# Joao-M-Silva/padel_analytics

Measured on AMD Instinct MI355X. Metric: frames/sec (all trackers) on 1280x720, higher is better.
Workload: dtype f32-equivalent (h2: fp16 pairs h + m/2048, 2 or 3 f16 MFMA products per multiply, fp32 accumulate)

## Files before the change

include/padel_hip.h:

```cpp
#ifndef PADEL_HIP_H
#define PADEL_HIP_H

#include <stddef.h>
#include <stdint.h>

#ifdef __cplusplus
extern "C" {
#endif

typedef struct pa_engine pa_engine;
typedef struct pa_model pa_model;

#define PA_ABI_VERSION 5


enum pa_op_kind {
    PA_OP_STEM = 1,
    PA_OP_CONV = 2,
    PA_OP_SPPF_POOL = 3,
    PA_OP_UPSAMPLE2X = 4,
    PA_OP_MAXPOOL2 = 5,
    PA_OP_STEM7 = 6,
    PA_OP_MAXPOOL3S2 = 7,
    PA_OP_GAP_FC = 8,
    PA_OP_DWCONV3 = 9,
    PA_OP_PSA_ATTN = 10
};

enum pa_act { PA_ACT_NONE = 0, PA_ACT_SILU = 1, PA_ACT_RELU = 2, PA_ACT_SIGMOID = 3, PA_ACT_LEAKY = 4  };

typedef struct pa_buf_desc {
    int32_t level;
    int32_t channels;
} pa_buf_desc;

typedef struct pa_op_desc {
    int32_t kind;
    int32_t in_buf, in_choff, cin;
    int32_t out_buf, out_choff, cout;
    int32_t ksize, stride, act;
    int32_t res_buf, res_choff;
    int32_t npad;
    int32_t reserved;
    int64_t w_off, b_off;
    int32_t flags;
    int32_t pad_;
} pa_op_desc;
#define PA_CONV_W_SINGLE 1
#define PA_CONV_RES_PREACT 4

enum pa_task { PA_TASK_DETECT = 0, PA_TASK_POSE = 1, PA_TASK_TRACKNET = 2, PA_TASK_RESNET = 3  };

enum pa_dtype { PA_DTYPE_F32 = 0, PA_DTYPE_F16 = 1, PA_DTYPE_H2 = 2 };

typedef struct pa_model_desc {
    int32_t task;
    int32_t nc;
    int32_t nk, kpt_dim;
    int32_t n_bufs;
    const pa_buf_desc* bufs;
    int32_t n_ops;
    const pa_op_desc* ops;
    int32_t head_buf[3];
    int32_t in_channels;
    int32_t dtype;
} pa_model_desc;

int pa_abi_version(void);
int pa_device_count(void);
int pa_engine_create(int device_id, pa_engine** out);
void pa_engine_destroy(pa_engine* eng);
const char* pa_last_error(pa_engine* eng);
int pa_engine_synchronize(pa_engine* eng);

int pa_device_malloc(pa_engine* eng, size_t nbytes, void** out_dev);
int pa_device_free(pa_engine* eng, void* dev);
size_t pa_device_bytes_live(void);
int pa_memcpy_h2d(pa_engine* eng, void* dst_dev, const void* src_host, size_t nbytes);
int pa_memcpy_d2h(pa_engine* eng, void* dst_host, const void* src_dev, size_t nbytes);
int pa_upload(pa_engine* eng, void* dst_dev, const void* src_host, size_t nbytes);

int pa_host_register(pa_engine* eng, void* ptr, size_t nbytes);
int pa_host_unregister(pa_engine* eng, void* ptr);

enum pa_yuv_layout {
    PA_YUV_NV12 = 0,
    PA_YUV_I420 = 1
};
typedef struct pa_yuv_desc {
    int32_t layout;
    int32_t pitch_y, pitch_c;
    int32_t off_u, off_v;
    int32_t reserved;
    int64_t frame_stride;
    int32_t y_off, cy, cvr, cug, cvg, cub;
} pa_yuv_desc;
int pa_yuv420_to_bgr(pa_engine* eng, const uint8_t* src, int src_on_device, int n, int h, int w,
                     const pa_yuv_desc* d, uint8_t* dst_bgr_dev);
int pa_yuv_last_path(pa_engine* eng);

enum pa_mark_kind { PA_MARK_DISC = 1, PA_MARK_SEGMENT = 2, PA_MARK_FILL = 3, PA_MARK_BOX = 4, PA_MARK_GLYPH = 5, PA_MARK_BLEND = 6 };
typedef struct pa_mark {
    int32_t kind;
    int32_t x0, y0, x1, y1;
    int32_t size;
    uint32_t bgr;
    int32_t arg;
} pa_mark;
typedef struct pa_yuv_enc {
    int32_t y_off;
    int32_t yr, yg, yb, ur, ug, ub, vr, vg, vb;
} pa_yuv_enc;
enum pa_render_out { PA_RENDER_BGR = 0, PA_RENDER_YUV420 = 1 };
int pa_render(pa_engine* eng, const uint8_t* src_bgr_dev, int n, int h, int w, const pa_mark* marks_host, const int32_t* first_host,
              int out, const pa_yuv_desc* geom, const pa_yuv_enc* enc, uint8_t* dst_dev);
int pa_render_check(int n, int h, int w, const pa_mark* marks_host, const int32_t* first_host, int out, const pa_yuv_desc* geom,
                    const pa_yuv_enc* enc, char* why, size_t cap);
int pa_render_last_path(pa_engine* eng);
int pa_glyph_rows(int code, uint8_t rows[7]);

#define PA_ACTIVITY_MAX_SIDE 16384
#define PA_ACTIVITY_MAX_FRAMES 65535
const char* pa_frame_activity_check(int n, int h, int w, const int32_t* roi, int tau);
int pa_frame_activity(pa_engine* eng, const uint8_t* frames_bgr_dev, int n, int h, int w, const uint8_t* ref_bgr_dev,
                      const uint8_t* prev_bgr_dev_or_null, const int32_t* roi_or_null, int tau, uint64_t* out_u64);
int pa_frames_median(pa_engine* eng, const uint8_t* frames_bgr_dev, int n, int h, int w, uint8_t* out_bgr_dev);

#define PA_BOX_HIST_BINS 512
#define PA_BOX_HIST_MAX_RECTS 16384
const char* pa_box_histograms_check(int n, int h, int w, const int32_t* rects, int k);
int pa_box_histograms(pa_engine* eng, const uint8_t* frames_bgr_dev, int n, int h, int w,
                      const int32_t* rects , int k, uint32_t* out_u32 );

#define PA_JPEG_MAX_WIDTH 2560
int pa_jpeg_encode(pa_engine* eng, const uint8_t* src_yuv_dev, int n, int h, int w, const pa_yuv_desc* geom, int quality,
                   uint8_t* dst_host, size_t cap, int64_t* offsets_host);
int pa_jpeg_check(int n, int h, int w, const pa_yuv_desc* geom, int quality, char* why, size_t cap);
size_t pa_jpeg_interval_bytes(int w);

#define PA_JPEG_DEC_MAX_DIM 4096
#define PA_JPEG_DEC_MAX_BYTES (1 << 27)
enum { PA_JPEG_ST_CODE = 1, PA_JPEG_ST_INDEX = 2, PA_JPEG_ST_SIZE = 4, PA_JPEG_ST_DATA = 8, PA_JPEG_ST_MARKERS = 16 };
typedef struct pa_jpeg_huff {
    uint8_t bits[16];
    uint8_t vals[256];
    int32_t nvals;
} pa_jpeg_huff;
typedef struct pa_jpeg_interval {
    int64_t begin, end;
    int32_t first_mcu, mcus;
} pa_jpeg_interval;
typedef struct pa_jpeg_frame_info {
    int32_t w, h, mcus_x, mcus_y;
    int32_t restart_interval;
    int32_t n_intervals;
    int32_t default_huffman;
    int32_t status;
    int64_t scan_begin, scan_end;
    uint8_t quant[3][64];
    uint8_t comp_dc[3], comp_ac[3], pad_[2];
    pa_jpeg_huff dc[2], ac[2];
} pa_jpeg_frame_info;
int pa_jpeg_parse(const uint8_t* jpeg, size_t len, pa_jpeg_frame_info* info, pa_jpeg_interval* ivls, size_t ivl_cap, char* why,
                  size_t cap);
int pa_jpeg_decode(pa_engine* eng, const uint8_t* jpegs_host, const int64_t* offsets, int n, int h, int w, uint8_t* dst_bgr_dev,
                   int32_t* status_host);
#define PA_JPEG_DEC_SPLIT_MIN_BYTES 7168
#define PA_JPEG_DEC_SPLIT_SUB_BYTES 128
int pa_jpeg_decode_set_split(pa_engine* eng, int64_t min_bytes, int32_t sub_bytes);
int pa_jpeg_decode_last_split(pa_engine* eng, int64_t out[4]);
int pa_jpeg_decode_last_path(pa_engine* eng);
int pa_jpeg_decode_last_times(pa_engine* eng, double ms[5]);

int pa_engine_timer_start(pa_engine* eng);
int pa_engine_timer_stop(pa_engine* eng, float* ms);

int pa_engine_set_tuning(pa_engine* eng, const char* key, int value);
int pa_engine_set_timeline_path(pa_engine* eng, const char* path);

int pa_model_create(pa_engine* eng, const pa_model_desc* desc, const float* weights, size_t n_floats,
                    pa_model** out);
void pa_model_destroy(pa_model* m);
int pa_model_take_overflow(pa_model* m, int* out);
int pa_model_set_max_batch(pa_model* m, int max_batch);
int pa_model_plan_bytes(pa_model* m, size_t* arena_bytes, size_t* logical_bytes);

int pa_model_fill_arena(pa_model* m, int byte_value);

enum pa_pre_mode {
    PA_PRE_LETTERBOX = 0,
    PA_PRE_PIL_STRETCH = 1
};

typedef struct pa_yolo_params {
    int32_t imgsz;
    int32_t pre_mode;
    int32_t channel_reverse;
    int32_t letterbox_auto;
    float conf, iou;
    int32_t max_det;
    int32_t n_classes;
    const int32_t* classes;
    int32_t frames_on_device;
} pa_yolo_params;

int pa_yolo_infer(pa_model* m, const uint8_t* frames, int n, int h, int w, const pa_yolo_params* p,
                  float* out_boxes, float* out_kpts, int32_t* out_counts);

#define PA_MAX_INFLIGHT 4
int pa_yolo_submit(pa_model* m, const uint8_t* frames, int n, int h, int w, const pa_yolo_params* p,
                   float* out_boxes, float* out_kpts, int32_t* out_counts, int* ticket);
int pa_yolo_wait(pa_model* m, int ticket, int* overflow);

int pa_yolo_postprocess(pa_model* m, const float* const* heads, int n, int h, int w, const pa_yolo_params* p,
                        float* out_boxes, float* out_kpts, int32_t* out_counts);

int pa_yolo_head_shape(pa_model* m, int level, int* h, int* w, int* c);
int pa_yolo_read_head(pa_model* m, int level, int n, float* out);
int pa_yolo_last_post_path(pa_model* m);
int pa_model_lanes_allocated(pa_model* m);
int pa_yolo_resample_passes(pa_model* m);
int pa_model_last_lane(pa_model* m);
int pa_model_last_stem_path(pa_model* m);

int pa_yolo_netin_shape(pa_model* m, int* h, int* w);
int pa_yolo_read_netin(pa_model* m, int n, uint8_t* out);

int pa_tracknet_infer(pa_model* m, const float* x, int n, int h, int w, int x_on_device, float* out,
                      int out_on_device);

int pa_resnet_infer(pa_model* m, const uint8_t* frames, int n, int h, int w, int frames_on_device, float* out_xy, float* out_logits);
int pa_resnet_read_netin(pa_model* m, int n, uint8_t* out);
int pa_resnet_read_fc(pa_model* m, int n, float* out_xy, float* out_logits);
int pa_resnet_read_head(pa_model* m, int n, float* out);

int pa_pil_coeffs(int in_size, int out_size, int filter, int32_t* bounds, int32_t* coefs, int coefs_cap, int* ksize);

typedef struct pa_ball pa_ball;
int pa_ball_create(pa_model* tracknet, int src_h, int src_w, pa_ball** out);
void pa_ball_destroy(pa_ball* b);
int pa_ball_set_background(pa_ball* b, const uint8_t* median_rgb);
int pa_ball_background_from_frames(pa_ball* b, const uint8_t* frames_bgr, int n, int frames_on_device,
                                   uint8_t* out_median_rgb);
int pa_ball_feed(pa_ball* b, const uint8_t* frames_bgr, int n, int frames_on_device, int flush,
                 uint8_t* out_masks, float* out_heat, int32_t* out_rects, int* out_count);

int pa_ball_locate(pa_ball* b, const uint8_t* masks, int n, int32_t* out_rects);

int pa_ball_read_resized(pa_ball* b, long long frame, uint8_t* out);

int pa_comm_unique_id(void* out, size_t cap);
int pa_engine_comm_init(pa_engine* eng, const void* unique_id, size_t id_bytes, int nranks, int rank);
void pa_engine_comm_destroy(pa_engine* eng);
int pa_engine_bcast_weights(pa_engine* eng, pa_model* m, int root);
int pa_engine_bcast_weights_from(pa_engine* eng, pa_model* src, pa_model* dst, int root);
int pa_engine_bcast(pa_engine* eng, void* dev_ptr, size_t nbytes, int root);
int pa_engine_allreduce_max(pa_engine* eng, double* value);
int pa_engine_gather_sizes(pa_engine* eng, size_t nbytes, uint64_t* sizes);
int pa_engine_gather(pa_engine* eng, const void* send, size_t nbytes, void* recv, size_t recv_cap, const uint64_t* sizes, int root);

typedef struct pa_bytetrack pa_bytetrack;
int pa_bytetrack_create(double track_activation_threshold, int lost_track_buffer, double minimum_matching_threshold,
                        int frame_rate, pa_bytetrack** out);
void pa_bytetrack_destroy(pa_bytetrack* b);
void pa_bytetrack_reset(pa_bytetrack* b);
int pa_bytetrack_update_batch(pa_bytetrack* b, const float* boxes, const int32_t* counts, const uint8_t* keep,
                              int n_frames, int stride, int32_t* out_ids);

int pa_engine_set_profiling(pa_engine* eng, int enable);
int pa_model_last_profile(pa_model* m, int cap, int32_t* kinds, float* ms, double* flops, int32_t* ksizes);
int pa_model_profile_text(pa_model* m, char* buf, size_t cap);

#ifdef __cplusplus
}
#endif
#endif
```

padel_analytics_amd/csrc/conv_patch_h2v.hip:

```cpp
#include "h2_common.h"

namespace padel {

namespace {

constexpr int kVSpans = (kPatchSqPix + 15) / 16;
constexpr int kVPlaneB = kVSpans * 1024;
constexpr int kVTSpans = (kPatchSqPix + 31) / 32;
constexpr int kVTPlaneB = kVTSpans * 1024;

}

template <int NF, bool CHUNK, bool TAIL, bool WS>
__global__ void __launch_bounds__(256, 2) conv_h2v_kernel(const ConvArgs a) {
    static_assert(CHUNK || TAIL, "cin = 32 CHUNK + 16 TAIL");
    static_assert(WS || NF <= 2, "three products: 2 fragments per wave (6 register sets of 4 VGPRs per step)");
    constexpr int MF = 4;
    constexpr int PATCH_B = (CHUNK ? 2 * kVPlaneB : 0);
    constexpr int TPATCH_B = (TAIL ? 2 * kVTPlaneB : 0);
    constexpr int NSTEPS = (CHUNK ? 9 : 0) + (TAIL ? 5 : 0);
    constexpr int NPL = WS ? 1 : 2;
    constexpr int NW = NF * NPL;
    __shared__ __attribute__((aligned(16))) float lds[(PATCH_B + TPATCH_B) / 4];
    char* const ldsb = reinterpret_cast<char*>(lds);
    const int tid = threadIdx.x;
    const int lane = tid & 63;
    const int wave = __builtin_amdgcn_readfirstlane(tid >> 6);
    const int lr = lane & 15, lq = lane >> 4;

    const int nmt = a.n_mtiles, nnt = a.n_ntiles;
    const int bid = blockIdx.x;
    const XcdSlot slot = xcd_slot(nmt, nnt, bid);
    if (xcd_slot_padding(slot)) return;
    const int mt = xcd_slot_mtile(slot), nt = slot.nt;
    const TileOrigin org = tile_origin<4, 4>(a.Ho, a.Wo, mt);
    const int n = org.n, y0 = org.y0, x0 = org.x0;
    const int f0 = nt * NF;

    const float* const in0 = a.in + (((long long)n * a.H + (y0 - 1)) * a.W + (x0 - 1)) * a.in_cs + a.in_choff;
    const i32x4 rsrcP = make_rsrc(in0);
    const unsigned lp0 = __builtin_amdgcn_readfirstlane((unsigned)(uintptr_t)lds);

    if constexpr (CHUNK) {
        const int p_lane = lane >> 2;
        const int p_q = (lane & 3) ^ (((lane >> 4) & 1) << 1);
        const unsigned p_piece = (unsigned)((p_q >> 1) * 64 + (p_q & 1) * 16);
#define PADEL_HV_PSPAN(S_)                                                                                        \
        if (((S_) & 3) == wave) {                                                                                 \
            const int pp_ = (S_) * 16 + p_lane;                                                                   \
            const int py_ = pp_ / kPatchW, px_ = pp_ - py_ * kPatchW;                                             \
            const bool ok_ = pp_ < kPatchSqPix && (unsigned)(y0 - 1 + py_) < (unsigned)a.H && (unsigned)(x0 - 1 + px_) < (unsigned)a.W; \
            const unsigned vo_ = ok_ ? (unsigned)((py_ * a.W + px_) * a.in_cs * 4) + p_piece : kOOR;              \
            lds_dma<(S_) * 1024>(vo_, rsrcP, 0u, lp0);                                                            \
            lds_dma<kVPlaneB + (S_) * 1024>(vo_, rsrcP, 32u, lp0);                                                \
        }
        PADEL_HV_PSPAN(0) PADEL_HV_PSPAN(1) PADEL_HV_PSPAN(2) PADEL_HV_PSPAN(3) PADEL_HV_PSPAN(4) PADEL_HV_PSPAN(5) PADEL_HV_PSPAN(6)
        PADEL_HV_PSPAN(7) PADEL_HV_PSPAN(8) PADEL_HV_PSPAN(9) PADEL_HV_PSPAN(10) PADEL_HV_PSPAN(11) PADEL_HV_PSPAN(12) PADEL_HV_PSPAN(13)
        PADEL_HV_PSPAN(14) PADEL_HV_PSPAN(15) PADEL_HV_PSPAN(16) PADEL_HV_PSPAN(17) PADEL_HV_PSPAN(18) PADEL_HV_PSPAN(19) PADEL_HV_PSPAN(20)
#undef PADEL_HV_PSPAN
    }
    if constexpr (TAIL) {
        const int t_lane = lane >> 1;
        const unsigned t_piece = (unsigned)(((lane & 1) ^ ((lane >> 4) & 1)) * 16);
        const unsigned t_so = CHUNK ? 128u : 0u;
#define PADEL_HV_TSPAN(S_)                                                                                        \
        if (((S_) & 3) == ((wave + 1) & 3)) {                                                                     \
            const int pp_ = (S_) * 32 + t_lane;                                                                   \
            const int py_ = pp_ / kPatchW, px_ = pp_ - py_ * kPatchW;                                             \
            const bool ok_ = pp_ < kPatchSqPix && (unsigned)(y0 - 1 + py_) < (unsigned)a.H && (unsigned)(x0 - 1 + px_) < (unsigned)a.W; \
            const unsigned vo_ = ok_ ? (unsigned)((py_ * a.W + px_) * a.in_cs * 4) + t_piece : kOOR;              \
            lds_dma<PATCH_B + (S_) * 1024>(vo_, rsrcP, t_so, lp0);                                                \
            lds_dma<PATCH_B + kVTPlaneB + (S_) * 1024>(vo_, rsrcP, t_so + 32u, lp0);                              \
        }
        PADEL_HV_TSPAN(0) PADEL_HV_TSPAN(1) PADEL_HV_TSPAN(2) PADEL_HV_TSPAN(3) PADEL_HV_TSPAN(4) PADEL_HV_TSPAN(5)
        PADEL_HV_TSPAN(6) PADEL_HV_TSPAN(7) PADEL_HV_TSPAN(8) PADEL_HV_TSPAN(9) PADEL_HV_TSPAN(10)
#undef PADEL_HV_TSPAN
    }

    constexpr unsigned fragb = (unsigned)NSTEPS * 2048u;
    const unsigned voffW = (unsigned)lane * 16u;
    i32x4 rsrcW[NF];
#pragma unroll
    for (int j = 0; j < NF; ++j) {
        const int frag = min(f0 + j, a.n16 - 1);
        rsrcW[j] = make_rsrc(reinterpret_cast<const char*>(a.wr) + (long long)frag * fragb);
    }
    i32x4 w[3][NF], wm[3][WS ? 1 : NF];
#define PADEL_HV_LOADW(ST_)                                                                                       \
    do {                                                                                                          \
        const unsigned so_ = (unsigned)((ST_) * 2048);                                                            \
        _Pragma("unroll") for (int j = 0; j < NF; ++j) {                                                          \
            asm volatile("buffer_load_dwordx4 %0, %1, %2, %3 offen"                                               \
                         : "=v"(w[(ST_) % 3][j]) : "v"(voffW), "s"(rsrcW[j]), "s"(so_) : "memory");               \
            if constexpr (!WS)                                                                                    \
                asm volatile("buffer_load_dwordx4 %0, %1, %2, %3 offen offset:1024"                               \
                             : "=v"(wm[(ST_) % 3][j]) : "v"(voffW), "s"(rsrcW[j]), "s"(so_) : "memory");          \
        }                                                                                                         \
    } while (0)
#define PADEL_HV_WAITW(ST_, N_)                                                                                   \
    do {                                                                                                          \
        if constexpr (NF == 3)                                                                                    \
            asm volatile("s_waitcnt vmcnt(%3)" : "+v"(w[(ST_) % 3][0]), "+v"(w[(ST_) % 3][1]), "+v"(w[(ST_) % 3][2]) : "n"(N_) : "memory"); \
        else if constexpr (NF == 2 && WS)                                                                         \
            asm volatile("s_waitcnt vmcnt(%2)" : "+v"(w[(ST_) % 3][0]), "+v"(w[(ST_) % 3][1]) : "n"(N_) : "memory"); \
        else if constexpr (NF == 2)                                                                               \
            asm volatile("s_waitcnt vmcnt(%4)" : "+v"(w[(ST_) % 3][0]), "+v"(w[(ST_) % 3][1]), "+v"(wm[(ST_) % 3][0]), "+v"(wm[(ST_) % 3][WS ? 0 : NF - 1]) \
                         : "n"(N_) : "memory");                                                                   \
        else if constexpr (WS)                                                                                    \
            asm volatile("s_waitcnt vmcnt(%1)" : "+v"(w[(ST_) % 3][0]) : "n"(N_) : "memory");                     \
        else                                                                                                      \
            asm volatile("s_waitcnt vmcnt(%2)" : "+v"(w[(ST_) % 3][0]), "+v"(wm[(ST_) % 3][0]) : "n"(N_) : "memory"); \
    } while (0)

    unsigned rbase[8];
    if constexpr (CHUNK) {
#pragma unroll
        for (int r = 0; r < 8; ++r) {
            const int p0 = 4 * wave * kPatchW + lr;
            rbase[r] = (unsigned)(p0 * 64 + ((lq ^ ((((p0 + r) >> 2) & 1) << 1)) << 4));
        }
    }
    const int rd_pix = 4 * wave * kPatchW + lr;

    f32x4 acc[MF][NF], part[MF][NF], cross[MF][NF];
#pragma unroll
    for (int f = 0; f < MF; ++f)
#pragma unroll
        for (int j = 0; j < NF; ++j) { acc[f][j] = (f32x4){0.f, 0.f, 0.f, 0.f}; part[f][j] = acc[f][j]; cross[f][j] = acc[f][j]; }
    h16x8 ah[4], am[4];
#define PADEL_HV_READROW(R_, KX_)                                                                                 \
    do {                                                                                                          \
        constexpr int d_ = (R_) * kPatchW + (KX_);                                                                \
        const char* p_ = ldsb + rbase[d_ & 7];                                                                    \
        ah[(R_) & 3] = *reinterpret_cast<const h16x8*>(p_ + d_ * 64);                                             \
        am[(R_) & 3] = *reinterpret_cast<const h16x8*>(p_ + d_ * 64 + kVPlaneB);                                  \
    } while (0)
#define PADEL_HV_MFMA_ROW(F_, S_, ST_)                                                                            \
    do {                                                                                                          \
        _Pragma("unroll") for (int j = 0; j < NF; ++j)                                                            \
            cross[F_][j] = __builtin_amdgcn_mfma_f32_16x16x32_f16(__builtin_bit_cast(h16x8, w[(ST_) % 3][j]), am[S_], cross[F_][j], 0, 0, 0); \
        if constexpr (!WS) {                                                                                      \
            _Pragma("unroll") for (int j = 0; j < NF; ++j)                                                        \
                cross[F_][j] = __builtin_amdgcn_mfma_f32_16x16x32_f16(__builtin_bit_cast(h16x8, wm[(ST_) % 3][WS ? 0 : j]), ah[S_], cross[F_][j], 0, 0, 0); \
        }                                                                                                         \
        _Pragma("unroll") for (int j = 0; j < NF; ++j)                                                            \
            part[F_][j] = __builtin_amdgcn_mfma_f32_16x16x32_f16(__builtin_bit_cast(h16x8, w[(ST_) % 3][j]), ah[S_], part[F_][j], 0, 0, 0); \
        __builtin_amdgcn_sched_barrier(0);                                                                        \
    } while (0)
#define PADEL_HV_TOP(ST_)                                                                                         \
    do {                                                                                                          \
        if constexpr ((ST_) + 2 < NSTEPS) PADEL_HV_LOADW((ST_) + 2);                                              \
        PADEL_HV_WAITW(ST_, NW * (((ST_) + 1 < NSTEPS ? 1 : 0) + ((ST_) + 2 < NSTEPS ? 1 : 0)));                  \
        __builtin_amdgcn_sched_barrier(0);                                                                        \
    } while (0)
#define PADEL_HV_STEP(T_)                                                                                         \
    do {                                                                                                          \
        constexpr int kx_ = h2_tap_kx(T_), ky_ = h2_tap_ky(T_);                                                   \
        PADEL_HV_TOP(T_);                                                                                         \
        if constexpr (ky_ == 0) {                                                                                 \
            PADEL_HV_MFMA_ROW(0, 0, T_);                                                                          \
            PADEL_HV_READROW(4, kx_);                                                                             \
            __builtin_amdgcn_sched_barrier(0);                                                                    \
            PADEL_HV_MFMA_ROW(1, 1, T_); PADEL_HV_MFMA_ROW(2, 2, T_); PADEL_HV_MFMA_ROW(3, 3, T_);                \
        } else if constexpr (ky_ == 1) {                                                                          \
            PADEL_HV_MFMA_ROW(0, 1, T_);                                                                          \
            PADEL_HV_READROW(5, kx_);                                                                             \
            __builtin_amdgcn_sched_barrier(0);                                                                    \
            PADEL_HV_MFMA_ROW(1, 2, T_); PADEL_HV_MFMA_ROW(2, 3, T_); PADEL_HV_MFMA_ROW(3, 0, T_);                \
        } else {                                            \
            PADEL_HV_MFMA_ROW(2, 0, T_);                                                                          \
            if constexpr (kx_ < 2) PADEL_HV_READROW(0, kx_ + 1);                                                  \
            __builtin_amdgcn_sched_barrier(0);                                                                    \
            PADEL_HV_MFMA_ROW(3, 1, T_);                                                                          \
            if constexpr (kx_ < 2) PADEL_HV_READROW(1, kx_ + 1);                                                  \
            __builtin_amdgcn_sched_barrier(0);                                                                    \
            PADEL_HV_MFMA_ROW(0, 2, T_);                                                                          \
            if constexpr (kx_ < 2) PADEL_HV_READROW(2, kx_ + 1);                                                  \
            __builtin_amdgcn_sched_barrier(0);                                                                    \
            PADEL_HV_MFMA_ROW(1, 3, T_);                                                                          \
            if constexpr (kx_ < 2) PADEL_HV_READROW(3, kx_ + 1);                                                  \
            __builtin_amdgcn_sched_barrier(0);                                                                    \
        }                                                                                                         \
    } while (0)
#define PADEL_HV_TSTEP(JT_, ST_)                                                                                  \
    do {                                                                                                          \
        constexpr int ta_ = 2 * (JT_), tb_ = 2 * (JT_) + 1 < 9 ? 2 * (JT_) + 1 : 8;                               \
        int rp_ = rd_pix;                                                                                         \
        asm volatile("" : "+v"(rp_));                                                                             \
        _Pragma("unroll") for (int f = 0; f < MF; ++f) {                                                          \
            const int pa_ = rp_ + (f + h2_tap_ky(ta_)) * kPatchW + h2_tap_kx(ta_), pb_ = rp_ + (f + h2_tap_ky(tb_)) * kPatchW + h2_tap_kx(tb_); \
            const char* p_ = ldsb + PATCH_B + swz_tail_off((lq >> 1) ? pb_ : pa_, lq & 1);                        \
            ah[f] = *reinterpret_cast<const h16x8*>(p_);                                                          \
            am[f] = *reinterpret_cast<const h16x8*>(p_ + kVTPlaneB);                                              \
        }                                                                                                         \
        __builtin_amdgcn_sched_barrier(0);                                                                        \
        PADEL_HV_TOP(ST_);                                                                                        \
        PADEL_HV_MFMA_ROW(0, 0, ST_); PADEL_HV_MFMA_ROW(1, 1, ST_); PADEL_HV_MFMA_ROW(2, 2, ST_); PADEL_HV_MFMA_ROW(3, 3, ST_); \
    } while (0)
#define PADEL_HV_FLUSH()                                                                                          \
    do {                                                                                                          \
        _Pragma("unroll") for (int f = 0; f < MF; ++f)                                                            \
            _Pragma("unroll") for (int j = 0; j < NF; ++j) { acc[f][j] += part[f][j]; part[f][j] = (f32x4){0.f, 0.f, 0.f, 0.f}; } \
    } while (0)

    PADEL_HV_LOADW(0);
    if constexpr (NSTEPS > 1) PADEL_HV_LOADW(1);
    wait_vm<NW * (NSTEPS > 1 ? 2 : 1)>();
    __builtin_amdgcn_s_barrier();
    asm volatile("" ::: "memory");
    if constexpr (CHUNK) {
        PADEL_HV_READROW(0, 0); PADEL_HV_READROW(1, 0); PADEL_HV_READROW(2, 0); PADEL_HV_READROW(3, 0);
        __builtin_amdgcn_sched_barrier(0);
        PADEL_HV_STEP(0); PADEL_HV_STEP(1); PADEL_HV_STEP(2); PADEL_HV_STEP(3); PADEL_HV_STEP(4);
        PADEL_HV_STEP(5); PADEL_HV_STEP(6); PADEL_HV_STEP(7); PADEL_HV_STEP(8);
        PADEL_HV_FLUSH();
    }
    if constexpr (TAIL) {
        constexpr int S0 = CHUNK ? 9 : 0;
        PADEL_HV_TSTEP(0, S0); PADEL_HV_TSTEP(1, S0 + 1); PADEL_HV_TSTEP(2, S0 + 2); PADEL_HV_TSTEP(3, S0 + 3); PADEL_HV_TSTEP(4, S0 + 4);
        PADEL_HV_FLUSH();
    }
#undef PADEL_HV_FLUSH
#undef PADEL_HV_TSTEP
#undef PADEL_HV_STEP
#undef PADEL_HV_TOP
#undef PADEL_HV_MFMA_ROW
#undef PADEL_HV_READROW
#undef PADEL_HV_WAITW
#undef PADEL_HV_LOADW

    int mpix[MF];
#pragma unroll
    for (int f = 0; f < MF; ++f) {
        const int oy = y0 + 4 * wave + f, ox = x0 + lr;
        mpix[f] = (oy < a.Ho && ox < a.Wo) ? (n * a.Ho + oy) * a.Wo + ox : -1;
    }
    const bool fast = y0 + 16 <= a.Ho && x0 + 16 <= a.Wo && (f0 + NF) * 16 <= a.cout && (((a.out_choff | a.out_cs) & 3) == 0) &&
                      (!a.res || (((a.res_choff | a.res_cs) & 3) == 0));
    h2_epilogue<MF, NF>(a, acc, cross, mpix, f0, lq, fast);
}

template <int NF, bool WS>
static hipError_t launch_hv(const ConvArgs& a_in, hipStream_t s) {
    ConvArgs a = a_in;
    const int batch = a.M / (a.Ho * a.Wo);
    a.n_mtiles = batch * ((a.Ho + 15) / 16) * ((a.Wo + 15) / 16);
    a.n_ntiles = (a.n16 + NF - 1) / NF;
    dim3 grid(8u * (unsigned)((a.n_mtiles + 7) / 8) * (unsigned)a.n_ntiles, 1, 1);
    if (a.cin == 48) hipLaunchKernelGGL((conv_h2v_kernel<NF, true, true, WS>), grid, dim3(256), 0, s, a);
    else if (a.cin == 32) hipLaunchKernelGGL((conv_h2v_kernel<NF, true, false, WS>), grid, dim3(256), 0, s, a);
    else hipLaunchKernelGGL((conv_h2v_kernel<NF, false, true, WS>), grid, dim3(256), 0, s, a);
    return hipGetLastError();
}

hipError_t launch_conv_h2v(const ConvArgs& a, int tile, hipStream_t s) {
    const int nf = tile - 340;
    if (a.w_single) {
        switch (nf) {
            case 1: return launch_hv<1, true>(a, s);
            case 2: return launch_hv<2, true>(a, s);
            case 3: return launch_hv<3, true>(a, s);
        }
    } else {
        switch (nf) {
            case 1: return launch_hv<1, false>(a, s);
            case 2: return launch_hv<2, false>(a, s);
        }
    }
    return hipErrorNotSupported;
}

}
```

padel_analytics_amd/csrc/conv_select.cpp:

```cpp
#include "kernels.h"

#include <string.h>

namespace padel {

struct ConvTile {
    int id;
    ConvFamily family;
    int rows, cols, bn;
    float s3, s1;
};

static const ConvTile kTapTiles[] = {
    {7, CONV_TAP, 0, 64, 96, 1.00f, 1.00f},   {13, CONV_TAP, 0, 128, 96, 0.99f, 0.99f}, {9, CONV_TAP, 0, 128, 64, 0.99f, 0.99f},
    {14, CONV_TAP, 0, 128, 128, 1.00f, 1.00f}, {6, CONV_TAP, 0, 64, 128, 0.98f, 0.98f},  {20, CONV_TAP, 0, 128, 48, 0.98f, 0.98f},
    {11, CONV_TAP, 0, 128, 32, 0.99f, 0.99f},  {12, CONV_TAP, 0, 128, 16, 0.80f, 0.80f},
    {10, CONV_TAP, 0, 128, 64, 0.f, 0.f},
    {15, CONV_TAP, 0, 128, 64, 0.f, 0.f},
};

static const ConvTile kBx3Tiles[] = {
    {213, CONV_BX3T, 0, 128, 96, 1.07f, 1.08f},
    {220, CONV_BX3T, 0, 128, 48, 1.00f, 1.00f}, {207, CONV_BX3T, 0, 64, 96, 0.98f, 0.95f}, {209, CONV_BX3T, 0, 128, 64, 1.00f, 1.00f},
    {206, CONV_BX3T, 0, 64, 128, 0.90f, 0.70f}, {211, CONV_BX3T, 0, 128, 32, 0.85f, 0.87f}, {225, CONV_BX3T, 0, 64, 80, 0.95f, 0.90f},
    {7, CONV_BX3T, 0, 64, 96, 0.93f, 0.84f},    {20, CONV_BX3T, 0, 128, 48, 0.93f, 0.87f}, {13, CONV_BX3T, 0, 128, 96, 0.85f, 0.82f},
    {14, CONV_BX3T, 0, 128, 128, 0.83f, 0.85f}, {25, CONV_BX3T, 0, 64, 80, 0.90f, 0.78f},
    {11, CONV_BX3T, 0, 128, 32, 0.80f, 0.61f},  {9, CONV_BX3T, 0, 128, 64, 0.65f, 0.70f},  {6, CONV_BX3T, 0, 64, 128, 0.50f, 0.49f},
    {12, CONV_BX3T, 0, 128, 16, 0.45f, 0.26f},
    {303, CONV_BX3P, 8, 16, 48, 1.17f, 0.f},    {304, CONV_BX3P, 8, 16, 64, 1.14f, 0.f},   {306, CONV_BX3P, 8, 16, 96, 0.f, 0.f},
#ifdef PADEL_BX3_PROBES
    {420, CONV_BX3T, 0, 128, 48, 0.f, 0.f},     {520, CONV_BX3T, 0, 128, 48, 0.f, 0.f},    {620, CONV_BX3T, 0, 128, 48, 0.f, 0.f},
    {720, CONV_BX3T, 0, 128, 48, 0.f, 0.f},     {820, CONV_BX3T, 0, 128, 48, 0.f, 0.f},    {920, CONV_BX3T, 0, 128, 48, 0.f, 0.f},
    {1020, CONV_BX3T, 0, 128, 48, 0.f, 0.f},    {1120, CONV_BX3T, 0, 128, 48, 0.f, 0.f},
#endif
};

static const ConvTile kH2Tiles[] = {
    {213, CONV_H2T, 0, 128, 96, 1.07f, 1.08f},
    {220, CONV_H2T, 0, 128, 48, 1.00f, 1.00f}, {207, CONV_H2T, 0, 64, 96, 0.98f, 0.95f}, {209, CONV_H2T, 0, 128, 64, 1.00f, 1.00f},
    {211, CONV_H2T, 0, 128, 32, 0.85f, 0.87f}, {225, CONV_H2T, 0, 64, 80, 0.95f, 0.90f},
    {239, CONV_H2D, 0, 128, 64, 0.f, 0.f},     {243, CONV_H2D, 0, 128, 96, 0.f, 0.f},
    {244, CONV_H2S, 0, 128, 96, 0.f, 0.f},     {245, CONV_H2S, 0, 128, 192, 0.f, 0.f},   {247, CONV_H2S, 0, 64, 192, 0.f, 0.f},
    {246, CONV_H2S3, 0, 128, 192, 0.f, 0.f},   {248, CONV_H2S3, 0, 64, 192, 0.f, 0.f},
    {303, CONV_H2P, 8, 16, 48, 1.17f, 0.f},    {304, CONV_H2P, 8, 16, 64, 1.10f, 0.f},
    {313, CONV_H2P, 8, 16, 48, 0.f, 0.f},
    {323, CONV_H2Q, 8, 16, 96, 1.21f, 0.f},
    {324, CONV_H2R, 8, 16, 96, 1.40f, 0.f},
    {325, CONV_H2R, 8, 16, 64, 1.33f, 0.f},
    {341, CONV_H2V, 16, 16, 16, 0.f, 0.f},     {341, CONV_H2W, 16, 16, 16, 1.28f, 0.f},
    {342, CONV_H2V, 16, 16, 32, 0.f, 0.f},     {342, CONV_H2W, 16, 16, 32, 1.42f, 0.f},
    {343, CONV_H2V, 16, 16, 48, 0.f, 0.f},     {343, CONV_H2W, 16, 16, 48, 1.46f, 0.f},
#ifdef PADEL_H2P_PROBES
    {333, CONV_H2P, 8, 16, 48, 0.f, 0.f},      {334, CONV_H2P, 8, 16, 48, 0.f, 0.f},     {335, CONV_H2P, 8, 16, 48, 0.f, 0.f},
    {336, CONV_H2P, 8, 16, 48, 0.f, 0.f},      {337, CONV_H2P, 8, 16, 48, 0.f, 0.f},     {339, CONV_H2P, 8, 16, 48, 0.f, 0.f},
    {340, CONV_H2P, 8, 16, 48, 0.f, 0.f},      {347, CONV_H2P, 8, 16, 48, 0.f, 0.f},     {348, CONV_H2P, 8, 16, 48, 0.f, 0.f},
    {349, CONV_H2P, 8, 16, 48, 0.f, 0.f},      {363, CONV_H2P, 8, 16, 48, 0.f, 0.f},
#endif
};
static const float kH2rThreeProducts = 1.22f;

static const ConvTile kF16Tiles[] = {
    {30, CONV_TAP16, 0, 128, 128, 1.30f, 1.30f},
    {31, CONV_TAP16, 0, 128, 96, 1.25f, 1.25f},  {32, CONV_TAP16, 0, 128, 64, 1.10f, 1.10f},  {6, CONV_TAP16, 0, 64, 128, 1.05f, 1.05f},
    {7, CONV_TAP16, 0, 64, 96, 1.00f, 1.00f},    {9, CONV_TAP16, 0, 128, 64, 1.00f, 1.00f},   {20, CONV_TAP16, 0, 128, 48, 0.95f, 0.95f},
    {11, CONV_TAP16, 0, 128, 32, 0.85f, 0.85f},  {12, CONV_TAP16, 0, 128, 16, 0.60f, 0.60f},
    {49, CONV_TAP16D, 0, 128, 64, 1.40f, 0.f},   {72, CONV_TAP16D, 0, 128, 64, 1.40f, 0.f},
    {46, CONV_TAP16D, 0, 64, 128, 0.f, 0.f},     {47, CONV_TAP16D, 0, 64, 96, 0.f, 0.f},      {51, CONV_TAP16D, 0, 128, 32, 0.f, 0.f},
    {60, CONV_TAP16D, 0, 128, 48, 0.f, 0.f},     {70, CONV_TAP16D, 0, 128, 128, 0.f, 0.f},    {71, CONV_TAP16D, 0, 128, 96, 0.f, 0.f},
    {304, CONV_P16, 8, 16, 64, 1.70f, 0.f},      {303, CONV_P16, 8, 16, 48, 1.55f, 0.f},      {306, CONV_P16, 8, 16, 96, 1.45f, 0.f},
    {323, CONV_P16Q, 16, 16, 48, 0.f, 0.f},      {324, CONV_P16Q, 16, 16, 64, 0.f, 0.f},      {326, CONV_P16Q, 16, 16, 96, 1.78f, 0.f},
};

struct TileSpan { const ConvTile* t; int n; };
static TileSpan tiles_of(int path) {
    switch (path) {
        case CONV_PATH_TAP: return {kTapTiles, (int)(sizeof(kTapTiles) / sizeof(ConvTile))};
        case CONV_PATH_BX3: return {kBx3Tiles, (int)(sizeof(kBx3Tiles) / sizeof(ConvTile))};
        case CONV_PATH_H2: return {kH2Tiles, (int)(sizeof(kH2Tiles) / sizeof(ConvTile))};
        case CONV_PATH_F16: return {kF16Tiles, (int)(sizeof(kF16Tiles) / sizeof(ConvTile))};
    }
    return {nullptr, 0};
}
static const ConvTile* find_tile(int path, int id, int family = -1) {
    const TileSpan ts = tiles_of(path);
    for (int i = 0; i < ts.n; ++i)
        if (ts.t[i].id == id && (family < 0 || ts.t[i].family == family)) return &ts.t[i];
    return nullptr;
}

bool conv_tile_shape(int path, int id, int* bm, int* bn) {
    const ConvTile* t = find_tile(path, id);
    if (!t) return false;
    *bm = t->rows ? t->rows * t->cols : t->cols;
    *bn = t->bn;
    return true;
}

int conv_timeline_words(const ConvLaunched& k, int ksize) {
    if (!strcmp(k.family, "h2q") || (!strcmp(k.family, "h2r") && k.tile == 324)) return kPatchDbgWords;
    if (!strcmp(k.family, "tap") && k.tile == 7 && ksize == 3) return kConvDbgWords;
    return 0;
}

int h2_ksteps(int cin, int ksize) { return ksize == 3 ? (cin >> 5) * 9 + ((cin & 16) ? 5 : 0) : (cin + 31) >> 5; }
size_t conv_h2r_copy_bytes(int n16, int cin, int ksize) { return (size_t)n16 * (size_t)h2_ksteps(cin, ksize) * 2048; }

static bool few_channels(int cin) { return cin == 16 || cin == 32 || cin == 48; }
static bool whole_chunks(int cin, int at_least) { return (cin & 31) == 0 && cin >= at_least; }
static bool h2r_layer(int k, int s, int cin) { return k == 3 && s == 1 && whole_chunks(cin, 64); }
static bool h2v_layer(int k, int s, int cin) { return k == 3 && s == 1 && few_channels(cin); }
static bool h2s_layer(int k, int s, int cin) { return k == 1 && s == 1 && whole_chunks(cin, 64); }
static bool h2s3_layer(int k, int s, int cin) { return k == 3 && s == 2 && whole_chunks(cin, 32); }
static bool stem_l1_layer(int k, int s, int cin) { return k == 3 && s == 2 && few_channels(cin); }

bool conv_wants_operand_copy(int ksize, int stride, int cin, bool w_single) {
    return h2r_layer(ksize, stride, cin) || h2v_layer(ksize, stride, cin) || stem_l1_layer(ksize, stride, cin) ||
           (w_single && (h2s_layer(ksize, stride, cin) || h2s3_layer(ksize, stride, cin)));
}

static bool same_size(const ConvArgs& a) { return a.Ho == a.H && a.Wo == a.W; }
static bool up_ok(const ConvArgs& a) { return (a.up_c & 31) == 0 && a.up_c > 0 && a.up_c <= a.cin && ((a.H | a.W) & 1) == 0; }
static bool up_ok_1x1(const ConvArgs& a) { return !a.in2 || (a.ksize == 1 && a.stride == 1 && up_ok(a)); }
static bool up_ok_patch(const ConvArgs& a) { return !a.in2 || ((a.cin & 31) == 0 && up_ok(a)); }

static bool conv_bx3p_supported(const ConvArgs& a) {
    return a.ksize == 3 && a.stride == 1 && (a.cin & 15) == 0 && a.cin >= 16 && same_size(a) && a.w3 != nullptr && up_ok_patch(a);
}
static bool conv_h2p_supported(const ConvArgs& a) {
    return a.ksize == 3 && a.stride == 1 && (a.cin & 15) == 0 && a.cin >= 16 && same_size(a) && a.w != nullptr && up_ok_patch(a);
}
static bool conv_h2q_supported(const ConvArgs& a) {
    return a.ksize == 3 && a.stride == 1 && whole_chunks(a.cin, 32) && same_size(a) && a.w != nullptr && !a.in2;
}
static bool conv_h2r_supported(const ConvArgs& a) {
    return a.wr && h2r_layer(a.ksize, a.stride, a.cin) && same_size(a) && a.w != nullptr && !a.in2;
}
static bool conv_h2w_supported(const ConvArgs& a) {
    return a.ksize == 3 && a.stride == 1 && few_channels(a.cin) && same_size(a) && a.w != nullptr && !a.in2;
}
static bool conv_h2v_supported(const ConvArgs& a) {
    return a.wr && h2v_layer(a.ksize, a.stride, a.cin) && same_size(a) && a.w != nullptr && !a.in2;
}
static bool conv_h2s_supported(const ConvArgs& a) {
    return a.w_single && a.wr && h2s_layer(a.ksize, a.stride, a.cin) && same_size(a) && a.w != nullptr && !a.in2 &&
           (long long)128 * a.in_cs * 4 < 0x7FFFFFFFll;
}
static bool conv_h2s3_supported(const ConvArgs& a) {
    return a.w_single && a.wr && h2s3_layer(a.ksize, a.stride, a.cin) && a.w != nullptr && !a.in2 && a.Ho <= (a.H + 1) / 2 &&
           a.Wo <= (a.W + 1) / 2 && (long long)4 * a.W * a.in_cs * 4 < 0x3FFFFFFFll;
}
static bool conv_p16_supported(const ConvArgs& a) { return a.ksize == 3 && a.stride == 1 && whole_chunks(a.cin, 32) && same_size(a); }

static bool family_takes(ConvFamily family, const ConvArgs& a, int id) {
    switch (family) {
        case CONV_TAP: case CONV_TAP16: case CONV_TAP16D: return true;
        case CONV_BX3T: return id < 400 ? up_ok_1x1(a) : a.ksize == 3;
        case CONV_BX3P: return conv_bx3p_supported(a);
        case CONV_H2T: return up_ok_1x1(a);
        case CONV_H2D: return a.ksize == 1 && up_ok_1x1(a);
        case CONV_H2S: return conv_h2s_supported(a);
        case CONV_H2S3: return conv_h2s3_supported(a);
        case CONV_H2P: return conv_h2p_supported(a) && (id < 330 || (!a.in2 && !(a.cin & 16)));
        case CONV_H2Q: return conv_h2q_supported(a);
        case CONV_H2R: return conv_h2r_supported(a) && (id == 325 || a.w_single);
        case CONV_H2V: return !(a.tune & 8) && conv_h2v_supported(a) && (id < 343 || a.w_single);
        case CONV_H2W: return conv_h2w_supported(a);
        case CONV_P16: case CONV_P16Q: return conv_p16_supported(a);
    }
    return false;
}

struct Resolved { int tile; ConvFamily family; };
static bool take(int path, const ConvArgs& a, int id, ConvFamily family, Resolved* out) {
    if (!find_tile(path, id, family) || !family_takes(family, a, id)) return false;
    out->tile = id; out->family = family;
    return true;
}
static bool take(int path, const ConvArgs& a, int id, Resolved* out) {
    const ConvTile* t = find_tile(path, id);
    return t && take(path, a, id, t->family, out);
}

static bool resolve_bx3(const ConvArgs& a, int id, Resolved* out) {
    if ((a.cin & 15) || a.cin < 16 || !a.w3) return false;
    const bool patch_id = id >= 300 && id < 400;
    if (a.in2 && a.ksize == 3) return patch_id && take(CONV_PATH_BX3, a, id, CONV_BX3P, out);
    if (a.in2) {
        id = (id == 209 || id == 9 || id == 304) ? 209 : (id == 213 || id == 13 || id == 14 || id == 306 || id == 206 || id == 6) ? 213 : 220;
        return take(CONV_PATH_BX3, a, id, CONV_BX3T, out);
    }
    if (patch_id) {
        if (conv_bx3p_supported(a)) return take(CONV_PATH_BX3, a, id, CONV_BX3P, out);
        id = id == 303 ? 220 : id == 304 ? 209 : 206;
    }
    return take(CONV_PATH_BX3, a, id, CONV_BX3T, out);
}

static bool resolve_f16(const ConvArgs& a, int id, Resolved* out) {
    if ((a.cin & 31) || a.cin < 32 || a.res_pre) return false;
    if (id >= 300 && id < 400) {
        if (conv_p16_supported(a)) return take(CONV_PATH_F16, a, id, out);
        id = id == 303 ? 20 : id == 304 ? 9 : 31;
    }
    return take(CONV_PATH_F16, a, id, out);
}

static bool resolve_h2(const ConvArgs& a, int id, Resolved* out) {
    const int P = CONV_PATH_H2;
    if ((a.cin & 15) || a.cin < 16 || !a.w || !a.oscale || !a.ovf_flag) return false;
    if (id >= 341 && id <= 343) {
        if (take(P, a, id, CONV_H2V, out) || take(P, a, id, CONV_H2W, out)) return true;
        id = 303;
    }
    if (id == 324 || id == 325) {
        if (take(P, a, id, CONV_H2R, out)) return true;
        id = id == 324 ? 323 : 304;
    }
    if (id == 323) {
        if (take(P, a, id, CONV_H2Q, out)) return true;
        id = 303;
    }
    if (a.in2 && a.ksize == 3) return id >= 300 && id < 400 && take(P, a, id, CONV_H2P, out);
    if (id >= 300 && id < 400) {
        if (conv_h2p_supported(a)) return take(P, a, id, CONV_H2P, out);
        const int nf = id - 300;
        id = (nf == 3 || nf == 13) ? 220 : (nf == 4 || nf == 14) ? 209 : 213;
    }
    if (id == 246 || id == 248) {
        if (take(P, a, id, CONV_H2S3, out)) return true;
        id = 213;
    }
    if (id == 244 || id == 245 || id == 247) {
        if (take(P, a, id, CONV_H2S, out)) return true;
        id = 243;
    }
    if (id == 243 || id == 239) {
        if (take(P, a, id, CONV_H2D, out)) return true;
        id -= 30;
    }
    return take(P, a, id, CONV_H2T, out);
}

const char* conv_family_name(ConvFamily f) {
    static const char* const names[] = {"tap", "bx3t", "bx3p", "h2t", "h2d", "h2s", "h2s3", "h2p", "h2q", "h2r", "h2w", "h2v", "tap16", "tap16d", "p16", "p16q"};
    return names[f];
}

bool resolve_conv(int path, const ConvArgs& a, int requested, ConvLaunched* out, ConvFamily* family) {
    Resolved r{-1, CONV_TAP};
    if (a.ksize != 3 && a.ksize != 1) return false;
    bool ok = false;
    switch (path) {
        case CONV_PATH_TAP: ok = !(a.cin & 15) && a.cin >= 16 && !a.res_pre && take(path, a, requested, &r); break;
        case CONV_PATH_BX3: ok = resolve_bx3(a, requested, &r); break;
        case CONV_PATH_H2: ok = resolve_h2(a, requested, &r); break;
        case CONV_PATH_F16: ok = resolve_f16(a, requested, &r); break;
    }
    if (ok && out) *out = ConvLaunched{r.tile, conv_family_name(r.family)};
    if (ok && family) *family = r.family;
    return ok;
}

static float tile_score(const ConvTile& t, const ConvArgs& a, float speed, bool rounds = true) {
    const int nf = t.bn / 16, bm = t.rows ? t.rows * t.cols : t.cols;
    const long long mtiles = t.rows ? (long long)(a.M / (a.Ho * a.Wo)) * ((a.Ho + t.rows - 1) / t.rows) * ((a.Wo + t.cols - 1) / t.cols)
                                    : (long long)((a.M + bm - 1) / bm);
    const int ntiles = (a.n16 + nf - 1) / nf;
    const float fill = (float)a.n16 / (float)(ntiles * nf) * (float)a.M / (float)(mtiles * bm);
    if (!rounds) return speed * fill;
    const long long blocks = mtiles * ntiles;
    const long long per_cu = (blocks + 255) / 256;
    if (t.rows) return speed * fill * (float)blocks / (256.f * (float)per_cu);
    const float occ = (float)blocks / (256.f * (float)per_cu);
    return speed * fill * occ;
}
struct Best {
    float score = -1.f;
    int id;
    void offer(float sc, int tile) { if (sc > score) { score = sc; id = tile; } }
};
static void offer_linear(Best& b, int path, const ConvArgs& a) {
    const TileSpan ts = tiles_of(path);
    for (int i = 0; i < ts.n; ++i) {
        const float sp = a.ksize == 3 ? ts.t[i].s3 : ts.t[i].s1;
        if (!ts.t[i].rows && sp > 0.0f) b.offer(tile_score(ts.t[i], a, sp), ts.t[i].id);
    }
}

int choose_conv_tap_variant(int M, int n16) {
    ConvArgs a{};
    a.M = M; a.n16 = n16; a.ksize = 3;
    Best b{-1.f, 7};
    offer_linear(b, CONV_PATH_TAP, a);
    return b.id;
}

int choose_conv_bx3_variant(const ConvArgs& a) {
    Best b{-1.f, 7};
    offer_linear(b, CONV_PATH_BX3, a);
    if (conv_bx3p_supported(a))
        for (const ConvTile& t : kBx3Tiles)
            if (t.rows && t.s3 > 0.f) b.offer(tile_score(t, a, t.s3), t.id);
    return b.id;
}

int choose_conv_tap16_variant(const ConvArgs& a) {
    const bool dbl_ok = a.ksize == 3 && (a.cin & 63) == 0 && a.cin >= 128;
    const int nch = a.cin >> 5;
    const bool patch_ok = conv_p16_supported(a);
    Best b{-1.f, 7};
    for (const ConvTile& t : kF16Tiles) {
        if (t.s3 <= 0.f) continue;
        if (t.rows) {
            if (patch_ok) b.offer(tile_score(t, a, t.s3 * (float)nch / (float)(nch + 1)), t.id);
            continue;
        }
        const bool dbl = t.family == CONV_TAP16D;
        if (dbl && !dbl_ok) continue;
        const int ntiles = (a.n16 + t.bn / 16 - 1) / (t.bn / 16);
        const float reread = 1.0f / (1.0f + 0.25f * (float)(ntiles - 1));
        b.offer(tile_score(t, a, t.s3) * (dbl ? 1.0f : reread), t.id);
    }
    return b.id;
}

int choose_conv_h2_variant(const ConvArgs& a) {
    const int n16 = a.n16, ksize = a.ksize;
    Best b{-1.f, 220};
    offer_linear(b, CONV_PATH_H2, a);
    int& bv = b.id;
    if (ksize == 1 && a.cin >= 192 && (bv == 213 || bv == 209)) bv += 30;
    if (ksize == 1 && a.w_single && n16 >= 24 && a.cin >= 384 && conv_h2s_supported(a)) bv = 245;
    if (ksize == 1 && a.w_single && n16 >= 12 && (float)(((n16 + 11) / 12) * 12) <= 1.1f * (float)n16 && a.cin >= 192 && a.cin < 960 &&
        conv_h2s_supported(a)) bv = 247;
    if (ksize == 3 && a.stride == 2 && n16 >= 10 && (float)(((n16 + 11) / 12) * 12) <= 1.2f * (float)n16 && conv_h2s3_supported(a)) bv = 246;
    if (bv == 246 && a.cin != 192) bv = 248;
    if (!conv_h2p_supported(a)) return bv;
    for (const ConvTile& t : kH2Tiles) {
        if (!t.rows || t.s3 <= 0.f || !family_takes(t.family, a, t.id)) continue;
        if (t.id == 323 && n16 % 6 != 0) continue;
        const bool persistent = t.family == CONV_H2R;
        b.offer(tile_score(t, a, t.id == 325 && !a.w_single ? kH2rThreeProducts : t.s3, !persistent), t.id);
    }
    if (bv == 303 && (a.cin & 16)) bv = 313;
    return bv;
}

}
```

padel_analytics_amd/csrc/engine.cpp:

```cpp
#include "engine_internal.h"

#include <atomic>

thread_local std::string g_err;

static std::atomic<size_t> g_live_bytes{0};
int dev_alloc(void** p, size_t bytes) { const hipError_t r = hipMalloc(p, bytes); if (r == hipSuccess) g_live_bytes += bytes; return (int)r; }
void dev_free(void* p, size_t bytes) { (void)hipFree(p); g_live_bytes -= bytes; }
int pin_alloc(void** p, size_t bytes) { return (int)hipHostMalloc(p, bytes, hipHostMallocDefault); }
void pin_free(void* p, size_t) { (void)hipHostFree(p); }
size_t pa_device_bytes_live(void) { return g_live_bytes.load(); }

static int knob_raw(int v) { return v; }
static int knob_flag(int v) { return v ? 1 : 0; }
static int knob_tap_pd(int v) { return v == 3 ? 3 : 2; }
static int knob_lanes(int v) { return v >= 2 ? 2 : 1; }
static const struct Knob { const char* key; const char* env; int Tuning::*field; int (*norm)(int); } kKnobs[] = {
    {"variant", "PADEL_CONV_VARIANT", &Tuning::variant, knob_raw},
    {"tune", "PADEL_CONV_TUNE", &Tuning::tune, knob_raw},
    {"tap_pd", "PADEL_CONV_TAP_PD", &Tuning::tap_pd, knob_tap_pd},
    {"graph", "PADEL_GRAPH", &Tuning::graph, knob_flag},
    {"timeline", nullptr, &Tuning::timeline, knob_flag},
    {"alias", "PADEL_ALIAS", &Tuning::alias, knob_flag},
    {"fold_up", "PADEL_FOLD_UP", &Tuning::fold_up, knob_flag},
    {"lanes", "PADEL_LANES", &Tuning::lanes, knob_lanes},
    {"fuse_stem", "PADEL_FUSE_STEM", &Tuning::fuse_stem, knob_raw},
    {"fuse_sppf", "PADEL_FUSE_SPPF", &Tuning::fuse_sppf, knob_raw},
    {"fuse_head", "PADEL_FUSE_HEAD", &Tuning::fuse_head, knob_flag},
    {"fuse_stem_cv1", "PADEL_FUSE_STEM_CV1", &Tuning::fuse_stem_cv1, knob_flag},
    {"w_single", nullptr, &Tuning::w_single, knob_flag},
};

int pa_abi_version(void) { return PA_ABI_VERSION; }

int pa_device_count(void) {
    int n = 0;
    if (hipGetDeviceCount(&n) != hipSuccess) return 0;
    return n;
}

const char* pa_last_error(pa_engine* eng) { return eng ? eng->err.c_str() : g_err.c_str(); }

int pa_engine_create(int device_id, pa_engine** out) {
    if (!out) PA_FAIL((pa_engine*)nullptr, "pa_engine_create: out is NULL");
    int n = 0;
    PA_HIP((pa_engine*)nullptr, hipGetDeviceCount(&n));
    if (device_id < 0 || device_id >= n) PA_FAIL((pa_engine*)nullptr, "pa_engine_create: device %d of %d", device_id, n);
    PA_HIP((pa_engine*)nullptr, hipSetDevice(device_id));
    pa_engine* e = new pa_engine();
    e->dev = device_id;
    hipError_t r = e->create_streams();
    if (r == hipSuccess) r = hipStreamCreateWithFlags(&e->copy_stream, hipStreamNonBlocking);
    if (r != hipSuccess) { pa_engine_destroy(e); PA_FAIL((pa_engine*)nullptr, "hipStreamCreate: %s", hipGetErrorString(r)); }
    r = (hipError_t)e->zeros.alloc(256);
    if (r == hipSuccess) r = hipMemset(e->zeros.get(), 0, 256);
    if (r != hipSuccess) { delete e; PA_FAIL((pa_engine*)nullptr, "zero page: %s", hipGetErrorString(r)); }
    r = padel::init_misc_kernels();
    if (r == hipSuccess) r = padel::init_head_tail_kernels();
    if (r != hipSuccess) { delete e; PA_FAIL((pa_engine*)nullptr, "kernel attributes: %s", hipGetErrorString(r)); }
    if (const char* v = getenv("PADEL_CONV_IMPL")) {
        if (v[0] == 'l') { delete e; PA_FAIL((pa_engine*)nullptr, "PADEL_CONV_IMPL=%s: the LDS kernel was retired in round 5; tap or bx3", v); }
        e->t.impl = (v[0] == 'b') ? 2 : 0;
    }
    for (const Knob& k : kKnobs)
        if (const char* v = k.env ? getenv(k.env) : nullptr) e->t.*k.field = k.norm(atoi(v));
    *out = e;
    return 0;
}

hipError_t pa_engine::create_streams() {
    hipError_t r = hipStreamCreateWithFlags(&main_, hipStreamNonBlocking);
    for (int i = 0; i < kMaxLanes && r == hipSuccess; ++i) {
        r = hipStreamCreateWithFlags(&lane_stream[i], hipStreamNonBlocking);
        if (r == hipSuccess) r = hipEventCreateWithFlags(&fork_ev_[i], hipEventDisableTiming);
    }
    return r;
}

void pa_engine::destroy_streams() {
    for (int i = 0; i < kMaxLanes; ++i) {
        if (lane_stream[i]) { hipStreamSynchronize(lane_stream[i]); hipStreamDestroy(lane_stream[i]); }
        if (fork_ev_[i]) hipEventDestroy(fork_ev_[i]);
        lane_stream[i] = nullptr; fork_ev_[i] = nullptr;
    }
    if (main_) hipStreamDestroy(main_);
    main_ = nullptr;
}

hipError_t pa_engine::fork_lane(int i) {
    if (forked_seq_[i] == main_seq_) return hipSuccess;
    hipError_t r = hipEventRecord(fork_ev_[i], main_);
    if (r == hipSuccess) r = hipStreamWaitEvent(lane_stream[i], fork_ev_[i], 0);
    if (r == hipSuccess) forked_seq_[i] = main_seq_;
    return r;
}

hipError_t pa_engine::sync_lanes() {
    for (hipStream_t s : lane_stream)
        if (s) { const hipError_t r = hipStreamSynchronize(s); if (r != hipSuccess) return r; }
    return hipSuccess;
}

int pa_engine_set_tuning(pa_engine* e, const char* key, int value) {
    if (!e || !key) return 1;
    if (!strcmp(key, "impl")) {
        if (value != 0 && value != 2) PA_FAIL(e, "tuning impl = %d: 0 (fp32-input MFMA tap kernels) or 2 (bf16x3); 1 was the LDS kernel, retired in round 5 (tools/legacy_conv)", value);
        e->t.impl = value;
    } else {
        const Knob* k = std::find_if(std::begin(kKnobs), std::end(kKnobs), [&](const Knob& c) { return !strcmp(c.key, key); });
        if (k == std::end(kKnobs)) PA_FAIL(e, "pa_engine_set_tuning: unknown key '%s'", key);
        e->t.*k->field = k->norm(value);
    }
    e->tuning_epoch++;
    return 0;
}

int pa_engine_set_timeline_path(pa_engine* e, const char* path) {
    if (!e) return 1;
    e->timeline_path = path ? path : "";
    return 0;
}

void pa_engine_destroy(pa_engine* e) {
    if (!e) return;
    hipSetDevice(e->dev);
    pa_engine_comm_destroy(e);
    if (e->main_stream_wait_only()) hipStreamSynchronize(e->main_stream_wait_only());
    jpeg_scratch_free(e);
    jpeg_dec_scratch_free(e);
    for (hipEvent_t ev : e->timer_ev) if (ev) hipEventDestroy(ev);
    e->destroy_streams();
    if (e->copy_stream) hipStreamDestroy(e->copy_stream);
    delete e;
}

int pa_engine_synchronize(pa_engine* e) {
    PA_HIP(e, hipSetDevice(e->dev));
    PA_HIP(e, hipStreamSynchronize(e->main_stream_wait_only()));
    return 0;
}

int pa_engine_set_profiling(pa_engine* e, int enable) { e->profiling = enable != 0; return 0; }

int pa_device_malloc(pa_engine* e, size_t nbytes, void** out) {
    PA_HIP(e, hipSetDevice(e->dev));
    PA_HIP(e, hipMalloc(out, nbytes));
    return 0;
}
int pa_device_free(pa_engine* e, void* p) {
    PA_HIP(e, hipSetDevice(e->dev));
    PA_HIP(e, hipFree(p));
    return 0;
}
int pa_memcpy_h2d(pa_engine* e, void* dst, const void* src, size_t n) {
    PA_HIP(e, hipSetDevice(e->dev));
    PA_HIP(e, hipMemcpyAsync(dst, src, n, hipMemcpyHostToDevice, e->main_stream()));
    PA_HIP(e, hipStreamSynchronize(e->main_stream_wait_only()));
    return 0;
}
int pa_upload(pa_engine* e, void* dst, const void* src, size_t n) {
    PA_HIP(e, hipSetDevice(e->dev));
    PA_HIP(e, hipMemcpyAsync(dst, src, n, hipMemcpyHostToDevice, e->copy_stream));
    PA_HIP(e, hipStreamSynchronize(e->copy_stream));
    return 0;
}
int pa_host_register(pa_engine* e, void* ptr, size_t nbytes) {
    PA_HIP(e, hipSetDevice(e->dev));
    PA_HIP(e, hipHostRegister(ptr, nbytes, hipHostRegisterDefault));
    return 0;
}
int pa_host_unregister(pa_engine* e, void* ptr) {
    PA_HIP(e, hipSetDevice(e->dev));
    PA_HIP(e, hipHostUnregister(ptr));
    return 0;
}
int pa_memcpy_d2h(pa_engine* e, void* dst, const void* src, size_t n) {
    PA_HIP(e, hipSetDevice(e->dev));
    PA_HIP(e, hipMemcpyAsync(dst, src, n, hipMemcpyDeviceToHost, e->main_stream()));
    PA_HIP(e, hipStreamSynchronize(e->main_stream_wait_only()));
    return 0;
}

int pa_engine_timer_start(pa_engine* e) {
    if (!e) return 1;
    PA_HIP(e, hipSetDevice(e->dev));
    for (hipEvent_t& ev : e->timer_ev) if (!ev) PA_HIP(e, hipEventCreate(&ev));
    PA_HIP(e, hipEventRecord(e->timer_ev[0], e->main_stream()));
    return 0;
}
int pa_engine_timer_stop(pa_engine* e, float* ms) {
    if (!e || !ms) return 1;
    if (!e->timer_ev[0] || !e->timer_ev[1]) PA_FAIL(e, "pa_engine_timer_stop without pa_engine_timer_start");
    PA_HIP(e, hipSetDevice(e->dev));
    PA_HIP(e, hipEventRecord(e->timer_ev[1], e->main_stream()));
    PA_HIP(e, hipEventSynchronize(e->timer_ev[1]));
    PA_HIP(e, hipEventElapsedTime(ms, e->timer_ev[0], e->timer_ev[1]));
    return 0;
}

int pa_model_create(pa_engine* e, const pa_model_desc* desc, const float* weights, size_t n_floats, pa_model** out) {
    if (!e || !desc || !out) PA_FAIL(e, "pa_model_create: NULL argument");
    std::string why;
    if (validate_desc(desc, n_floats, why)) PA_FAIL(e, "%s", why.c_str());
    PA_HIP(e, hipSetDevice(e->dev));
    pa_model* m = new pa_model();
    m->e = e;
    m->d = *desc;
    m->bufs.assign(desc->bufs, desc->bufs + desc->n_bufs);
    m->ops.assign(desc->ops, desc->ops + desc->n_ops);
    m->d.bufs = m->bufs.data();
    m->d.ops = m->ops.data();
    std::vector<int> fold_dst;
    find_upsample_folds(m->d, m->fold_src, fold_dst);
    m->stem_fuse.resize(m->ops.size());
    for (size_t i = 0; i < m->ops.size(); ++i) m->stem_fuse[i] = stem_cv1_fusable(m->d, i) ? 2 : stem_fusable(m->d, i) ? 1 : 0;
    m->tail = find_head_tail(m->d, m->fold_src);
    m->n_w = n_floats;
    if (desc->task == PA_TASK_DETECT || desc->task == PA_TASK_POSE)
        for (int i = 0; i < kMaxLanes; ++i) m->ln[i].stream = e->lane_stream[i];
    hipError_t r = (hipError_t)m->d_w.alloc(n_floats * sizeof(float) + kConvReadSlack);
    if (r == hipSuccess)
        r = weights ? hipMemcpyAsync(m->d_w.get(), weights, n_floats * sizeof(float), hipMemcpyHostToDevice, e->main_stream())
                    : hipMemsetAsync(m->d_w.get(), 0, n_floats * sizeof(float), e->main_stream());
    if (r == hipSuccess) r = hipMemsetAsync(m->d_w.get() + n_floats, 0, kConvReadSlack, e->main_stream());
    if (r == hipSuccess) r = (hipError_t)m->d_ovf.alloc(256);
    if (r == hipSuccess) r = hipMemsetAsync(m->d_ovf.get(), 0, 256, e->main_stream());
    if (r == hipSuccess) r = (hipError_t)m->h_pin.alloc(64 * sizeof(unsigned));
    if (r == hipSuccess) memset(m->h_pin.get(), 0, 64 * sizeof(unsigned));
    for (int k = 0; k < PA_MAX_INFLIGHT && r == hipSuccess; ++k) r = hipEventCreateWithFlags(&m->tk_ev[k], hipEventDisableTiming);
    if (r == hipSuccess) r = hipStreamSynchronize(e->main_stream_wait_only());
    if (r != hipSuccess) { delete m; PA_FAIL(e, "weights upload: %s", hipGetErrorString(r)); }
    *out = m;
    return 0;
}

static void destroy_graphs(pa_model* m) {
    for (Lane& L : m->ln) {
        for (auto& g : L.graphs) hipGraphExecDestroy(g.second);
        L.graphs.clear();
    }
}

void free_lane(Lane& L) {
    for (auto& g : L.graphs) hipGraphExecDestroy(g.second);
    L.graphs.clear();
    const hipStream_t s = L.stream;
    L = Lane{};
    L.stream = s;
}

void free_plan(pa_model* m) {
    (void)m->e->sync_lanes();
    for (Lane& L : m->ln) free_lane(L);
    m->d_xtab.reset();
    m->d_ytab.reset();
    m->rs = ResamplePlan{};
    m->lane1_refused = false;
    m->last_lane = 0;
    m->planned = false;
    m->heads_stale = false;
}

void pa_model_destroy(pa_model* m) {
    if (!m) return;
    hipSetDevice(m->e->dev);
    hipStreamSynchronize(m->e->main_stream_wait_only());
    free_plan(m);
    for (auto& r : m->prof) { hipEventDestroy(r.e0); hipEventDestroy(r.e1); }
    for (int k = 0; k < PA_MAX_INFLIGHT; ++k) if (m->tk_ev[k]) hipEventDestroy(m->tk_ev[k]);
    delete m;
}

int pa_model_take_overflow(pa_model* m, int* out) {
    if (!m || !out) return 1;
    pa_engine* e = m->e;
    *out = 0;
    if (!guards_range(m)) return 0;
    PA_HIP(e, hipSetDevice(e->dev));
    unsigned v = 0;
    if (m->ovf_cached) {
        v = m->h_ovf;
    } else {
        PA_HIP(e, hipMemcpyAsync(&v, m->d_ovf.get(), sizeof(v), hipMemcpyDeviceToHost, e->main_stream()));
        PA_HIP(e, hipStreamSynchronize(e->main_stream_wait_only()));
    }
    m->ovf_cached = false;
    m->h_ovf = 0;
    if (v) {
        PA_HIP(e, hipMemsetAsync(m->d_ovf.get(), 0, sizeof(v), e->main_stream()));
        PA_HIP(e, hipStreamSynchronize(e->main_stream_wait_only()));
    }
    *out = v ? 1 : 0;
    return 0;
}

int pa_model_set_max_batch(pa_model* m, int max_batch) {
    if (max_batch < 1) PA_FAIL(m->e, "max_batch %d", max_batch);
    if (max_batch != m->max_batch) { hipSetDevice(m->e->dev); hipStreamSynchronize(m->e->main_stream_wait_only()); free_plan(m); m->max_batch = max_batch; }
    return 0;
}

int plan_buffers(pa_model* m, Lane& L, int batch, hipStream_t s) {
    pa_engine* e = m->e;
    BufferPlan bp;
    std::string why;
    if (plan_activations(m->d, m->fold_src, m->net_h, m->net_w, batch, e->t.alias != 0, bp, why, &m->tail)) PA_FAIL(e, "%s", why.c_str());
    m->fc_nout = 0;
    m->conv_flops = 0;
    for (const auto& o : m->ops) {
        if (o.kind == PA_OP_GAP_FC) m->fc_nout = o.cout;
        if (o.kind == PA_OP_CONV) {
            const int lvl = m->bufs[o.out_buf].level;
            m->conv_flops += 2.0 * batch * (double)(m->net_h >> lvl) * (m->net_w >> lvl) * o.cout * o.cin * o.ksize * o.ksize;
        }
    }
    if (m->fc_nout) {
        PA_HIP(e, L.d_fc.alloc((size_t)batch * 2 * kGapFcMaxOut * sizeof(float)));
        PA_HIP(e, hipMemsetAsync(L.d_fc.get(), 0, (size_t)batch * 2 * kGapFcMaxOut * sizeof(float), s));
    }
    PA_HIP(e, L.arena.alloc(bp.arena_bytes + kConvReadSlack));
    PA_HIP(e, hipMemsetAsync(L.arena.get(), 0, bp.arena_bytes + kConvReadSlack, s));
    L.bptr.assign(m->bufs.size(), nullptr);
    for (size_t i = 0; i < m->bufs.size(); ++i) L.bptr[i] = reinterpret_cast<float*>(L.arena.get() + bp.off[i]);
    L.allocated = true;
    m->arena_bytes = bp.arena_bytes;
    m->logical_bytes = bp.logical_bytes;
    m->p_batch = batch;
    return 0;
}

ProfRec* prof_begin(pa_model* m, hipStream_t s, size_t idx, int kind, int ksize, double flops) {
    if (!m->e->profiling) return nullptr;
    if (m->prof.size() <= idx) {
        m->prof.resize(idx + 1);
        hipEventCreate(&m->prof[idx].e0);
        hipEventCreate(&m->prof[idx].e1);
    }
    ProfRec* r = &m->prof[idx];
    r->kind = kind; r->ksize = ksize; r->flops = flops; r->ms = 0.f;
    r->M = r->cout = r->cin = r->stride = r->mf = r->nf = r->res = 0;
    r->tile = -1; r->family = "";
    hipEventRecord(r->e0, s);
    return r;
}

static PlanPointers plan_pointers(const pa_model* m, const Lane& L) {
    return PlanPointers{L.bptr.data(), m->d_w.get(), m->d_wr.get(), m->wr_valid ? m->wr_off.data() : nullptr, m->e->zeros.get(), m->d_ovf.get(),
                        L.d_netin.get(), L.d_fc.get(), m->p_batch};
}

static int plan_steps(pa_model* m, Lane& L, int n) {
    std::string why;
    if (build_steps(m->d, m->fold_src, m->stem_fuse, m->tail, m->e->t, plan_pointers(m, L), m->net_h, m->net_w, n, L.steps, why,
                    hipGetErrorString(hipErrorNotSupported)))
        PA_FAIL(m->e, "%s", why.c_str());
    return 0;
}

void head_tail_convs(const pa_model* m, const Lane& L, HeadTailArgs& a) {
    bool single = m->e->t.w_single != 0;
    for (int l = 0; l < 3; ++l)
        for (int c = 0; c < 3; ++c) {
            HeadTailConv& v = a.cv[l][c];
            v = HeadTailConv{};
            const int i = m->tail.op[l][c];
            if (i < 0) continue;
            const pa_op_desc& o = m->ops[i];
            v.in = L.bptr[o.in_buf]; v.in_cs = m->bufs[o.in_buf].channels; v.in_choff = o.in_choff;
            v.w = m->d_w.get() + o.w_off; v.bias = m->d_w.get() + o.b_off; v.oscale = m->d_w.get() + o.reserved;
            v.cin = o.cin; v.n16 = o.npad / 16;
            single = single && (o.flags & PA_CONV_W_SINGLE);
        }
    a.w_single = single ? 1 : 0;
}

bool head_fused(const pa_model* m) {
    const pa_engine* e = m->e;
    if (!e->t.fuse_head || m->d.dtype != PA_DTYPE_H2 || !m->tail.found || e->profiling || e->t.timeline || !m->planned) return false;
    HeadTailArgs a{};
    a.d.cs = m->bufs[m->d.head_buf[0]].channels; a.d.nc = m->d.nc; a.d.nk = m->d.nk;
    head_tail_convs(m, m->ln[0], a);
    return head_tail_h2_supported(a);
}

static hipError_t launch_step(const Step& st, const ConvArgs& a, hipStream_t s) {
    const SliceArgs& v = st.sl;
    switch (st.kind) {
        case PA_OP_CONV: return launch_conv_family(st.family, a, st.ran.tile, s);
        case PA_OP_STEM: return st.n_ops == 2 ? launch_stem_l1_h2(st.stem, a, nullptr, s) : launch_stem(st.stem, s);
        case PA_OP_SPPF_POOL: return launch_sppf_pool(v.in, v.in_cs, v.in_choff, v.c, v.B, v.H, v.W, s, v.fmt, v.fused);
        case PA_OP_UPSAMPLE2X: return launch_upsample2x(v.in, v.in_cs, v.in_choff, v.out, v.out_cs, v.out_choff, v.c, v.B, v.H, v.W, s, v.fmt);
        case PA_OP_MAXPOOL2: return launch_maxpool2(v.in, v.in_cs, v.in_choff, v.out, v.out_cs, v.out_choff, v.c, v.B, v.H, v.W, s, v.fmt);
        case PA_OP_MAXPOOL3S2: return launch_maxpool3s2(v.in, v.in_cs, v.in_choff, v.out, v.out_cs, v.out_choff, v.c, v.B, v.H, v.W, v.Ho, v.Wo, s, v.fmt);
        case PA_OP_STEM7: return launch_stem7(st.stem7, s);
        case PA_OP_GAP_FC: return launch_gap_fc(v.in, v.in_cs, v.in_choff, v.c, v.B, v.H, v.w, v.bias, v.nout, v.logits, v.probs, s, v.fmt);
        case PA_OP_DWCONV3: return launch_dwconv3(st.dw, s);
        case PA_OP_PSA_ATTN: return launch_psa_attn(st.attn, s);
    }
    return hipSuccess;
}

static hipError_t launch_conv_timeline(pa_model* m, const Step& st, hipStream_t s) {
    pa_engine* e = m->e;
    ConvArgs a = st.conv;
    const size_t patches = (size_t)(a.M / (a.Ho * a.Wo)) * ((a.Ho + 7) / 8) * ((a.Wo + 15) / 16);
    const size_t records = st.path == CONV_PATH_H2 ? 8 * ((patches + 7) / 8) * (size_t)((a.n16 + 5) / 6)
                                                   : (size_t)((a.M + 63) / 64) * ((m->ops[st.op].npad + 95) / 96);
    const size_t dbg_bytes = records * conv_timeline_words(st.ran, a.ksize) * 8;
    DevMem<unsigned long long> dbg_dev;
    if (dbg_bytes && dbg_dev.alloc(dbg_bytes) == 0) (void)hipMemsetAsync(dbg_dev.get(), 0, dbg_bytes, s);
    a.dbg = dbg_dev.get();
    const hipError_t r = launch_step(st, a, s);
    if (dbg_dev) {
        (void)hipStreamSynchronize(s);
        std::vector<unsigned long long> host(dbg_bytes / 8);
        (void)hipMemcpy(host.data(), dbg_dev.get(), dbg_bytes, hipMemcpyDeviceToHost);
        if (FILE* f = fopen(e->timeline_path.c_str(), "wb")) { fwrite(host.data(), 1, dbg_bytes, f); fclose(f); }
    }
    return r;
}

int run_tail_ops(pa_model* m, Lane& L, hipStream_t s, int n) {
    if (plan_steps(m, L, n)) return 1;
    for (const Step& st : L.steps) {
        if (!st.tail) continue;
        const hipError_t r = launch_step(st, st.conv, s);
        if (r != hipSuccess) PA_FAIL(m->e, "op %d (head tail) launch failed: %s", st.op, hipGetErrorString(r));
    }
    return 0;
}

static int run_ops(pa_model* m, Lane& L, hipStream_t s, int n, size_t* pi, bool skip_tail) {
    pa_engine* e = m->e;
    if (plan_steps(m, L, n)) return 1;
    const bool cv1_fused = !e->profiling && !e->t.timeline;
    m->last_stem_path = 0;
    for (const Step& st : L.steps) {
        if (skip_tail && st.tail) continue;
        if (cv1_fused && st.stem_cv1) continue;
        if (cv1_fused && st.kind == PA_OP_STEM && st.n_ops == 2 && st.has_cv1) {
            const hipError_t r = launch_stem_l1_h2(st.stem, st.conv, &st.cv1, s);
            if (r != hipSuccess) PA_FAIL(e, "fused stem + layer 1 + 1x1 launch failed: %s", hipGetErrorString(r));
            m->last_stem_path = 1;
            ++*pi;
            continue;
        }
        ProfRec* pr = prof_begin(m, s, (*pi)++, st.kind, st.ksize, st.flops);
        if (pr) {
            pr->M = st.M; pr->cout = st.cout; pr->cin = st.cin; pr->stride = st.stride; pr->mf = st.mf; pr->nf = st.nf; pr->res = st.res;
            pr->tile = st.ran.tile; pr->family = st.ran.family;
        }
        const bool timeline = st.kind == PA_OP_CONV && e->t.timeline && !e->timeline_path.empty() && st.ran.tile == st.requested;
        const hipError_t r = timeline ? launch_conv_timeline(m, st, s) : launch_step(st, st.conv, s);
        prof_end(s, pr);
        if (r != hipSuccess && st.n_ops == 2) PA_FAIL(e, "fused stem + layer 1 launch failed: %s", hipGetErrorString(r));
        if (r != hipSuccess) PA_FAIL(e, "op %d (kind %d) launch failed: %s", st.op, st.kind, hipGetErrorString(r));
    }
    return 0;
}

static int ensure_operand_copies(pa_model* m) {
    if (m->wr_valid || m->d.dtype != PA_DTYPE_H2) return 0;
    pa_engine* e = m->e;
    {
        bool any = false;
        PA_HIP(e, hipMemsetAsync(m->d_ovf.get() + 32, 0, sizeof(unsigned) * 8, e->main_stream()));
        for (size_t i = 0; i < m->ops.size(); ++i) {
            const pa_op_desc& o = m->ops[i];
            if (o.kind != PA_OP_CONV || !(o.flags & PA_CONV_W_SINGLE)) continue;
            PA_HIP(e, launch_h2_mplane_check(m->d_w.get() + o.w_off, (long long)o.npad * h2_ksteps(o.cin, o.ksize), m->d_ovf.get() + 32, e->main_stream()));
            any = true;
        }
        if (any) {
            unsigned bad = 0;
            PA_HIP(e, hipMemcpyAsync(&bad, m->d_ovf.get() + 32, sizeof(bad), hipMemcpyDeviceToHost, e->main_stream()));
            PA_HIP(e, hipStreamSynchronize(e->main_stream_wait_only()));
            if (bad) PA_FAIL(e, "a conv flagged PA_CONV_W_SINGLE has a non-zero m plane in the weight blob (pack it without the flag, or with fp16-number weights)");
        }
    }
    if (m->wr_off.empty()) {
        std::vector<long long> off;
        const size_t total = operand_copy_offsets(m->d, m->stem_fuse, off);
        if (total) {
            PA_HIP(e, m->d_wr.fit(total + 8192, total + 8192));
            PA_HIP(e, hipMemsetAsync(m->d_wr.get() + total, 0, 8192, e->main_stream()));
        }
        m->wr_off = std::move(off);
    }
    for (size_t i = 0; i < m->ops.size(); ++i) {
        if (m->wr_off[i] < 0) continue;
        const pa_op_desc& o = m->ops[i];
        if (o.kind == PA_OP_STEM) {
            PA_HIP(e, launch_stem_l1_operands(m->d_w.get() + o.w_off, o.cout, m->d_wr.get() + m->wr_off[i], e->main_stream()));
            continue;
        }
        PA_HIP(e, launch_h2r_repack(m->d_w.get() + o.w_off, m->d_wr.get() + m->wr_off[i], o.npad / 16, o.cin, o.ksize, e->main_stream()));
    }
    PA_HIP(e, hipStreamSynchronize(e->main_stream_wait_only()));
    m->wr_valid = true;
    return 0;
}

int run_graph(pa_model* m, Lane& L, hipStream_t s, int n, size_t* pi, bool skip_tail) {
    pa_engine* e = m->e;
    if (ensure_operand_copies(m)) return 1;
    if (!e->t.graph || e->profiling || e->t.timeline) return run_ops(m, L, s, n, pi, skip_tail);
    if (m->graph_epoch != e->tuning_epoch) {
        PA_HIP(e, hipStreamSynchronize(e->main_stream_wait_only()));
        PA_HIP(e, e->sync_lanes());
        destroy_graphs(m);
        m->graph_epoch = e->tuning_epoch;
    }
    auto it = L.graphs.find(n);
    if (it == L.graphs.end()) {
        hipGraph_t g = nullptr;
        hipGraphExec_t ge = nullptr;
        PA_HIP(e, hipStreamBeginCapture(s, hipStreamCaptureModeThreadLocal));
        size_t dummy = 0;
        const int rc = run_ops(m, L, s, n, &dummy, skip_tail);
        const hipError_t r = hipStreamEndCapture(s, &g);
        if (rc) { if (g) hipGraphDestroy(g); return 1; }
        if (r != hipSuccess) PA_FAIL(e, "hipStreamEndCapture: %s", hipGetErrorString(r));
        const hipError_t ri = hipGraphInstantiate(&ge, g, nullptr, nullptr, 0);
        hipGraphDestroy(g);
        if (ri != hipSuccess) PA_FAIL(e, "hipGraphInstantiate: %s", hipGetErrorString(ri));
        it = L.graphs.emplace(n, ge).first;
        L.graph_stem_path[n] = m->last_stem_path;
    }
    PA_HIP(e, hipGraphLaunch(it->second, s));
    m->last_stem_path = L.graph_stem_path[n];
    return 0;
}

int finish_profile(pa_model* m, size_t n_rec) {
    if (!m->e->profiling) { m->n_prof = 0; return 0; }
    for (size_t i = 0; i < n_rec && i < m->prof.size(); ++i)
        hipEventElapsedTime(&m->prof[i].ms, m->prof[i].e0, m->prof[i].e1);
    m->n_prof = n_rec;
    return 0;
}

int pa_model_plan_bytes(pa_model* m, size_t* arena_bytes, size_t* logical_bytes) {
    if (!m->planned) PA_FAIL(m->e, "pa_model_plan_bytes: no plan yet");
    if (arena_bytes) *arena_bytes = m->arena_bytes;
    if (logical_bytes) *logical_bytes = m->logical_bytes;
    return 0;
}

int pa_model_fill_arena(pa_model* m, int byte_value) {
    if (!m) return 1;
    pa_engine* e = m->e;
    if (!m->planned || !m->ln[0].arena) PA_FAIL(e, "pa_model_fill_arena: no plan yet");
    PA_HIP(e, hipSetDevice(e->dev));
    for (Lane& L : m->ln) {
        if (!L.allocated) continue;
        const hipStream_t s = L.stream ? L.stream : e->main_stream();
        PA_HIP(e, hipMemsetAsync(L.arena.get(), byte_value & 0xFF, m->arena_bytes, s));
        if (L.d_netin) PA_HIP(e, hipMemsetAsync(L.d_netin.get(), byte_value & 0xFF, (size_t)m->p_batch * m->net_h * m->net_w * 4, s));
        PA_HIP(e, hipStreamSynchronize(s));
    }
    return 0;
}

int pa_model_lanes_allocated(pa_model* m) {
    int n = 0;
    if (m) for (const Lane& L : m->ln) n += L.allocated ? 1 : 0;
    return n;
}

int pa_model_last_lane(pa_model* m) { return m ? m->last_lane : 0; }

int pa_model_last_stem_path(pa_model* m) { return m ? m->last_stem_path : 0; }

int pa_model_profile_text(pa_model* m, char* buf, size_t cap) {
    size_t off = 0;
    for (size_t i = 0; i < m->n_prof && i < m->prof.size(); ++i) {
        const ProfRec& r = m->prof[i];
        int n = snprintf(buf + off, off < cap ? cap - off : 0, "%d,%d,%d,%d,%d,%d,%d,%d,%.5f,%.0f,%d,%d,%s\n", r.kind, r.ksize, r.M, r.cout,
                         r.cin, r.stride, r.mf, r.nf, r.ms, r.flops, r.res, r.tile, r.family ? r.family : "");
        if (n < 0 || off + n >= cap) break;
        off += n;
    }
    if (off < cap) buf[off] = 0;
    return (int)off;
}

int pa_model_last_profile(pa_model* m, int cap, int32_t* kinds, float* ms, double* flops, int32_t* ksizes) {
    int n = 0;
    for (size_t i = 0; i < m->n_prof && i < m->prof.size() && n < cap; ++i, ++n) {
        kinds[n] = m->prof[i].kind; ms[n] = m->prof[i].ms; flops[n] = m->prof[i].flops; ksizes[n] = m->prof[i].ksize;
    }
    return n;
}
```

padel_analytics_amd/csrc/engine_internal.h:

```cpp
#pragma once
#include "../../include/padel_hip.h"
#include "graph_plan.h"
#include "launch_plan.h"
#include "lane_plan.h"
#include "device_mem.h"
#include "kernels.h"

#include <algorithm>
#include <cmath>
#include <cstdio>
#include <cstdlib>
#include <cstring>
#include <map>
#include <memory>
#include <string>
#include <vector>

using namespace padel;

struct pa_comm;
struct JpegScratch;
struct JpegDecScratch;

struct pa_engine {
    int dev = 0;
    hipStream_t main_stream() { ++main_seq_; return main_; }
    hipStream_t main_stream_wait_only() const { return main_; }
    hipError_t create_streams();
    void destroy_streams();
    hipError_t fork_lane(int i);
    hipError_t join_lane(hipEvent_t ev) { return hipStreamWaitEvent(main_, ev, 0); }
    hipError_t sync_lanes();
    hipStream_t lane_stream[kMaxLanes] = {nullptr, nullptr};
    hipStream_t copy_stream = nullptr;
    std::string err;
    bool profiling = false;
    DevMem<float> zeros;
    Tuning t;
    int tuning_epoch = 0;
    std::string timeline_path;
    pa_comm* comm = nullptr;
    DevMem<uint8_t> yuv_stage;
    int yuv_last_path = 0;
    hipEvent_t timer_ev[2]{};
    DevMem<uint8_t> render_stage;
    DevMem<uint8_t> activity_stage;
    DevMem<uint8_t> box_stage;
    int render_last_path = 0;
    JpegScratch* jpeg = nullptr;
    JpegDecScratch* jpeg_dec = nullptr;
    int jpeg_dec_last_path = 0;
    long long jpeg_dec_split_min = 0;
    int jpeg_dec_split_sub = 0;
    long long jpeg_dec_last_split[4] = {0, 0, 0, 0};
private:
    hipStream_t main_ = nullptr;
    unsigned long long main_seq_ = 1;
    unsigned long long forked_seq_[kMaxLanes] = {0, 0};
    hipEvent_t fork_ev_[kMaxLanes] = {nullptr, nullptr};
};

extern thread_local std::string g_err;

#define PA_FAIL(eng, ...)                                        \
    do {                                                         \
        char _b[512];                                            \
        snprintf(_b, sizeof(_b), __VA_ARGS__);                   \
        if (eng) (eng)->err = _b; else g_err = _b;               \
        return 1;                                                \
    } while (0)

#define PA_HIP(eng, call)                                                                  \
    do {                                                                                   \
        const hipError_t _e = static_cast<hipError_t>(call);    \
        if (_e != hipSuccess) {                                                            \
            (void)hipGetLastError();    \
            PA_FAIL(eng, "%s failed: %s (%s:%d)", #call, hipGetErrorString(_e), __FILE__, __LINE__); \
        }                                                                                  \
    } while (0)

struct ProfRec { int kind; int ksize; double flops; hipEvent_t e0, e1; float ms; int M, cout, cin, stride, mf, nf, res; int tile; const char* family; };
enum { PROF_PRE = 100, PROF_DECODE = 101, PROF_NMS = 102 };

struct ResamplePlan {
    int sh = 0, sw = 0, dh = 0, dw = 0;
    DevMem<int32_t> d_hb, d_hk, d_vb, d_vk;
    int hks = 0, vks = 0;
    DevMem<uint8_t> d_tmp;
};

struct Lane {
    bool allocated = false;
    hipStream_t stream = nullptr;
    DevMem<char> arena;
    std::vector<float*> bptr;
    DevMem<float> d_fc;
    DevMem<float> d_stage;
    DevMem<uint8_t> d_netin;
    HeadLevel lv[3]{};
    DevMem<float> d_cand; DevMem<int32_t> d_cidx, d_ccnt;
    DevMem<uint64_t> d_keys; DevMem<int32_t> d_order; DevMem<uint8_t> d_supp;
    DevMem<float> d_oboxes, d_okpts; DevMem<int32_t> d_ocnt;
    std::vector<Step> steps;
    std::map<int, hipGraphExec_t> graphs;
    std::map<int, int> graph_stem_path;
    DevMem<uint8_t> d_rs_tmp;
    LaneState st;
    size_t device_bytes() const {
        return arena.bytes() + d_fc.bytes() + d_stage.bytes() + d_netin.bytes() + d_cand.bytes() + d_cidx.bytes() + d_ccnt.bytes() + d_keys.bytes() +
               d_order.bytes() + d_supp.bytes() + d_oboxes.bytes() + d_okpts.bytes() + d_ocnt.bytes() + d_rs_tmp.bytes();
    }
};

struct pa_model {
    pa_engine* e = nullptr;
    pa_model_desc d{};
    std::vector<pa_buf_desc> bufs;
    std::vector<pa_op_desc> ops;
    std::vector<int> fold_src;
    std::vector<char> stem_fuse;
    HeadTail tail;
    DevMem<float> d_w;
    size_t n_w = 0;
    DevMem<char> d_wr;
    std::vector<long long> wr_off;
    bool wr_valid = false;
    DevMem<unsigned> d_ovf;
    int fc_nout = 0;
    int max_batch = 64;
    Lane ln[kMaxLanes];
    int last_lane = 0;
    bool lane1_refused = false;
    double conv_flops = 0;
    size_t lane_bytes = 0;

    bool planned = false;
    int p_h0 = 0, p_w0 = 0, p_imgsz = 0, p_pre = 0, p_auto = 0, p_batch = 0;
    int net_h = 0, net_w = 0;
    int rw = 0, rh = 0, top = 0, left = 0, lb_mode = 0;
    size_t arena_bytes = 0, logical_bytes = 0;
    unsigned h_ovf = 0;
    bool ovf_cached = false;
    PinMem<unsigned> h_pin;
    hipEvent_t tk_ev[PA_MAX_INFLIGHT]{};
    bool tk_busy[PA_MAX_INFLIGHT]{};
    int tk_lane[PA_MAX_INFLIGHT]{};
    int next_ticket = 0, n_inflight = 0;
    std::vector<int32_t> classes_host;
    int graph_epoch = -1;
    DevMem<uint8_t> d_frames;
    DevMem<int32_t> d_xtab, d_ytab;
    ResamplePlan rs;
    int A = 0, P2 = 0;
    YoloGeometry geom;
    DevMem<int32_t> d_classes;
    int last_n = 0;
    int last_post_path = 0;
    int last_stem_path = 0;
    bool heads_stale = false;
    std::vector<ProfRec> prof;
    size_t n_prof = 0;
};

inline bool guards_range(const pa_model* m) { return m->d.dtype == PA_DTYPE_H2 || m->d.dtype == PA_DTYPE_F16; }
ProfRec* prof_begin(pa_model* m, hipStream_t s, size_t idx, int kind, int ksize, double flops);
inline void prof_end(hipStream_t s, ProfRec* r) { if (r) hipEventRecord(r->e1, s); }
int finish_profile(pa_model* m, size_t n_rec);
void free_plan(pa_model* m);
int plan_buffers(pa_model* m, Lane& L, int batch, hipStream_t s);
void free_lane(Lane& L);
int run_graph(pa_model* m, Lane& L, hipStream_t s, int n, size_t* pi, bool skip_tail);
bool head_fused(const pa_model* m);
void head_tail_convs(const pa_model* m, const Lane& L, HeadTailArgs& a);
int run_tail_ops(pa_model* m, Lane& L, hipStream_t s, int n);

void jpeg_scratch_free(pa_engine* e);

void jpeg_dec_scratch_free(pa_engine* e);

hipError_t upload_table(pa_engine* e, DevMem<int32_t>& d, const std::vector<int32_t>& v);
int stage_frames(pa_model* m, const uint8_t** src, int nb, size_t frame_bytes, hipStream_t s);
int resample_plan(pa_engine* e, ResamplePlan* rs, int sh, int sw, int dh, int dw, int filter, int max_batch, bool identity_pass = false);
hipError_t resample_enqueue(const ResamplePlan& rs, const uint8_t* src, uint8_t* dst, int n, int out_c, int reverse, hipStream_t s, uint8_t* tmp = nullptr);
```

padel_analytics_amd/csrc/kernels.h:

```cpp
#pragma once
#include <hip/hip_runtime.h>
#include <stdint.h>

namespace padel {

enum Act : int { ACT_NONE = 0, ACT_SILU = 1, ACT_RELU = 2, ACT_SIGMOID = 3, ACT_LEAKY = 4 };

struct ConvArgs {
    const float* in;
    const float* w;
    const void* w3;
    const float* bias;
    const float* res;
    int res_pre;
    const float* zeros;
    const float* in2;
    int in2_cs, in2_choff, up_c;
    float* out;
    int in_cs, in_choff;
    int out_cs, out_choff;
    int res_cs, res_choff;
    int H, W;
    int Ho, Wo;
    int cin;
    int cout;
    int n16;
    int ksize, stride;
    int act;
    int M;
    int n_mtiles;
    int n_ntiles;
    int tune;
    int tap_pd;
    int out_f32;
    const float* oscale;
    unsigned* ovf_flag;
    unsigned* f16_flag;
    int w_single;
    const void* wr;
    unsigned long long* dbg;
    unsigned howo_magic, howo_shift, wo_magic, wo_shift;
};
inline void fill_fastdiv(unsigned d, unsigned* magic, unsigned* shift) {
    unsigned s = 0;
    while ((1ull << s) < d) ++s;
    *magic = (unsigned)((((1ull << 32) * ((1ull << s) - d)) / d) + 1ull);
    *shift = s;
}
constexpr int conv_dbg_words(int steps) { return 8 + 4 * steps * 5; }
constexpr int kConvDbgSteps = 64;
constexpr int kConvDbgWords = conv_dbg_words(kConvDbgSteps);
constexpr int kPatchDbgSteps = 32;
constexpr int kPatchDbgWords = conv_dbg_words(kPatchDbgSteps);

enum ConvPath : int { CONV_PATH_TAP = 0, CONV_PATH_BX3 = 1, CONV_PATH_H2 = 2, CONV_PATH_F16 = 3 };
bool conv_tile_shape(int path, int id, int* bm, int* bn);
struct ConvLaunched { int tile; const char* family; };
enum ConvFamily : int { CONV_TAP, CONV_BX3T, CONV_BX3P, CONV_H2T, CONV_H2D, CONV_H2S, CONV_H2S3, CONV_H2P, CONV_H2Q, CONV_H2R, CONV_H2W, CONV_H2V,
                        CONV_TAP16, CONV_TAP16D, CONV_P16, CONV_P16Q };
const char* conv_family_name(ConvFamily f);
bool resolve_conv(int path, const ConvArgs& a, int requested, ConvLaunched* out, ConvFamily* family = nullptr);
int conv_timeline_words(const ConvLaunched& k, int ksize);
hipError_t launch_conv_family(ConvFamily f, const ConvArgs& a, int tile, hipStream_t s);
constexpr size_t kConvReadSlack = 512;
int choose_conv_tap_variant(int M, int n16);
int choose_conv_bx3_variant(const ConvArgs& a);
int choose_conv_h2_variant(const ConvArgs& a);
int choose_conv_tap16_variant(const ConvArgs& a);
bool conv_wants_operand_copy(int ksize, int stride, int cin, bool w_single);
int h2_ksteps(int cin, int ksize);
size_t conv_h2r_copy_bytes(int n16, int cin, int ksize);

hipError_t launch_conv_tapt(const ConvArgs& a, int tile, hipStream_t s);
hipError_t launch_conv_bx3t(const ConvArgs& a, int tile, hipStream_t s);
hipError_t launch_conv_bx3p(const ConvArgs& a, int tile, hipStream_t s);
hipError_t launch_conv_h2t(const ConvArgs& a, int tile, hipStream_t s);
hipError_t launch_conv_h2d(const ConvArgs& a, int tile, hipStream_t s);
hipError_t launch_conv_h2s(const ConvArgs& a, int tile, hipStream_t s);
hipError_t launch_conv_h2s3(const ConvArgs& a, int tile, hipStream_t s);
hipError_t launch_conv_h2p(const ConvArgs& a, int tile, hipStream_t s);
hipError_t launch_conv_h2q(const ConvArgs& a, int tile, hipStream_t s);
hipError_t launch_conv_h2r(const ConvArgs& a, int tile, hipStream_t s);
hipError_t launch_conv_h2w(const ConvArgs& a, int tile, hipStream_t s);
hipError_t launch_conv_h2v(const ConvArgs& a, int tile, hipStream_t s);
hipError_t launch_conv_t16(const ConvArgs& a, int tile, hipStream_t s);
hipError_t launch_conv_p16(const ConvArgs& a, int tile, hipStream_t s);
hipError_t launch_h2r_repack(const float* w, void* wr, int n16, int cin, int ksize, hipStream_t s);
hipError_t launch_h2_mplane_check(const float* w, long long rows_x_ksteps, unsigned* flag, hipStream_t s);

struct StemArgs {
    const uint8_t* in;
    const float* w;
    const float* bias;
    float* out;
    int out_cs, out_choff;
    int H, W, Ho, Wo, cout, B;
    int out_f16;
    unsigned* ovf_flag;
    unsigned howo_magic, howo_shift, wo_magic, wo_shift;
    const void* opw;
};
hipError_t launch_stem(const StemArgs& a, hipStream_t s);
struct ConvArgs;
bool stem_l1_h2_supported(const StemArgs& st, const ConvArgs& cv);
bool stem_l1_cv1_h2_supported(const StemArgs& st, const ConvArgs& cv, const ConvArgs& cv1);
hipError_t launch_stem_l1_h2(const StemArgs& st, const ConvArgs& cv, const ConvArgs* cv1, hipStream_t s);
size_t stem_l1_operand_bytes(int cout);
hipError_t launch_stem_l1_operands(const float* w, int cout, void* blk, hipStream_t s);

hipError_t init_misc_kernels();
hipError_t launch_sppf_pool(float* buf, int cs, int choff, int c, int B, int H, int W, hipStream_t s, int f16 = 0, int fused = 1);
hipError_t launch_upsample2x(const float* in, int in_cs, int in_choff, float* out, int out_cs, int out_choff,
                             int c, int B, int H, int W, hipStream_t s, int f16 = 0);
hipError_t launch_h2_encode(const float* in, float* out, long long n_floats, unsigned* ovf_flag, hipStream_t s);
hipError_t launch_maxpool2(const float* in, int in_cs, int in_choff, float* out, int out_cs, int out_choff,
                           int c, int B, int H, int W, hipStream_t s, int f16 = 0);

struct Stem7Args {
    const uint8_t* in;
    const float* w;
    const float* bias;
    const float* lut;
    float* out;
    int out_cs, out_choff;
    int H, W, Ho, Wo, B;
    int act;
    int out_h2;
    unsigned* ovf_flag;
    unsigned howo_magic, howo_shift, wo_magic, wo_shift;
};
hipError_t launch_stem7(const Stem7Args& a, hipStream_t s);
hipError_t launch_maxpool3s2(const float* in, int in_cs, int in_choff, float* out, int out_cs, int out_choff,
                             int c, int B, int H, int W, int Ho, int Wo, hipStream_t s, int h2);
hipError_t launch_gap_fc(const float* in, int in_cs, int in_choff, int c, int B, int HW, const float* w, const float* bias, int nout,
                         float* logits, float* probs, hipStream_t s, int h2);
constexpr int kGapFcMaxC = 4096, kGapFcMaxOut = 64;

struct DwConvArgs {
    const float* in;
    const float* w;
    const float* bias;
    const float* res;
    float* out;
    int in_cs, in_choff, out_cs, out_choff, res_cs, res_choff;
    int C, B, H, W;
    int act;
    int h2, out_f32;
    unsigned* ovf_flag;
};
hipError_t launch_dwconv3(const DwConvArgs& a, hipStream_t s);
struct AttnArgs {
    const float* qkv;
    float* out;
    int cs, q_choff, k_choff, v_choff, out_cs, out_choff;
    int heads, kd, hd, N, B;
    float scale;
    int h2, out_f32;
    unsigned* ovf_flag;
};
hipError_t launch_psa_attn(const AttnArgs& a, hipStream_t s);

struct LetterboxArgs {
    const uint8_t* src;
    uint8_t* dst;
    int B, h0, w0;
    int rw, rh;
    int top, left;
    int nh, nw;
    int mode;
    int reverse;
    const int32_t* xtab;
    const int32_t* ytab;
};
hipError_t launch_letterbox(const LetterboxArgs& a, hipStream_t s);

struct YuvArgs {
    const uint8_t* src;
    uint8_t* dst;
    int n, h, w;
    int nv12;
    int pitch_y, pitch_c;
    int off_u, off_v;
    long long frame_stride;
    int y_off, cy, cvr, cug, cvg, cub;
};
bool yuv_vector_path_ok(const YuvArgs& a);
hipError_t launch_yuv420_to_bgr(const YuvArgs& a, hipStream_t s, int* vec_out = nullptr);

struct RenderArgs {
    const uint8_t* src;
    uint8_t* dst;
    const void* marks;
    const void* boxes;
    const int32_t* first;
    int n, h, w;
    int out;
    int in_place;
    int pitch_y, pitch_c, off_u, off_v;
    long long frame_stride;
    int y_off, yr, yg, yb, ur, ug, ub, vr, vg, vb;
#ifdef PADEL_RENDER_PROBE
    unsigned long long* probe;
#endif
};
bool render_vector_path_ok(const RenderArgs& a);
hipError_t launch_render(const RenderArgs& a, hipStream_t s, int* vec_out = nullptr);

struct ResamplePassArgs {
    const uint8_t* in; uint8_t* out;
    int B, in_h, in_w, in_c;
    int out_h, out_w, out_c;
    int vertical;
    const int32_t* bounds;
    const int32_t* coefs;
    int ksize;
    int reverse;
};
hipError_t launch_resample_pass(const ResamplePassArgs& a, hipStream_t s);

struct HeadLevel { const float* buf; int H, W, stride, anchor0; };
struct DecodeArgs {
    HeadLevel lv[3];
    int cs;
    int nc, nk, kdim;
    int A, B;
    float conf;
    const int32_t* classes; int n_classes;
    float* cand;
    int32_t* cand_idx;
    int32_t* cand_cnt;
};
hipError_t launch_decode(const DecodeArgs& a, hipStream_t s);

struct HeadTailConv {
    const float* in;
    const float* w;
    const float* bias;
    const float* oscale;
    int in_cs, in_choff, cin, n16;
};
struct HeadTailArgs {
    DecodeArgs d;
    HeadTailConv cv[3][3];
    int w_single;
    int wg_end[3];
};
bool head_tail_h2_supported(const HeadTailArgs& a);
hipError_t init_head_tail_kernels();
hipError_t launch_head_tail_h2(const HeadTailArgs& a, hipStream_t s);

struct NmsArgs {
    const float* cand; const int32_t* cand_idx; const int32_t* cand_cnt;
    uint64_t* keys;
    int32_t* order;
    uint8_t* supp;
    HeadLevel lv[3];
    int cs, nc, nk, kdim, A, B, P2;
    float iou; int max_det; int max_nms;
    float gain; float pad_x, pad_y;
    float kpad_x, kpad_y;
    float w0, h0;
    float* out_boxes;
    float* out_kpts;
    int32_t* out_cnt;
};
hipError_t launch_nms(const NmsArgs& a, hipStream_t s);

struct BallAssembleArgs {
    const uint8_t* median;
    const uint8_t* frames;
    const float* lut;
    float* out;
    int B, H, W, ring, first_slot;
    int out_f16;
};
hipError_t launch_ball_assemble(const BallAssembleArgs& a, hipStream_t s);

struct BallEnsembleArgs {
    const float* Y;
    int cs, H, W;
    const int32_t* row0;
    const int32_t* mode;
    const float* div;
    float w[8];
    float threshold;
    float* heat;
    uint8_t* mask;
};
hipError_t launch_ball_ensemble(const BallEnsembleArgs& a, int nout, hipStream_t s);

struct BallLocateArgs {
    const uint8_t* mask;
    int32_t* label;
    int32_t* bbox;
    int32_t* rect;
    int H, W;
};
hipError_t launch_ball_locate(const BallLocateArgs& a, int nout, hipStream_t s);
hipError_t launch_median(const uint8_t* frames, int N, long long frame_bytes, uint8_t* out_rgb, hipStream_t s, bool keep_bgr = false);

struct ActivityArgs {
    const uint8_t* frames;
    const uint8_t* ref;
    const uint8_t* prev;
    int n, h, w;
    int x0, y0, x1, y1;
    int tau;
    int band_rows, bands;
    uint32_t* slab;
    unsigned long long* out;
};
hipError_t launch_frame_activity(const ActivityArgs& a, hipStream_t s);

struct BoxHistArgs {
    const uint8_t* frames;
    const int32_t* rects;
    uint32_t* out;
    int h, w, k;
};
hipError_t launch_box_histograms(const BoxHistArgs& a, hipStream_t s);

}
```

padel_analytics_amd/csrc/launch_plan.cpp:

```cpp
#include "launch_plan.h"

#include <cmath>
#include <cstdarg>
#include <cstdio>

namespace padel {

int choose_conv_tile(int path, const ConvArgs& a) {
    return path == CONV_PATH_H2 ? choose_conv_h2_variant(a) : path == CONV_PATH_F16 ? choose_conv_tap16_variant(a)
           : path == CONV_PATH_BX3 ? choose_conv_bx3_variant(a) : choose_conv_tap_variant(a.M, a.n16);
}

ConvRequest request_conv(int path, ConvArgs& a, int forced, const ConvUp* up) {
    ConvRequest r{forced >= 0 ? forced : choose_conv_tile(path, a), false, ConvLaunched{-1, ""}, CONV_TAP};
    if (up) {
        a.in2 = up->in2; a.in2_cs = up->cs; a.in2_choff = up->choff; a.up_c = up->c;
        if ((r.resolved = resolve_conv(path, a, r.tile, &r.ran, &r.family))) return r;
        a.in2 = nullptr; a.in2_cs = a.in2_choff = a.up_c = 0;
    }
    r.resolved = resolve_conv(path, a, r.tile, &r.ran, &r.family);
    if (!r.resolved) r.ran = ConvLaunched{-1, ""};
    return r;
}

bool stem_l1_h2_supported(const StemArgs& st, const ConvArgs& a) {
    const int c = st.cout;
    return st.out_f16 == 2 && (c == 16 || c == 32 || c == 48) && a.ksize == 3 && a.stride == 2 && a.cin == c && a.n16 * 16 == 2 * c &&
           a.cout == 2 * c && a.H == st.Ho && a.W == st.Wo && a.Ho == (st.Ho + 1) / 2 && a.Wo == (st.Wo + 1) / 2 && a.w && a.oscale &&
           a.ovf_flag && !a.in2 && !a.res && (st.Ho & 1) == 0 && (st.Wo & 1) == 0;
}

bool stem_l1_cv1_h2_supported(const StemArgs& st, const ConvArgs& a, const ConvArgs& b) {
    return stem_l1_h2_supported(st, a) && a.w_single && a.wr && st.opw && (st.W & 3) == 0 && !(a.tune & 8) &&
           a.act == ACT_SILU && !a.out_f32 && a.out &&
           b.ksize == 1 && b.stride == 1 && b.cin == a.cout && b.cout == a.cout && b.n16 * 16 == b.cout && b.H == a.Ho && b.W == a.Wo &&
           b.Ho == a.Ho && b.Wo == a.Wo && b.M == a.M && b.in == a.out && b.in_cs == a.out_cs && b.in_choff == a.out_choff &&
           b.w_single && b.wr && b.w && b.bias && b.oscale && b.out && b.ovf_flag && !b.in2 && !b.res;
}

size_t stem_l1_operand_bytes(int cout) { return (size_t)(cout / 16) * 2048 + (size_t)cout * sizeof(float); }

size_t operand_copy_offsets(const pa_model_desc& d, const std::vector<char>& stem_fuse, std::vector<long long>& off) {
    off.assign(d.n_ops, -1);
    size_t total = 0;
    for (int i = 0; i < d.n_ops; ++i) {
        const pa_op_desc& o = d.ops[i];
        if (o.kind == PA_OP_STEM && stem_fuse[i] && (o.cout == 16 || o.cout == 32 || o.cout == 48)) {
            off[i] = (long long)total;
            total += (stem_l1_operand_bytes(o.cout) + 2047) / 2048 * 2048;
            continue;
        }
        const bool stem_cv1 = i >= 2 && stem_fuse[i - 2] == 2;
        if (o.kind != PA_OP_CONV || !(stem_cv1 || conv_wants_operand_copy(o.ksize, o.stride, o.cin, (o.flags & PA_CONV_W_SINGLE) != 0))) continue;
        off[i] = (long long)total;
        total += conv_h2r_copy_bytes(o.npad / 16, o.cin, o.ksize);
    }
    return total;
}

namespace {

struct Builder {
    const pa_model_desc& d;
    const std::vector<int>& fold_src;
    const Tuning& t;
    const PlanPointers& p;
    int net_h, net_w, n;

    const void* operand_copy(int i) const { return (p.wr_off && p.wr_off[i] >= 0) ? (const void*)(p.wr + p.wr_off[i]) : nullptr; }

    bool conv(int i, Step& st) const {
        const pa_op_desc& o = d.ops[i];
        const pa_buf_desc& ob = d.bufs[o.out_buf];
        const pa_buf_desc& ib = d.bufs[o.in_buf];
        const int Ho = net_h >> ob.level, Wo = net_w >> ob.level;
        ConvArgs& a = st.conv;
        a = ConvArgs{};
        a.in = p.bptr[o.in_buf]; a.in_cs = ib.channels; a.in_choff = o.in_choff;
        a.out = p.bptr[o.out_buf]; a.out_cs = ob.channels; a.out_choff = o.out_choff;
        a.res = o.res_buf >= 0 ? p.bptr[o.res_buf] : nullptr;
        a.res_cs = o.res_buf >= 0 ? d.bufs[o.res_buf].channels : 0; a.res_choff = o.res_choff;
        a.res_pre = (o.res_buf >= 0 && (o.flags & PA_CONV_RES_PREACT)) ? 1 : 0;
        a.zeros = p.zeros;
        a.w = p.blob + o.w_off; a.bias = p.blob + o.b_off;
        a.H = net_h >> ib.level; a.W = net_w >> ib.level; a.Ho = Ho; a.Wo = Wo;
        a.cin = o.cin; a.cout = o.cout; a.n16 = o.npad / 16; a.ksize = o.ksize; a.stride = o.stride; a.act = o.act;
        a.M = n * Ho * Wo;
        fill_fastdiv((unsigned)(Ho * Wo), &a.howo_magic, &a.howo_shift);
        fill_fastdiv((unsigned)Wo, &a.wo_magic, &a.wo_shift);
        a.tune = t.tune; a.tap_pd = t.tap_pd;
        const bool f16 = d.dtype == PA_DTYPE_F16, h2 = d.dtype == PA_DTYPE_H2;
        const bool use_bx3 = !f16 && !h2 && t.impl == 2 && o.reserved > 0;
        a.w3 = use_bx3 ? (const void*)(p.blob + o.reserved) : nullptr;
        a.out_f32 = (f16 || h2) && is_head_buf(d, o.out_buf);
        st.path = h2 ? CONV_PATH_H2 : f16 ? CONV_PATH_F16 : use_bx3 ? CONV_PATH_BX3 : CONV_PATH_TAP;
        if (h2) {
            a.oscale = p.blob + o.reserved;
            a.ovf_flag = p.ovf;
            a.w_single = (o.flags & PA_CONV_W_SINGLE) && t.w_single ? 1 : 0;
            a.wr = operand_copy(i);
        }
        if (f16) a.f16_flag = p.ovf;
        ConvUp up{};
        const bool fold = (h2 || use_bx3) && t.fold_up && fold_src[i] >= 0;
        if (fold) {
            const pa_op_desc& u = d.ops[fold_src[i]];
            up = ConvUp{p.bptr[u.in_buf], d.bufs[u.in_buf].channels, u.in_choff, u.cin};
        }
        const ConvRequest r = request_conv(st.path, a, t.variant, fold ? &up : nullptr);
        st.requested = r.tile; st.ran = r.ran; st.family = r.family;
        return r.resolved;
    }

    void stem(int i, StemArgs& a) const {
        const pa_op_desc& o = d.ops[i];
        const pa_buf_desc& ob = d.bufs[o.out_buf];
        a = StemArgs{};
        a.in = p.netin; a.w = p.blob + o.w_off; a.bias = p.blob + o.b_off;
        a.out = p.bptr[o.out_buf]; a.out_cs = ob.channels; a.out_choff = o.out_choff;
        a.H = net_h; a.W = net_w; a.Ho = net_h >> ob.level; a.Wo = net_w >> ob.level; a.cout = o.cout; a.B = n;
        a.out_f16 = d.dtype == PA_DTYPE_F16 ? 1 : d.dtype == PA_DTYPE_H2 ? 2 : 0;
        a.ovf_flag = p.ovf;
        a.opw = operand_copy(i);
    }
};

int refuse(std::vector<Step>& out, std::string& err, const char* fmt, ...) {
    char b[512];
    va_list ap;
    va_start(ap, fmt);
    vsnprintf(b, sizeof(b), fmt, ap);
    va_end(ap);
    err = b;
    out.clear();
    return 1;
}

}

int build_steps(const pa_model_desc& d, const std::vector<int>& fold_src, const std::vector<char>& stem_fuse,
                const HeadTail& tail, const Tuning& t, const PlanPointers& p, int net_h, int net_w, int n, std::vector<Step>& out,
                std::string& err, const char* not_supported) {
    const Builder b{d, fold_src, t, p, net_h, net_w, n};
    const bool h2 = d.dtype == PA_DTYPE_H2;
    out.clear();
    int cv1_op = -1;
    for (int i = 0; i < d.n_ops; ++i) {
        const pa_op_desc& o = d.ops[i];
        const pa_buf_desc& ob = d.bufs[o.out_buf];
        const int Ho = net_h >> ob.level, Wo = net_w >> ob.level;
        Step st{};
        st.op = i; st.n_ops = 1; st.kind = o.kind; st.ran = ConvLaunched{-1, ""};
        st.stem_cv1 = i == cv1_op;
        for (int l = 0; l < 3 && tail.found; ++l)
            for (int c = 0; c < 3; ++c) st.tail = st.tail || tail.op[l][c] == i;
        if (o.kind == PA_OP_CONV) {
            const bool resolved = b.conv(i, st);
            const ConvArgs& a = st.conv;
            if (a.res_pre && st.path != CONV_PATH_H2 && st.path != CONV_PATH_BX3)
                return refuse(out, err, "op %d: PA_CONV_RES_PREACT needs the h2 or the bf16x3 kernels (tuning impl = 2, bf16x3 weights in the blob), not the %s family",
                              i, st.path == CONV_PATH_F16 ? "fp16" : "fp32-MFMA tap");
            if (!resolved) return refuse(out, err, "op %d (kind %d) launch failed: %s", i, o.kind, not_supported);
            if (a.in2)
                for (size_t k = out.size(); k-- > 0;)
                    if (out[k].op == fold_src[i]) { out.erase(out.begin() + (long)k); break; }
            conv_tile_shape(st.path, st.requested, &st.mf, &st.nf);
            st.ksize = o.ksize; st.flops = 2.0 * a.M * (double)o.cout * o.cin * o.ksize * o.ksize;
            st.M = a.M; st.cout = o.cout; st.cin = o.cin; st.stride = o.stride; st.res = a.res != nullptr;
        } else if (o.kind == PA_OP_STEM) {
            b.stem(i, st.stem);
            st.ksize = 3; st.flops = 2.0 * n * Ho * Wo * (double)o.cout * 27;
            if (t.fuse_stem && h2 && stem_fuse[i]) {
                b.conv(i + 1, st);
                if (stem_l1_h2_supported(st.stem, st.conv)) {
                    st.n_ops = 2;
                    if (t.fuse_stem_cv1 && stem_fuse[i] == 2) {
                        Step c1{};
                        if (b.conv(i + 2, c1) && stem_l1_cv1_h2_supported(st.stem, st.conv, c1.conv)) { st.cv1 = c1.conv; st.has_cv1 = true; cv1_op = i + 2; }
                    }
                    ++i;
                } else {
                    st.conv = ConvArgs{};
                }
                st.path = st.requested = 0; st.family = CONV_TAP; st.ran = ConvLaunched{-1, ""};
            }
        } else if (o.kind == PA_OP_SPPF_POOL) {
            st.sl = SliceArgs{p.bptr[o.in_buf], d.bufs[o.in_buf].channels, o.in_choff, nullptr, 0, 0, o.cin, n, Ho, Wo, 0, 0, (int)d.dtype, t.fuse_sppf,
                              nullptr, nullptr, 0, nullptr, nullptr};
            st.ksize = 5;
        } else if (o.kind == PA_OP_UPSAMPLE2X) {
            st.sl = SliceArgs{p.bptr[o.in_buf], d.bufs[o.in_buf].channels, o.in_choff, p.bptr[o.out_buf], ob.channels, o.out_choff, o.cin, n, Ho / 2, Wo / 2,
                              0, 0, (int)d.dtype, 0, nullptr, nullptr, 0, nullptr, nullptr};
        } else if (o.kind == PA_OP_MAXPOOL2) {
            st.sl = SliceArgs{p.bptr[o.in_buf], d.bufs[o.in_buf].channels, o.in_choff, p.bptr[o.out_buf], ob.channels, o.out_choff, o.cin, n, Ho * 2, Wo * 2,
                              0, 0, (int)d.dtype, 0, nullptr, nullptr, 0, nullptr, nullptr};
            st.ksize = 2;
        } else if (o.kind == PA_OP_MAXPOOL3S2) {
            const int lin = d.bufs[o.in_buf].level;
            st.sl = SliceArgs{p.bptr[o.in_buf], d.bufs[o.in_buf].channels, o.in_choff, p.bptr[o.out_buf], ob.channels, o.out_choff, o.cin, n,
                              net_h >> lin, net_w >> lin, Ho, Wo, h2 ? 1 : 0, 0, nullptr, nullptr, 0, nullptr, nullptr};
            st.ksize = 3;
        } else if (o.kind == PA_OP_STEM7) {
            if (!p.netin) return refuse(out, err, "op %d: the 7x7 stem reads the u8 network input of pa_resnet_infer", i);
            Stem7Args& a = st.stem7;
            a = Stem7Args{};
            a.in = p.netin; a.w = p.blob + o.w_off; a.bias = p.blob + o.b_off; a.lut = p.blob + o.reserved;
            a.out = p.bptr[o.out_buf]; a.out_cs = ob.channels; a.out_choff = o.out_choff;
            a.H = net_h; a.W = net_w; a.Ho = Ho; a.Wo = Wo; a.B = n; a.act = o.act;
            a.out_h2 = (h2 && !is_head_buf(d, o.out_buf)) ? 1 : 0;
            a.ovf_flag = p.ovf;
            st.ksize = 7; st.flops = 2.0 * n * Ho * Wo * 64.0 * 147.0;
            st.M = n * Ho * Wo; st.cout = 64; st.cin = 3; st.stride = 2;
        } else if (o.kind == PA_OP_GAP_FC) {
            const int lin = d.bufs[o.in_buf].level;
            st.sl = SliceArgs{p.bptr[o.in_buf], d.bufs[o.in_buf].channels, o.in_choff, nullptr, 0, 0, o.cin, n, (net_h >> lin) * (net_w >> lin), 0, 0, 0,
                              h2 ? 1 : 0, 0, p.blob + o.w_off, p.blob + o.b_off, o.cout, p.fc, p.fc + (size_t)p.p_batch * kGapFcMaxOut};
            st.flops = 2.0 * n * (double)o.cout * o.cin;
            st.M = n; st.cout = o.cout; st.cin = o.cin;
        } else if (o.kind == PA_OP_DWCONV3) {
            DwConvArgs& a = st.dw;
            a = DwConvArgs{};
            a.in = p.bptr[o.in_buf]; a.in_cs = d.bufs[o.in_buf].channels; a.in_choff = o.in_choff;
            a.w = p.blob + o.w_off; a.bias = p.blob + o.b_off;
            a.out = p.bptr[o.out_buf]; a.out_cs = ob.channels; a.out_choff = o.out_choff;
            if (o.res_buf >= 0) { a.res = p.bptr[o.res_buf]; a.res_cs = d.bufs[o.res_buf].channels; a.res_choff = o.res_choff; }
            a.C = o.cin; a.B = n; a.H = Ho; a.W = Wo; a.act = o.act;
            a.h2 = h2 ? 1 : 0; a.out_f32 = (h2 && is_head_buf(d, o.out_buf)) ? 1 : 0; a.ovf_flag = p.ovf;
            st.ksize = 3; st.flops = 2.0 * n * Ho * Wo * (double)o.cin * 9.0;
            st.M = n * Ho * Wo; st.cout = o.cout; st.cin = o.cin; st.stride = 1; st.res = o.res_buf >= 0;
        } else if (o.kind == PA_OP_PSA_ATTN) {
            AttnArgs& a = st.attn;
            a = AttnArgs{};
            a.heads = o.stride; a.kd = o.ksize; a.hd = o.npad;
            a.qkv = p.bptr[o.in_buf]; a.cs = d.bufs[o.in_buf].channels;
            a.q_choff = o.in_choff; a.k_choff = o.in_choff + a.heads * a.kd; a.v_choff = o.in_choff + 2 * a.heads * a.kd;
            a.out = p.bptr[o.out_buf]; a.out_cs = ob.channels; a.out_choff = o.out_choff;
            a.N = Ho * Wo; a.B = n; a.scale = (float)(1.0 / std::sqrt((double)a.kd));
            a.h2 = h2 ? 1 : 0; a.out_f32 = (h2 && is_head_buf(d, o.out_buf)) ? 1 : 0; a.ovf_flag = p.ovf;
            st.flops = 2.0 * n * (double)a.heads * a.N * (double)a.N * (a.kd + a.hd);
            st.M = n * a.N; st.cout = o.cout; st.cin = o.cin; st.stride = a.heads;
        }
        out.push_back(st);
    }
    return 0;
}

}
```

padel_analytics_amd/csrc/launch_plan.h:

```cpp
#pragma once
#include "graph_plan.h"
#include "kernels.h"

#include <string>
#include <vector>

namespace padel {

struct Tuning {
    int impl = 2;
    int variant = -1;
    int tune = 1;
    int tap_pd = 2;
    int graph = 0;
    int timeline = 0;
    int alias = 1;
    int fuse_stem = 1;
    int fuse_stem_cv1 = 1;
    int w_single = 1;
    int fuse_sppf = 1;
    int fuse_head = 1;
    int lanes = 2;
    int fold_up = 1;
};

int choose_conv_tile(int path, const ConvArgs& a);
struct ConvUp { const float* in2; int cs, choff, c; };
struct ConvRequest {
    int tile;
    bool resolved;
    ConvLaunched ran;
    ConvFamily family;
};
ConvRequest request_conv(int path, ConvArgs& a, int forced, const ConvUp* up);

size_t stem_l1_operand_bytes(int cout);
size_t operand_copy_offsets(const pa_model_desc& d, const std::vector<char>& stem_fuse, std::vector<long long>& off);

struct PlanPointers {
    float* const* bptr;
    const float* blob;
    const char* wr;
    const long long* wr_off;
    const float* zeros;
    unsigned* ovf;
    const uint8_t* netin;
    float* fc;
    int p_batch;
};

struct SliceArgs {
    float* in; int in_cs, in_choff;
    float* out; int out_cs, out_choff;
    int c, B, H, W, Ho, Wo;
    int fmt;
    int fused;
    const float* w; const float* bias; int nout; float* logits; float* probs;
};

struct Step {
    int op, n_ops;
    int kind;
    bool tail;
    ConvArgs conv;
    bool has_cv1, stem_cv1;
    ConvArgs cv1;
    int path;
    int requested;
    ConvFamily family;
    ConvLaunched ran;
    union {
        StemArgs stem;
        Stem7Args stem7;
        DwConvArgs dw;
        AttnArgs attn;
        SliceArgs sl;
    };
    int ksize; double flops; int M, cout, cin, stride, mf, nf, res;
};

int build_steps(const pa_model_desc& d, const std::vector<int>& fold_src, const std::vector<char>& stem_fuse,
                const HeadTail& tail, const Tuning& t, const PlanPointers& p, int net_h, int net_w, int n, std::vector<Step>& out,
                std::string& err, const char* not_supported = "operation not supported");

}
```

padel_analytics_amd/engine.py:

```python
from __future__ import annotations

import ctypes as C
import sys as _sys
import os
from pathlib import Path
from typing import Optional, Sequence

import numpy as np

from . import graph as G

_LIB_PATH = Path(os.environ["PADEL_LIB"]).resolve() if os.environ.get("PADEL_LIB") else Path(__file__).resolve().parent / "libpadel_hip.so"
_lib = None


class EngineUnavailable(RuntimeError):
    pass


class EngineError(RuntimeError):
    pass


class RangeOverflow(EngineError):
    """An activation of an h2 model (fp16 pairs, |x| <= 65504) did not fit: the results of that call are invalid and
    the caller repeats it on the full-range fp32 (bf16x3) model (yolo.py / trackers/ball_tracker.py do)."""


def fp32_mode() -> str:
    m = os.environ.get("PADEL_FP32_MODE", "h2").lower()
    if m not in ("h2", "bx3"):
        raise ValueError(f"PADEL_FP32_MODE={m!r}: expected 'h2' or 'bx3'")
    return m


class pa_buf_desc(C.Structure):
    _fields_ = [("level", C.c_int32), ("channels", C.c_int32)]


class pa_op_desc(C.Structure):
    _fields_ = [("kind", C.c_int32), ("in_buf", C.c_int32), ("in_choff", C.c_int32), ("cin", C.c_int32),
                ("out_buf", C.c_int32), ("out_choff", C.c_int32), ("cout", C.c_int32),
                ("ksize", C.c_int32), ("stride", C.c_int32), ("act", C.c_int32),
                ("res_buf", C.c_int32), ("res_choff", C.c_int32), ("npad", C.c_int32), ("reserved", C.c_int32),
                ("w_off", C.c_int64), ("b_off", C.c_int64), ("flags", C.c_int32), ("pad_", C.c_int32)]


class pa_model_desc(C.Structure):
    _fields_ = [("task", C.c_int32), ("nc", C.c_int32), ("nk", C.c_int32), ("kpt_dim", C.c_int32),
                ("n_bufs", C.c_int32), ("bufs", C.POINTER(pa_buf_desc)),
                ("n_ops", C.c_int32), ("ops", C.POINTER(pa_op_desc)),
                ("head_buf", C.c_int32 * 3), ("in_channels", C.c_int32), ("dtype", C.c_int32)]


class pa_yolo_params(C.Structure):
    _fields_ = [("imgsz", C.c_int32), ("pre_mode", C.c_int32), ("channel_reverse", C.c_int32),
                ("letterbox_auto", C.c_int32), ("conf", C.c_float), ("iou", C.c_float),
                ("max_det", C.c_int32), ("n_classes", C.c_int32), ("classes", C.POINTER(C.c_int32)),
                ("frames_on_device", C.c_int32)]


class pa_yuv_desc(C.Structure):
    _fields_ = [("layout", C.c_int32), ("pitch_y", C.c_int32), ("pitch_c", C.c_int32), ("off_u", C.c_int32),
                ("off_v", C.c_int32), ("reserved", C.c_int32), ("frame_stride", C.c_int64),
                ("y_off", C.c_int32), ("cy", C.c_int32), ("cvr", C.c_int32), ("cug", C.c_int32), ("cvg", C.c_int32),
                ("cub", C.c_int32)]


class pa_mark(C.Structure):
    _fields_ = [("kind", C.c_int32), ("x0", C.c_int32), ("y0", C.c_int32), ("x1", C.c_int32), ("y1", C.c_int32),
                ("size", C.c_int32), ("bgr", C.c_uint32), ("arg", C.c_int32)]


class pa_yuv_enc(C.Structure):
    _fields_ = [("y_off", C.c_int32), ("yr", C.c_int32), ("yg", C.c_int32), ("yb", C.c_int32), ("ur", C.c_int32), ("ug", C.c_int32),
                ("ub", C.c_int32), ("vr", C.c_int32), ("vg", C.c_int32), ("vb", C.c_int32)]


MARK_DTYPE = np.dtype([("kind", "<i4"), ("x0", "<i4"), ("y0", "<i4"), ("x1", "<i4"), ("y1", "<i4"), ("size", "<i4"), ("bgr", "<u4"),
                       ("arg", "<i4")])
MARK_DISC, MARK_SEGMENT, MARK_FILL, MARK_BOX, MARK_GLYPH, MARK_BLEND = 1, 2, 3, 4, 5, 6
RENDER_BGR, RENDER_YUV420 = 0, 1
RENDER_PATH_VECTOR, RENDER_PATH_BYTE = 1, 2

PRE_LETTERBOX, PRE_PIL_STRETCH = 0, 1
YUV_NV12, YUV_I420 = 0, 1
POST_PATH_DECODE, POST_PATH_FUSED = 0, 1
YUV_PATH_VECTOR, YUV_PATH_BYTE = 1, 2

ABI_SYMBOLS = [
    "pa_abi_version", "pa_device_count", "pa_engine_create", "pa_engine_destroy", "pa_last_error",
    "pa_engine_synchronize", "pa_device_malloc", "pa_device_free", "pa_memcpy_h2d", "pa_memcpy_d2h",
    "pa_model_create", "pa_model_destroy", "pa_model_set_max_batch", "pa_yolo_infer", "pa_yolo_head_shape",
    "pa_yolo_read_head", "pa_tracknet_infer", "pa_engine_set_profiling", "pa_model_last_profile",
    "pa_model_profile_text", "pa_ball_create", "pa_ball_destroy", "pa_ball_set_background", "pa_ball_feed",
    "pa_ball_locate", "pa_ball_background_from_frames",
    "pa_upload", "pa_engine_set_tuning", "pa_engine_set_timeline_path", "pa_model_plan_bytes",
    "pa_yolo_netin_shape", "pa_yolo_read_netin",
    "pa_comm_unique_id", "pa_engine_comm_init", "pa_engine_comm_destroy", "pa_engine_bcast_weights",
    "pa_engine_bcast", "pa_engine_allreduce_max", "pa_engine_gather_sizes", "pa_engine_gather",
    "pa_bytetrack_create", "pa_bytetrack_destroy", "pa_bytetrack_reset", "pa_bytetrack_update_batch",
    "pa_model_take_overflow", "pa_yolo_postprocess", "pa_host_register", "pa_host_unregister",
    "pa_engine_bcast_weights_from", "pa_model_fill_arena", "pa_yolo_submit", "pa_yolo_wait",
    "pa_resnet_infer", "pa_resnet_read_netin", "pa_resnet_read_fc", "pa_resnet_read_head", "pa_pil_coeffs",
    "pa_yuv420_to_bgr", "pa_yuv_last_path", "pa_engine_timer_start", "pa_engine_timer_stop",
    "pa_render", "pa_render_check", "pa_render_last_path", "pa_glyph_rows", "pa_ball_read_resized",
    "pa_jpeg_encode", "pa_jpeg_check", "pa_jpeg_interval_bytes",
    "pa_jpeg_parse", "pa_jpeg_decode", "pa_jpeg_decode_last_path", "pa_jpeg_decode_last_times",
    "pa_yolo_last_post_path", "pa_jpeg_decode_set_split", "pa_jpeg_decode_last_split",
    "pa_model_lanes_allocated", "pa_model_last_lane", "pa_model_last_stem_path", "pa_yolo_resample_passes", "pa_device_bytes_live",
    "pa_frame_activity", "pa_frame_activity_check", "pa_frames_median",
    "pa_box_histograms", "pa_box_histograms_check",
]


def lib_path() -> Path:
    return _LIB_PATH


def load_library():
    global _lib
    if _lib is not None:
        return _lib
    if not _LIB_PATH.exists():
        raise EngineUnavailable(f"{_LIB_PATH} not built — run `python -c 'import __graft_entry__ as g; g.build()'`")
    if os.environ.get("PADEL_HIP_STANDALONE") != "1":
        import torch
    lib = C.CDLL(str(_LIB_PATH))
    vp, i32, sz = C.c_void_p, C.c_int, C.c_size_t
    lib.pa_abi_version.restype = i32
    lib.pa_device_count.restype = i32
    lib.pa_engine_create.argtypes = [i32, C.POINTER(vp)]
    lib.pa_engine_destroy.argtypes = [vp]
    lib.pa_engine_destroy.restype = None
    lib.pa_last_error.argtypes = [vp]
    lib.pa_last_error.restype = C.c_char_p
    lib.pa_engine_synchronize.argtypes = [vp]
    lib.pa_device_malloc.argtypes = [vp, sz, C.POINTER(vp)]
    lib.pa_device_free.argtypes = [vp, vp]
    lib.pa_device_bytes_live.argtypes = []
    lib.pa_device_bytes_live.restype = sz
    lib.pa_memcpy_h2d.argtypes = [vp, vp, vp, sz]
    lib.pa_memcpy_d2h.argtypes = [vp, vp, vp, sz]
    lib.pa_model_create.argtypes = [vp, C.POINTER(pa_model_desc), vp, sz, C.POINTER(vp)]
    lib.pa_model_destroy.argtypes = [vp]
    lib.pa_model_destroy.restype = None
    lib.pa_model_set_max_batch.argtypes = [vp, i32]
    lib.pa_yolo_infer.argtypes = [vp, vp, i32, i32, i32, C.POINTER(pa_yolo_params), vp, vp, vp]
    lib.pa_yolo_submit.argtypes = [vp, vp, i32, i32, i32, C.POINTER(pa_yolo_params), vp, vp, vp, C.POINTER(C.c_int)]
    lib.pa_yolo_wait.argtypes = [vp, i32, C.POINTER(C.c_int)]
    lib.pa_yolo_head_shape.argtypes = [vp, i32, C.POINTER(i32), C.POINTER(i32), C.POINTER(i32)]
    lib.pa_yolo_read_head.argtypes = [vp, i32, i32, vp]
    lib.pa_yolo_last_post_path.argtypes = [vp]
    lib.pa_model_lanes_allocated.argtypes = [vp]
    lib.pa_model_last_lane.argtypes = [vp]
    lib.pa_model_last_stem_path.argtypes = [vp]
    lib.pa_yolo_resample_passes.argtypes = [vp]
    lib.pa_tracknet_infer.argtypes = [vp, vp, i32, i32, i32, i32, vp, i32]
    lib.pa_resnet_infer.argtypes = [vp, vp, i32, i32, i32, i32, vp, vp]
    lib.pa_resnet_read_netin.argtypes = [vp, i32, vp]
    lib.pa_resnet_read_fc.argtypes = [vp, i32, vp, vp]
    lib.pa_resnet_read_head.argtypes = [vp, i32, vp]
    lib.pa_pil_coeffs.argtypes = [i32, i32, i32, vp, vp, i32, C.POINTER(i32)]
    lib.pa_engine_set_profiling.argtypes = [vp, i32]
    lib.pa_model_last_profile.argtypes = [vp, i32, vp, vp, vp, vp]
    lib.pa_model_profile_text.argtypes = [vp, C.c_char_p, sz]
    lib.pa_ball_create.argtypes = [vp, i32, i32, C.POINTER(vp)]
    lib.pa_ball_destroy.argtypes = [vp]
    lib.pa_ball_destroy.restype = None
    lib.pa_ball_set_background.argtypes = [vp, vp]
    lib.pa_ball_feed.argtypes = [vp, vp, i32, i32, i32, vp, vp, vp, C.POINTER(i32)]
    lib.pa_ball_locate.argtypes = [vp, vp, i32, vp]
    lib.pa_ball_background_from_frames.argtypes = [vp, vp, i32, i32, vp]
    lib.pa_ball_read_resized.argtypes = [vp, C.c_longlong, vp]
    lib.pa_upload.argtypes = [vp, vp, vp, sz]
    lib.pa_engine_set_tuning.argtypes = [vp, C.c_char_p, i32]
    lib.pa_engine_set_timeline_path.argtypes = [vp, C.c_char_p]
    lib.pa_model_plan_bytes.argtypes = [vp, C.POINTER(sz), C.POINTER(sz)]
    lib.pa_yolo_netin_shape.argtypes = [vp, C.POINTER(i32), C.POINTER(i32)]
    lib.pa_yolo_read_netin.argtypes = [vp, i32, vp]
    lib.pa_comm_unique_id.argtypes = [vp, sz]
    lib.pa_engine_comm_init.argtypes = [vp, vp, sz, i32, i32]
    lib.pa_engine_comm_destroy.argtypes = [vp]
    lib.pa_engine_comm_destroy.restype = None
    lib.pa_engine_bcast_weights.argtypes = [vp, vp, i32]
    lib.pa_engine_bcast.argtypes = [vp, vp, sz, i32]
    lib.pa_engine_bcast_weights_from.argtypes = [vp, vp, vp, i32]
    lib.pa_engine_allreduce_max.argtypes = [vp, C.POINTER(C.c_double)]
    lib.pa_engine_gather_sizes.argtypes = [vp, sz, C.POINTER(C.c_uint64)]
    lib.pa_engine_gather.argtypes = [vp, vp, sz, vp, sz, C.POINTER(C.c_uint64), i32]
    lib.pa_bytetrack_create.argtypes = [C.c_double, i32, C.c_double, i32, C.POINTER(vp)]
    lib.pa_bytetrack_destroy.argtypes = [vp]
    lib.pa_bytetrack_destroy.restype = None
    lib.pa_bytetrack_reset.argtypes = [vp]
    lib.pa_bytetrack_reset.restype = None
    lib.pa_bytetrack_update_batch.argtypes = [vp, vp, vp, vp, i32, i32, vp]
    lib.pa_model_fill_arena.argtypes = [vp, i32]
    lib.pa_host_register.argtypes = [vp, vp, sz]
    lib.pa_host_unregister.argtypes = [vp, vp]
    lib.pa_model_take_overflow.argtypes = [vp, C.POINTER(i32)]
    lib.pa_yolo_postprocess.argtypes = [vp, C.POINTER(vp), i32, i32, i32, C.POINTER(pa_yolo_params), vp, vp, vp]
    lib.pa_yuv420_to_bgr.argtypes = [vp, vp, i32, i32, i32, i32, C.POINTER(pa_yuv_desc), vp]
    lib.pa_yuv_last_path.argtypes = [vp]
    lib.pa_render.argtypes = [vp, vp, i32, i32, i32, vp, vp, i32, C.POINTER(pa_yuv_desc), C.POINTER(pa_yuv_enc), vp]
    lib.pa_render_check.argtypes = [i32, i32, i32, vp, vp, i32, C.POINTER(pa_yuv_desc), C.POINTER(pa_yuv_enc), C.c_char_p, sz]
    lib.pa_render_last_path.argtypes = [vp]
    lib.pa_glyph_rows.argtypes = [i32, vp]
    lib.pa_jpeg_encode.argtypes = [vp, vp, i32, i32, i32, C.POINTER(pa_yuv_desc), i32, vp, sz, vp]
    lib.pa_jpeg_check.argtypes = [i32, i32, i32, C.POINTER(pa_yuv_desc), i32, C.c_char_p, sz]
    lib.pa_jpeg_interval_bytes.argtypes = [i32]
    lib.pa_jpeg_interval_bytes.restype = sz
    lib.pa_jpeg_parse.argtypes = [vp, sz, C.POINTER(pa_jpeg_frame_info), vp, sz, C.c_char_p, sz]
    lib.pa_jpeg_decode.argtypes = [vp, vp, vp, i32, i32, i32, vp, vp]
    lib.pa_jpeg_decode_last_path.argtypes = [vp]
    lib.pa_jpeg_decode_last_times.argtypes = [vp, vp]
    lib.pa_jpeg_decode_set_split.argtypes = [vp, C.c_int64, i32]
    lib.pa_jpeg_decode_last_split.argtypes = [vp, vp]
    lib.pa_frame_activity_check.argtypes = [i32, i32, i32, vp, i32]
    lib.pa_frame_activity_check.restype = C.c_char_p
    lib.pa_frame_activity.argtypes = [vp, vp, i32, i32, i32, vp, vp, vp, i32, vp]
    lib.pa_frames_median.argtypes = [vp, vp, i32, i32, i32, vp]
    lib.pa_box_histograms_check.argtypes = [i32, i32, i32, vp, i32]
    lib.pa_box_histograms_check.restype = C.c_char_p
    lib.pa_box_histograms.argtypes = [vp, vp, i32, i32, i32, vp, i32, vp]
    lib.pa_engine_timer_start.argtypes = [vp]
    lib.pa_engine_timer_stop.argtypes = [vp, C.POINTER(C.c_float)]
    if lib.pa_abi_version() != 5:
        raise EngineUnavailable("libpadel_hip.so ABI version mismatch")
    _lib = lib
    return lib


def device_bytes_live() -> int:
    return int(load_library().pa_device_bytes_live())


PIL_BICUBIC, PIL_BILINEAR = 0, 1


def pil_coeffs(in_size: int, out_size: int, filter: int = PIL_BICUBIC):
    lib = load_library()
    ks = C.c_int(0)
    if lib.pa_pil_coeffs(in_size, out_size, filter, None, None, 0, C.byref(ks)) != 0:
        raise EngineError("pa_pil_coeffs: bad arguments")
    bounds = np.zeros((out_size, 2), np.int32)
    coefs = np.zeros((out_size, ks.value), np.int32)
    if lib.pa_pil_coeffs(in_size, out_size, filter, bounds.ctypes.data, coefs.ctypes.data, coefs.size, C.byref(ks)) != 0:
        raise EngineError("pa_pil_coeffs failed")
    return bounds, coefs


def graph_dtype(mode: Optional[str] = None) -> str:
    return {"h2": "h2", "bx3": "f32"}[mode or fp32_mode()]


def yuv_span_bytes(n: int, h: int, w: int, d: "pa_yuv_desc") -> Optional[int]:
    if n < 1 or h < 2 or w < 2 or h % 2 or w % 2 or d.layout not in (YUV_NV12, YUV_I420):
        return None
    crow = w if d.layout == YUV_NV12 else w // 2
    if d.pitch_y < w or d.pitch_c < crow or d.off_u < 0 or d.off_v < 0:
        return None
    c_len = (h // 2 - 1) * d.pitch_c + crow
    extent = max((h - 1) * d.pitch_y + w, d.off_u + c_len, 0 if d.layout == YUV_NV12 else d.off_v + c_len)
    if d.frame_stride < extent:
        return None
    return (n - 1) * d.frame_stride + extent


def glyph_rows(code) -> Optional[np.ndarray]:
    rows = np.zeros(7, np.uint8)
    code = ord(code) if isinstance(code, str) else int(code)
    return rows if load_library().pa_glyph_rows(code, rows.ctypes.data) == 0 else None


def _render_args(marks, first, geom, enc):
    marks = np.ascontiguousarray(marks, MARK_DTYPE).reshape(-1)
    first = np.ascontiguousarray(first, np.int32).reshape(-1)
    if geom is not None and not isinstance(geom, pa_yuv_desc):
        geom = pa_yuv_desc(**{k: int(v) for k, v in geom.items()})
    if enc is not None and not isinstance(enc, pa_yuv_enc):
        enc = pa_yuv_enc(*(int(c) for c in enc))
    return marks, first, geom, enc


def render_check(n: int, h: int, w: int, marks, first, out: int = RENDER_BGR, geom=None, enc=None) -> Optional[str]:
    marks, first, geom, enc = _render_args(marks, first, geom, enc)
    if first.size != max(int(n), 0) + 1:
        return f"pa_render: first has {first.size} entries, n + 1 = {int(n) + 1} are needed"
    if marks.size < int(first[-1]):
        return f"pa_render: first[] announces {int(first[-1])} marks, marks holds {marks.size}"
    why = C.create_string_buffer(512)
    rc = load_library().pa_render_check(int(n), int(h), int(w), marks.ctypes.data if marks.size else None, first.ctypes.data, int(out),
                                        C.byref(geom) if geom is not None else None, C.byref(enc) if enc is not None else None, why, 512)
    return why.value.decode() if rc else None


ACTIVITY_MAX_SIDE, ACTIVITY_MAX_FRAMES = 16384, 65535


def _roi_arg(roi):
    if roi is None:
        return None
    roi = np.ascontiguousarray(roi, np.int32).reshape(-1)
    if roi.size != 4:
        raise ValueError(f"roi must be (x0, y0, x1, y1), got {roi.size} numbers")
    return roi


def frame_activity_check(n: int, h: int, w: int, roi=None, tau: int = 24) -> Optional[str]:
    roi = _roi_arg(roi)
    why = load_library().pa_frame_activity_check(int(n), int(h), int(w), roi.ctypes.data if roi is not None else None, int(tau))
    return why.decode() if why else None


BOX_HIST_BINS, BOX_HIST_MAX_RECTS = 512, 16384


def _rects_arg(rects) -> np.ndarray:
    rects = np.ascontiguousarray(rects, np.int32)
    if rects.size == 0:
        return rects.reshape(0, 5)
    if rects.ndim != 2 or rects.shape[1] != 5:
        raise ValueError(f"rects must be (k, 5): frame, x0, y0, x1, y1; got shape {rects.shape}")
    return rects


def box_histograms_check(n: int, h: int, w: int, rects) -> Optional[str]:
    if rects is None:
        ptr, k = None, 1
    else:
        rects = _rects_arg(rects)
        ptr, k = (rects.ctypes.data if len(rects) else None), len(rects)
    why = load_library().pa_box_histograms_check(int(n), int(h), int(w), ptr, int(k))
    return why.decode() if why else None


JPEG_MAX_WIDTH = 2560


def _yuv_desc_arg(desc):
    return desc if desc is None or isinstance(desc, pa_yuv_desc) else pa_yuv_desc(**{k: int(v) for k, v in desc.items()})


def jpeg_check(n: int, h: int, w: int, desc, quality: int = 90) -> Optional[str]:
    desc = _yuv_desc_arg(desc)
    why = C.create_string_buffer(512)
    rc = load_library().pa_jpeg_check(int(n), int(h), int(w), C.byref(desc) if desc is not None else None, int(quality), why, 512)
    return why.value.decode() if rc else None


def jpeg_interval_bytes(w: int) -> int:
    return int(load_library().pa_jpeg_interval_bytes(int(w)))


JPEG_DEC_MAX_DIM = 4096
JPEG_DEC_PATH_VECTOR, JPEG_DEC_PATH_BYTE = 1, 2
JPEG_DEC_SPLIT_MIN_BYTES, JPEG_DEC_SPLIT_SUB_BYTES = 7168, 128


class pa_jpeg_huff(C.Structure):
    _fields_ = [("bits", C.c_uint8 * 16), ("vals", C.c_uint8 * 256), ("nvals", C.c_int32)]


class pa_jpeg_interval(C.Structure):
    _fields_ = [("begin", C.c_int64), ("end", C.c_int64), ("first_mcu", C.c_int32), ("mcus", C.c_int32)]


class pa_jpeg_frame_info(C.Structure):
    _fields_ = [("w", C.c_int32), ("h", C.c_int32), ("mcus_x", C.c_int32), ("mcus_y", C.c_int32), ("restart_interval", C.c_int32),
                ("n_intervals", C.c_int32), ("default_huffman", C.c_int32), ("status", C.c_int32), ("scan_begin", C.c_int64),
                ("scan_end", C.c_int64), ("quant", (C.c_uint8 * 64) * 3), ("comp_dc", C.c_uint8 * 3), ("comp_ac", C.c_uint8 * 3),
                ("pad_", C.c_uint8 * 2), ("dc", pa_jpeg_huff * 2), ("ac", pa_jpeg_huff * 2)]


def jpeg_parse(jpeg) -> dict:
    raw = np.frombuffer(bytes(jpeg), np.uint8)
    info, why = pa_jpeg_frame_info(), C.create_string_buffer(512)
    lib = load_library()
    if lib.pa_jpeg_parse(raw.ctypes.data, raw.size, C.byref(info), None, 0, why, 512):
        raise ValueError(why.value.decode())
    ivls = (pa_jpeg_interval * max(info.n_intervals, 1))()
    if lib.pa_jpeg_parse(raw.ctypes.data, raw.size, C.byref(info), ivls, info.n_intervals, why, 512):
        raise ValueError(why.value.decode())
    table = lambda t: (list(t.bits), list(t.vals)[:t.nvals])
    return dict(w=info.w, h=info.h, mcus_x=info.mcus_x, mcus_y=info.mcus_y, restart_interval=info.restart_interval,
                n_intervals=info.n_intervals, default_huffman=info.default_huffman, status=info.status, scan_begin=info.scan_begin,
                scan_end=info.scan_end, quant=np.array([list(q) for q in info.quant], np.uint8), comp_dc=list(info.comp_dc),
                comp_ac=list(info.comp_ac), dc=[table(t) for t in info.dc], ac=[table(t) for t in info.ac],
                intervals=[(v.begin, v.end, v.first_mcu, v.mcus) for v in ivls[:info.n_intervals]])


class DeviceBuffer:

    def __init__(self, engine: "Engine", nbytes: int, _ptr: Optional[int] = None):
        self.engine, self.nbytes = engine, nbytes
        self.owner = _ptr is None
        if _ptr is None:
            p = C.c_void_p()
            engine._check(engine.lib.pa_device_malloc(engine.handle, nbytes, C.byref(p)))
            _ptr = p.value
        self.ptr = _ptr

    def view(self, offset: int, nbytes: int) -> "DeviceBuffer":
        assert 0 <= offset and offset + nbytes <= self.nbytes
        return DeviceBuffer(self.engine, nbytes, _ptr=self.ptr + offset)

    def upload(self, arr: np.ndarray, copy_stream: bool = False) -> "DeviceBuffer":
        arr = np.ascontiguousarray(arr)
        assert arr.nbytes <= self.nbytes
        f = self.engine.lib.pa_upload if copy_stream else self.engine.lib.pa_memcpy_h2d
        self.engine._check(f(self.engine.handle, self.ptr, arr.ctypes.data, arr.nbytes))
        return self

    def download(self, arr: np.ndarray) -> np.ndarray:
        assert arr.flags.c_contiguous and arr.nbytes <= self.nbytes
        self.engine._check(self.engine.lib.pa_memcpy_d2h(self.engine.handle, arr.ctypes.data, self.ptr, arr.nbytes))
        return arr

    def free(self):
        if self.ptr and self.owner:
            self.engine.lib.pa_device_free(self.engine.handle, self.ptr)
        self.ptr = None


class Engine:

    def __init__(self, device_id: int = 0):
        self.lib = load_library()
        if self.lib.pa_device_count() <= 0:
            raise EngineUnavailable("no HIP device visible: the padel_analytics_amd engine needs an AMD GPU (gfx950)")
        h = C.c_void_p()
        if self.lib.pa_engine_create(device_id, C.byref(h)) != 0:
            raise EngineUnavailable(self.lib.pa_last_error(None).decode())
        self.handle = h
        self.device_id = device_id

    def _check(self, rc: int):
        if rc != 0:
            raise EngineError(self.lib.pa_last_error(self.handle).decode())

    def synchronize(self):
        self._check(self.lib.pa_engine_synchronize(self.handle))

    def set_profiling(self, on: bool):
        self._check(self.lib.pa_engine_set_profiling(self.handle, 1 if on else 0))
        self.profiling = bool(on)

    def alloc(self, nbytes: int) -> DeviceBuffer:
        return DeviceBuffer(self, nbytes)

    def pin(self, arr: np.ndarray) -> None:
        assert arr.flags.c_contiguous
        self._check(self.lib.pa_host_register(self.handle, arr.ctypes.data, arr.nbytes))

    def unpin(self, arr: np.ndarray) -> None:
        self._check(self.lib.pa_host_unregister(self.handle, arr.ctypes.data))

    def yuv420_to_bgr(self, src, n: int, h: int, w: int, desc, dst: DeviceBuffer) -> None:
        if not isinstance(desc, pa_yuv_desc):
            desc = pa_yuv_desc(**{k: int(v) for k, v in desc.items()})
        on_dev = isinstance(src, DeviceBuffer)
        if on_dev:
            ptr, have = src.ptr, src.nbytes
        else:
            if not (isinstance(src, np.ndarray) and src.dtype == np.uint8 and src.ndim == 1 and src.flags.c_contiguous):
                raise TypeError("yuv420_to_bgr: src must be a contiguous 1-D uint8 array of raw bytes or a DeviceBuffer")
            ptr, have = src.ctypes.data, src.nbytes
        need = yuv_span_bytes(n, h, w, desc)
        if need is not None and have < need:
            raise EngineError(f"yuv420_to_bgr: {n} frames as described span {need} bytes, src holds {have}")
        if n >= 1 and h >= 1 and w >= 1 and dst.nbytes < n * h * w * 3:
            raise EngineError(f"yuv420_to_bgr: dst holds {dst.nbytes} bytes, {n} BGR frames need {n * h * w * 3}")
        self._check(self.lib.pa_yuv420_to_bgr(self.handle, ptr, int(on_dev), int(n), int(h), int(w), C.byref(desc), dst.ptr))

    def yuv_last_path(self) -> int:
        return int(self.lib.pa_yuv_last_path(self.handle))

    def render(self, src: DeviceBuffer, n: int, h: int, w: int, marks, first, dst: DeviceBuffer, out: int = RENDER_BGR, geom=None,
               enc=None) -> None:
        marks, first, geom, enc = _render_args(marks, first, geom, enc)
        if first.size != max(int(n), 0) + 1:
            raise EngineError(f"render: first has {first.size} entries, n + 1 = {int(n) + 1} are needed")
        if marks.size < int(first[-1]):
            raise EngineError(f"render: first[] announces {int(first[-1])} marks, marks holds {marks.size}")
        if n >= 1 and h >= 1 and w >= 1 and src.nbytes < n * h * w * 3:
            raise EngineError(f"render: src holds {src.nbytes} bytes, {n} BGR frames need {n * h * w * 3}")
        if out == RENDER_YUV420 and geom is not None:
            need = yuv_span_bytes(n, h, w, geom)
        else:
            need = n * h * w * 3 if (n >= 1 and h >= 1 and w >= 1) else None
        if need is not None and dst.nbytes < need:
            raise EngineError(f"render: {n} frames as described span {need} bytes, dst holds {dst.nbytes}")
        self._check(self.lib.pa_render(self.handle, src.ptr, int(n), int(h), int(w), marks.ctypes.data if marks.size else None,
                                       first.ctypes.data, int(out), C.byref(geom) if geom is not None else None,
                                       C.byref(enc) if enc is not None else None, dst.ptr))

    def render_last_path(self) -> int:
        return int(self.lib.pa_render_last_path(self.handle))

    def frame_activity(self, src: DeviceBuffer, n: int, h: int, w: int, ref: DeviceBuffer, prev: Optional[DeviceBuffer] = None, roi=None,
                       tau: int = 24, out: Optional[np.ndarray] = None) -> np.ndarray:
        roi = _roi_arg(roi)
        why = frame_activity_check(n, h, w, roi, tau)
        if why is not None:
            raise EngineError(why)
        fb = h * w * 3
        if src.nbytes < n * fb:
            raise EngineError(f"frame_activity: src holds {src.nbytes} bytes, {n} BGR frames need {n * fb}")
        for name, buf in (("ref", ref), ("prev", prev)):
            if buf is not None and buf.nbytes < fb:
                raise EngineError(f"frame_activity: {name} holds {buf.nbytes} bytes, one BGR frame needs {fb}")
        if out is None:
            out = np.zeros((n, 3), np.uint64)
        elif not (isinstance(out, np.ndarray) and out.dtype == np.uint64 and out.flags.c_contiguous and out.ndim == 2
                  and out.shape[1] == 3 and out.shape[0] >= n):
            raise EngineError("frame_activity: out must be a C-contiguous uint64 array of at least n rows of 3")
        self._check(self.lib.pa_frame_activity(self.handle, src.ptr, int(n), int(h), int(w), ref.ptr, prev.ptr if prev is not None else None,
                                               roi.ctypes.data if roi is not None else None, int(tau), out.ctypes.data))
        return out

    def box_histograms(self, src: DeviceBuffer, n: int, h: int, w: int, rects, out: Optional[np.ndarray] = None) -> np.ndarray:
        if rects is None:
            raise EngineError(box_histograms_check(n, h, w, None))
        rects = _rects_arg(rects)
        k = len(rects)
        why = box_histograms_check(n, h, w, rects)
        if why is not None:
            raise EngineError(why)
        if src.nbytes < n * h * w * 3:
            raise EngineError(f"box_histograms: src holds {src.nbytes} bytes, {n} BGR frames need {n * h * w * 3}")
        if out is None:
            out = np.zeros((k, BOX_HIST_BINS), np.uint32)
        elif not (isinstance(out, np.ndarray) and out.dtype == np.uint32 and out.flags.c_contiguous and out.ndim == 2
                  and out.shape[1] == BOX_HIST_BINS and out.shape[0] >= k):
            raise EngineError("box_histograms: out must be a C-contiguous uint32 array of at least k rows of 512")
        self._check(self.lib.pa_box_histograms(self.handle, src.ptr, int(n), int(h), int(w), rects.ctypes.data if k else None, int(k),
                                               out.ctypes.data))
        return out

    def frames_median(self, src: DeviceBuffer, n: int, h: int, w: int, out: Optional[DeviceBuffer] = None) -> DeviceBuffer:
        fb = h * w * 3
        if n >= 1 and h >= 1 and w >= 1 and src.nbytes < n * fb:
            raise EngineError(f"frames_median: src holds {src.nbytes} bytes, {n} BGR frames need {n * fb}")
        own = out is None
        if own:
            out = self.alloc(max(fb, 1))
        elif out.nbytes < fb:
            raise EngineError(f"frames_median: out holds {out.nbytes} bytes, one BGR frame needs {fb}")
        try:
            self._check(self.lib.pa_frames_median(self.handle, src.ptr, int(n), int(h), int(w), out.ptr))
        except EngineError:
            if own:
                out.free()
            raise
        return out

    def jpeg_encode(self, buffer: DeviceBuffer, n: int, h: int, w: int, desc, quality: int = 90, out: Optional[np.ndarray] = None):
        desc = _yuv_desc_arg(desc)
        need = yuv_span_bytes(n, h, w, desc)
        if need is not None and buffer.nbytes < need:
            raise EngineError(f"jpeg_encode: {n} frames as described span {need} bytes, the buffer holds {buffer.nbytes}")
        offsets = np.zeros(max(int(n), 0) + 1, np.int64)
        own = out is None
        if own:
            out = np.empty(max(int(n), 1) * (max(int(h), 1) * max(int(w), 1) // 4 + 4096), np.uint8)
        elif not (isinstance(out, np.ndarray) and out.dtype == np.uint8 and out.ndim == 1 and out.flags.c_contiguous):
            raise TypeError("jpeg_encode: out must be a contiguous 1-D uint8 array")
        for attempt in (0, 1):
            rc = self.lib.pa_jpeg_encode(self.handle, buffer.ptr, int(n), int(h), int(w), C.byref(desc), int(quality), out.ctypes.data,
                                         out.size, offsets.ctypes.data)
            if rc == 0:
                return out[:int(offsets[-1])], offsets
            needed = int(offsets[-1])
            if needed <= out.size or not own or attempt:
                err = EngineError(self.lib.pa_last_error(self.handle).decode())
                err.needed = needed if needed > out.size else None
                raise err
            out = np.empty(needed, np.uint8)

    def jpeg_decode(self, data, offsets, dst: DeviceBuffer, h: Optional[int] = None, w: Optional[int] = None) -> np.ndarray:
        data = np.frombuffer(data, np.uint8) if isinstance(data, (bytes, bytearray)) else data
        if not (isinstance(data, np.ndarray) and data.dtype == np.uint8 and data.ndim == 1 and data.flags.c_contiguous):
            raise TypeError("jpeg_decode: data must be bytes or a contiguous 1-D uint8 array")
        offsets = np.ascontiguousarray(offsets, np.int64)
        n = offsets.size - 1
        if n < 1 or offsets[0] < 0 or np.any(np.diff(offsets) < 0) or offsets[-1] > data.size:
            raise EngineError(f"jpeg_decode: offsets must be n + 1 >= 2 ascending positions inside the {data.size} bytes of data")
        if h is None or w is None:
            try:
                info = jpeg_parse(data[int(offsets[0]):int(offsets[1])].tobytes())
            except ValueError as e:
                raise EngineError(f"jpeg_decode: frame 0: {e}") from None
            h, w = info["h"], info["w"]
        h, w = int(h), int(w)
        if dst.nbytes < n * h * w * 3:
            raise EngineError(f"jpeg_decode: dst holds {dst.nbytes} bytes, {n} BGR frames of {w} x {h} need {n * h * w * 3}")
        status = np.zeros(n, np.int32)
        self._check(self.lib.pa_jpeg_decode(self.handle, data.ctypes.data, offsets.ctypes.data, n, h, w, dst.ptr, status.ctypes.data))
        return status

    def jpeg_decode_last_path(self) -> int:
        return int(self.lib.pa_jpeg_decode_last_path(self.handle))

    def jpeg_decode_last_times(self) -> dict:
        ms = (C.c_double * 5)()
        self._check(self.lib.pa_jpeg_decode_last_times(self.handle, ms))
        return dict(zip(("parse", "upload", "entropy", "idct", "colour"), (float(v) for v in ms)))

    def jpeg_decode_set_split(self, min_bytes: int = 0, sub_bytes: int = 0) -> None:
        self._check(self.lib.pa_jpeg_decode_set_split(self.handle, int(min_bytes), int(sub_bytes)))

    def jpeg_decode_last_split(self) -> dict:
        out = (C.c_int64 * 4)()
        self._check(self.lib.pa_jpeg_decode_last_split(self.handle, out))
        return dict(zip(("split", "subsequences", "rounds", "serial"), (int(v) for v in out)))

    def timer_start(self) -> None:
        self._check(self.lib.pa_engine_timer_start(self.handle))

    def timer_stop(self) -> float:
        ms = C.c_float(0.0)
        self._check(self.lib.pa_engine_timer_stop(self.handle, C.byref(ms)))
        return float(ms.value)

    def set_tuning(self, **kv):
        for k, v in kv.items():
            self._check(self.lib.pa_engine_set_tuning(self.handle, k.encode(), int(v)))
            if k == "timeline":
                self.timeline = bool(v)

    def comm_init(self, unique_id: bytes, nranks: int, rank: int):
        buf = C.create_string_buffer(bytes(unique_id), len(unique_id))
        self._check(self.lib.pa_engine_comm_init(self.handle, buf, len(unique_id), nranks, rank))
        self.nranks, self.rank = nranks, rank
        if nranks > 1:
            from . import dist as _dist
            _dist.use_engine_comm(self)

    def bcast_weights(self, model: "Model", root: int = 0):
        self._check(self.lib.pa_engine_bcast_weights(self.handle, model.handle, root))

    def bcast_weights_from(self, src: Optional["Model"], dst: "Model", root: int = 0):
        self._check(self.lib.pa_engine_bcast_weights_from(self.handle, src.handle if src is not None else None, dst.handle, root))

    def bcast(self, buf: DeviceBuffer, nbytes: int, root: int = 0):
        self._check(self.lib.pa_engine_bcast(self.handle, buf.ptr, nbytes, root))

    def gather_bytes(self, buf: np.ndarray, root: int = 0):
        buf = np.ascontiguousarray(buf, np.uint8).reshape(-1)
        n = max(getattr(self, "nranks", 1), 1)
        me = getattr(self, "rank", 0)
        sizes = (C.c_uint64 * n)()
        self._check(self.lib.pa_engine_gather_sizes(self.handle, int(buf.size), sizes))
        total = int(sum(sizes))
        recv = np.empty(max(total, 1), np.uint8) if me == root else None
        self._check(self.lib.pa_engine_gather(self.handle, buf.ctypes.data if buf.size else None, int(buf.size),
                                              recv.ctypes.data if recv is not None else None, total if recv is not None else 0, sizes, root))
        if me != root:
            return None
        out, off = [], 0
        for k in range(n):
            out.append(recv[off:off + int(sizes[k])])
            off += int(sizes[k])
        return out

    def allreduce_max(self, value: float) -> float:
        v = C.c_double(value)
        self._check(self.lib.pa_engine_allreduce_max(self.handle, C.byref(v)))
        return v.value

    def close(self):
        if self.handle:
            from . import dist as _dist
            if _dist._comm_engine is self:
                _dist.use_engine_comm(None)
            self.lib.pa_engine_destroy(self.handle)
            self.handle = None


_default_engines: dict = {}


def comm_unique_id() -> bytes:
    lib = load_library()
    buf = C.create_string_buffer(128)
    if lib.pa_comm_unique_id(buf, 128) != 0:
        raise EngineError(lib.pa_last_error(None).decode())
    return buf.raw


def default_engine(device_id: Optional[int] = None) -> Engine:
    if device_id is None:
        device_id = int(os.environ.get("LOCAL_RANK", "0")) if os.environ.get("PADEL_DEVICE") is None \
            else int(os.environ["PADEL_DEVICE"])
        load_library()
        n = _lib.pa_device_count()
        if n > 0:
            device_id %= n
    if device_id not in _default_engines:
        _default_engines[device_id] = Engine(device_id)
    return _default_engines[device_id]


_PAGE = 4096


def _round_up(x: int, a: int) -> int:
    return (int(x) + a - 1) // a * a


def _frames_arg(frames, n: Optional[int], h: int, w: int):
    if isinstance(frames, DeviceBuffer):
        assert n is not None and frames.nbytes >= n * h * w * 3
        return frames, frames.ptr, n, True
    frames = np.ascontiguousarray(frames, np.uint8)
    n = len(frames) if n is None else n
    assert frames.shape == (n, h, w, 3), frames.shape
    return frames, frames.ctypes.data, n, False


def _yolo_params(classes: Optional[Sequence[int]], **fields):
    cls_arr = (C.c_int32 * len(classes))(*[int(c) for c in classes]) if classes is not None and len(classes) else None
    return pa_yolo_params(n_classes=0 if cls_arr is None else len(cls_arr), classes=cls_arr, **fields), cls_arr


class _PinnedBlock:

    def __init__(self, engine, nbytes: int):
        import mmap
        size = _round_up(max(int(nbytes), 1), _PAGE)
        self._mm = mmap.mmap(-1, size, flags=mmap.MAP_PRIVATE | mmap.MAP_ANONYMOUS, prot=mmap.PROT_READ | mmap.PROT_WRITE)
        self.block = np.frombuffer(self._mm, np.uint8)
        self.engine = engine
        engine.pin(self.block)
        self._pinned = True

    def release(self) -> None:
        if self._pinned:
            self._pinned = False
            try:
                self.engine.unpin(self.block)
            except Exception as exc:
                if _sys is not None and getattr(_sys, "meta_path", None) is not None and getattr(self.engine, "handle", None):
                    print(f"padel_analytics_amd: hipHostUnregister of a result block failed ({exc}); pages left registered", file=_sys.stderr)

    def __del__(self):
        self.release()


class Model:

    def __init__(self, engine: Engine, graph: G.Graph, blob: Optional[np.ndarray] = None, *, empty: bool = False):
        self.engine, self.graph = engine, graph
        if not empty:
            blob = graph.blob() if blob is None else np.ascontiguousarray(blob, np.float32)
        bufs = (pa_buf_desc * len(graph.bufs))(*[pa_buf_desc(l, c) for l, c in graph.bufs])
        ops = (pa_op_desc * len(graph.ops))()
        for i, o in enumerate(graph.ops):
            for k, v in o.items():
                setattr(ops[i], k, int(v))
        d = pa_model_desc(task=graph.task, nc=graph.nc, nk=graph.nk, kpt_dim=graph.kpt_dim, n_bufs=len(graph.bufs),
                          bufs=bufs, n_ops=len(graph.ops), ops=ops, in_channels=graph.in_channels,
                          dtype=graph.dtype)
        for i in range(3):
            d.head_buf[i] = graph.head_buf[i] if i < len(graph.head_buf) else -1
        h = C.c_void_p()
        engine._check(engine.lib.pa_model_create(engine.handle, C.byref(d), None if empty else blob.ctypes.data,
                                                 graph.n_floats if empty else blob.size, C.byref(h)))
        self.handle = h
        self.max_batch = 64
        self._out_ring: dict = {}

    MAX_INFLIGHT = 4
    OUT_RING = MAX_INFLIGHT + 2

    def _ring_outputs(self, n: int, max_det: int):
        key = (int(n), int(max_det))
        ring = self._out_ring.get(key)
        if ring is None:
            nk = self.graph.nk
            sizes = [n * max_det * 6 * 4, n * max_det * nk * 4, n * 4]
            offs = [0, _round_up(sizes[0], 64), 0]
            offs[2] = offs[1] + _round_up(sizes[1], 64)
            sets = []
            for _ in range(self.OUT_RING):
                pb = _PinnedBlock(self.engine, offs[2] + sizes[2])
                block = pb.block
                boxes = block[offs[0]:offs[0] + sizes[0]].view(np.float32).reshape(n, max_det, 6)
                kpts = block[offs[1]:offs[1] + sizes[1]].view(np.float32).reshape(n, max_det, nk) if nk else None
                counts = block[offs[2]:offs[2] + sizes[2]].view(np.int32).reshape(n)
                sets.append((boxes, kpts, counts, pb))
            ring = self._out_ring[key] = [sets, 0]
        sets, i = ring
        ring[1] = (i + 1) % self.OUT_RING
        return sets[i][:3]

    def _fresh_outputs(self, n: int, max_det: int):
        nk = self.graph.nk
        return (np.zeros((n, max_det, 6), np.float32), np.zeros((n, max_det, nk), np.float32) if nk else None,
                np.zeros((n,), np.int32))

    def _free_rings(self):
        for sets, _ in self._out_ring.values():
            for arrs in sets:
                arrs[3].release()
        self._out_ring = {}

    def __del__(self):
        try:
            if self._out_ring and getattr(self, "handle", None) and self.engine.handle:
                self.engine.synchronize()
        except Exception:
            pass
        try:
            self._free_rings()
        except Exception:
            pass

    def set_max_batch(self, n: int):
        self.engine._check(self.engine.lib.pa_model_set_max_batch(self.handle, int(n)))
        self.max_batch = int(n)

    def yolo_infer(self, frames, n: int, h: int, w: int, *, imgsz: int, conf: float, iou: float,
                   classes: Optional[Sequence[int]] = None, max_det: int = 300, pre_mode: int = PRE_LETTERBOX,
                   channel_reverse: bool = False, letterbox_auto: bool = True, reuse_outputs: bool = False):
        frames, ptr, n, on_dev = _frames_arg(frames, n, h, w)
        p, cls_arr = _yolo_params(classes, imgsz=imgsz, pre_mode=pre_mode, channel_reverse=int(channel_reverse),
                                  letterbox_auto=int(letterbox_auto), conf=conf, iou=iou, max_det=max_det,
                                  frames_on_device=int(on_dev))
        boxes, kpts, counts = self._ring_outputs(n, max_det) if reuse_outputs else self._fresh_outputs(n, max_det)
        self.engine._check(self.engine.lib.pa_yolo_infer(
            self.handle, ptr, n, h, w, C.byref(p), boxes.ctypes.data,
            kpts.ctypes.data if kpts is not None else None, counts.ctypes.data))
        return boxes, kpts, counts

    def yolo_submit(self, frames: "DeviceBuffer", n: int, h: int, w: int, *, imgsz: int, conf: float, iou: float,
                    classes: Optional[Sequence[int]] = None, max_det: int = 300, pre_mode: int = PRE_LETTERBOX,
                    channel_reverse: bool = False, letterbox_auto: bool = True):
        assert isinstance(frames, DeviceBuffer) and frames.nbytes >= n * h * w * 3
        p, cls_arr = _yolo_params(classes, imgsz=imgsz, pre_mode=pre_mode, channel_reverse=int(channel_reverse),
                                  letterbox_auto=int(letterbox_auto), conf=conf, iou=iou, max_det=max_det, frames_on_device=1)
        boxes, kpts, counts = self._ring_outputs(n, max_det)
        t = C.c_int(-1)
        self.engine._check(self.engine.lib.pa_yolo_submit(
            self.handle, frames.ptr, n, h, w, C.byref(p), boxes.ctypes.data,
            kpts.ctypes.data if kpts is not None else None, counts.ctypes.data, C.byref(t)))
        return (t.value, boxes, kpts, counts)

    def yolo_wait(self, ticket):
        t, boxes, kpts, counts = ticket
        ovf = C.c_int(0)
        self.engine._check(self.engine.lib.pa_yolo_wait(self.handle, t, C.byref(ovf)))
        return boxes, kpts, counts, bool(ovf.value)

    def head_shapes(self, h: int, w: int, imgsz: int, pre_mode: int = PRE_LETTERBOX, letterbox_auto: bool = True) -> list:
        if pre_mode == PRE_PIL_STRETCH or not letterbox_auto:
            nh = nw = imgsz
        else:
            r = min(imgsz / h, imgsz / w)
            rw, rh = int(round(w * r)), int(round(h * r))
            nw, nh = rw + (imgsz - rw) % 32, rh + (imgsz - rh) % 32
        c = self.graph.bufs[self.graph.head_buf[0]][1]
        return [(nh >> (3 + l), nw >> (3 + l), c) for l in range(3)]

    def yolo_postprocess(self, heads, h: int, w: int, *, imgsz: int, conf: float, iou: float,
                         classes: Optional[Sequence[int]] = None, max_det: int = 300, pre_mode: int = PRE_LETTERBOX):
        heads = [np.ascontiguousarray(x, np.float32) for x in heads]
        n = heads[0].shape[0]
        assert [x.shape[1:] for x in heads] == [tuple(s) for s in self.head_shapes(h, w, imgsz, pre_mode)], [x.shape for x in heads]
        p, cls_arr = _yolo_params(classes, imgsz=imgsz, pre_mode=pre_mode, channel_reverse=0, letterbox_auto=1, conf=conf, iou=iou,
                                  max_det=max_det, frames_on_device=0)
        ptrs = (C.c_void_p * 3)(*[x.ctypes.data for x in heads])
        boxes, kpts, counts = self._fresh_outputs(n, max_det)
        self.engine._check(self.engine.lib.pa_yolo_postprocess(self.handle, ptrs, n, h, w, C.byref(p), boxes.ctypes.data,
                                                               kpts.ctypes.data if kpts is not None else None, counts.ctypes.data))
        return boxes, kpts, counts

    def fill_arena(self, byte_value: int = 0xFF) -> None:
        self.engine._check(self.engine.lib.pa_model_fill_arena(self.handle, int(byte_value)))

    def take_overflow(self) -> bool:
        v = C.c_int(0)
        self.engine._check(self.engine.lib.pa_model_take_overflow(self.handle, C.byref(v)))
        return bool(v.value)

    def read_head(self, level: int, n: int) -> np.ndarray:
        hh, ww, cc = C.c_int(), C.c_int(), C.c_int()
        self.engine._check(self.engine.lib.pa_yolo_head_shape(self.handle, level, C.byref(hh), C.byref(ww), C.byref(cc)))
        out = np.empty((n, hh.value, ww.value, cc.value), np.float32)
        self.engine._check(self.engine.lib.pa_yolo_read_head(self.handle, level, n, out.ctypes.data))
        return out

    def last_post_path(self) -> int:
        return int(self.engine.lib.pa_yolo_last_post_path(self.handle))

    def last_stem_path(self) -> int:
        return int(self.engine.lib.pa_model_last_stem_path(self.handle))

    def lanes_allocated(self) -> int:
        return int(self.engine.lib.pa_model_lanes_allocated(self.handle))

    def resample_passes(self) -> int:
        return int(self.engine.lib.pa_yolo_resample_passes(self.handle))

    def last_lane(self) -> int:
        return int(self.engine.lib.pa_model_last_lane(self.handle))

    def read_netin(self, n: int) -> np.ndarray:
        hh, ww = C.c_int(), C.c_int()
        self.engine._check(self.engine.lib.pa_yolo_netin_shape(self.handle, C.byref(hh), C.byref(ww)))
        out = np.empty((n, hh.value, ww.value, 4), np.uint8)
        self.engine._check(self.engine.lib.pa_yolo_read_netin(self.handle, n, out.ctypes.data))
        return out

    def plan_bytes(self) -> tuple:
        a, l = C.c_size_t(), C.c_size_t()
        self.engine._check(self.engine.lib.pa_model_plan_bytes(self.handle, C.byref(a), C.byref(l)))
        return a.value, l.value

    def tracknet_infer(self, x: np.ndarray) -> np.ndarray:
        x = np.ascontiguousarray(x, np.float16 if self.graph.dtype == G.DTYPE_F16 else np.float32)
        n, h, w, c = x.shape
        assert c == self.graph.bufs[0][1], (c, self.graph.bufs[0])
        lvl, cout = self.graph.bufs[self.graph.head_buf[0]]
        out = np.empty((n, h >> lvl, w >> lvl, cout), np.float32)
        self.engine._check(self.engine.lib.pa_tracknet_infer(self.handle, x.ctypes.data, n, h, w, 0, out.ctypes.data, 0))
        return out

    def resnet_infer(self, frames, n: int, h: int, w: int, *, want_logits: bool = False):
        frames, ptr, n, on_dev = _frames_arg(frames, n, h, w)
        c = next((o["cout"] for o in self.graph.ops if o["kind"] == G.OP_GAP_FC), 0)
        xy = np.zeros((n, c), np.float32) if c else None
        logits = np.zeros((n, c), np.float32) if (c and want_logits) else None
        self.engine._check(self.engine.lib.pa_resnet_infer(self.handle, ptr, n, h, w, int(on_dev),
                                                           xy.ctypes.data if c else None,
                                                           logits.ctypes.data if logits is not None else None))
        return xy, logits

    def resnet_read_netin(self, n: int) -> np.ndarray:
        out = np.empty((n, G.RESNET_INPUT, G.RESNET_INPUT, 4), np.uint8)
        self.engine._check(self.engine.lib.pa_resnet_read_netin(self.handle, n, out.ctypes.data))
        return out

    def read_fc(self, n: int):
        c = next(o["cout"] for o in self.graph.ops if o["kind"] == G.OP_GAP_FC)
        xy, logits = np.empty((n, c), np.float32), np.empty((n, c), np.float32)
        self.engine._check(self.engine.lib.pa_resnet_read_fc(self.handle, n, xy.ctypes.data, logits.ctypes.data))
        return xy, logits

    def resnet_read_head(self, n: int) -> np.ndarray:
        lvl, ch = self.graph.bufs[self.graph.head_buf[0]]
        out = np.empty((n, G.RESNET_INPUT >> lvl, G.RESNET_INPUT >> lvl, ch), np.float32)
        self.engine._check(self.engine.lib.pa_resnet_read_head(self.handle, n, out.ctypes.data))
        return out

    def last_profile(self, cap: int = 4096):
        kinds = np.zeros(cap, np.int32)
        ms = np.zeros(cap, np.float32)
        fl = np.zeros(cap, np.float64)
        ks = np.zeros(cap, np.int32)
        n = self.engine.lib.pa_model_last_profile(self.handle, cap, kinds.ctypes.data, ms.ctypes.data, fl.ctypes.data,
                                                  ks.ctypes.data)
        return [dict(kind=int(kinds[i]), ms=float(ms[i]), flops=float(fl[i]), ksize=int(ks[i])) for i in range(n)]

    def profile_rows(self):
        buf = C.create_string_buffer(1 << 20)
        self.engine.lib.pa_model_profile_text(self.handle, buf, len(buf))
        return parse_profile_text(buf.value.decode())

    def close(self):
        if self.handle:
            self.engine.lib.pa_model_destroy(self.handle)
            self.handle = None
            self._free_rings()


PROF_PRE, PROF_DECODE, PROF_NMS = 100, 101, 102


def parse_profile_text(text: str):
    rows = []
    for line in text.splitlines():
        f = line.split(",")
        k, ks, M, co, ci, st, mf, nf, ms, fl, res = (f + ["0"])[:11]
        rows.append(dict(kind=int(k), ksize=int(ks), M=int(M), cout=int(co), cin=int(ci), stride=int(st),
                         mf=int(mf), nf=int(nf), ms=float(ms), flops=float(fl), res=int(res),
                         tile=int(f[11]) if len(f) > 11 and f[11] else -1, family=f[12] if len(f) > 12 else ""))
    return rows


class NativeByteTrack:

    def __init__(self, track_activation_threshold: float = 0.25, lost_track_buffer: int = 30,
                 minimum_matching_threshold: float = 0.8, frame_rate: int = 30):
        self.lib = load_library()
        h = C.c_void_p()
        if self.lib.pa_bytetrack_create(track_activation_threshold, lost_track_buffer, minimum_matching_threshold,
                                        int(frame_rate), C.byref(h)) != 0:
            raise EngineError("pa_bytetrack_create failed")
        self.handle = h

    def reset(self) -> None:
        self.lib.pa_bytetrack_reset(self.handle)

    def update_batch(self, boxes: np.ndarray, counts: np.ndarray, keep: Optional[np.ndarray] = None) -> np.ndarray:
        boxes = np.ascontiguousarray(boxes, np.float32)
        counts = np.ascontiguousarray(counts, np.int32)
        n, stride, six = boxes.shape
        assert six == 6 and counts.shape == (n,)
        kp = None
        if keep is not None:
            keep = np.ascontiguousarray(keep, np.uint8)
            assert keep.shape == (n, stride)
            kp = keep.ctypes.data
        ids = np.empty((n, stride), np.int32)
        if self.lib.pa_bytetrack_update_batch(self.handle, boxes.ctypes.data, counts.ctypes.data, kp, n, stride,
                                              ids.ctypes.data) != 0:
            raise EngineError("pa_bytetrack_update_batch failed")
        return ids

    def update_with_detections(self, detections):
        n = len(detections)
        boxes = np.zeros((1, max(n, 1), 6), np.float32)
        boxes[0, :n, :4] = detections.xyxy
        boxes[0, :n, 4] = 1.0 if detections.confidence is None else detections.confidence
        ids = self.update_batch(boxes, np.array([n], np.int32))[0, :n]
        out = detections[np.nonzero(ids >= 0)[0]]
        out.tracker_id = ids[ids >= 0].astype(int)
        return out

    def __del__(self):
        if getattr(self, "handle", None):
            self.lib.pa_bytetrack_destroy(self.handle)
            self.handle = None


class BallSession:

    H, W = 288, 512

    def __init__(self, model: Model, src_h: int, src_w: int):
        self.model, self.src_h, self.src_w = model, src_h, src_w
        h = C.c_void_p()
        model.engine._check(model.engine.lib.pa_ball_create(model.handle, src_h, src_w, C.byref(h)))
        self.handle = h
        self.max_feed = model.max_batch

    def set_background(self, median_rgb: np.ndarray):
        m = np.ascontiguousarray(median_rgb, np.uint8)
        assert m.shape == (self.src_h, self.src_w, 3), m.shape
        self.model.engine._check(self.model.engine.lib.pa_ball_set_background(self.handle, m.ctypes.data))

    def background_from_frames(self, frames_bgr, want_median: bool = False, n: Optional[int] = None):
        on_dev = isinstance(frames_bgr, DeviceBuffer)
        frames_bgr, ptr, n, _ = _frames_arg(frames_bgr, n if on_dev else None, self.src_h, self.src_w)
        med = np.empty((self.src_h, self.src_w, 3), np.uint8) if want_median else None
        self.model.engine._check(self.model.engine.lib.pa_ball_background_from_frames(
            self.handle, ptr, n, int(on_dev), med.ctypes.data if want_median else None))
        return med

    def feed(self, frames_bgr, flush: bool = False, want_heat: bool = False,
             want_rects: bool = False, want_masks: bool = True, n: Optional[int] = None):
        on_dev = isinstance(frames_bgr, DeviceBuffer)
        ptr = None
        if not on_dev:
            n = 0 if frames_bgr is None else len(frames_bgr)
        if on_dev or n:
            frames_bgr, ptr, n, _ = _frames_arg(frames_bgr, n, self.src_h, self.src_w)
            assert 0 < n <= self.max_feed
        masks = np.empty((n + 7, self.H, self.W), np.uint8) if (want_masks or not want_rects) else None
        heat = np.empty((n + 7, self.H, self.W), np.float32) if want_heat else None
        rects = np.empty((n + 7, 4), np.int32) if want_rects else None
        cnt = C.c_int(0)
        self.model.engine._check(self.model.engine.lib.pa_ball_feed(
            self.handle, ptr, n, int(on_dev), int(flush), masks.ctypes.data if masks is not None else None,
            heat.ctypes.data if want_heat else None, rects.ctypes.data if want_rects else None, C.byref(cnt)))
        k = cnt.value
        out = (None if masks is None else masks[:k], heat[:k] if want_heat else None)
        return out + (rects[:k],) if want_rects else out

    def locate(self, masks: np.ndarray) -> np.ndarray:
        masks = np.ascontiguousarray(masks, np.uint8)
        n = len(masks)
        assert masks.shape == (n, self.H, self.W)
        rects = np.empty((n, 4), np.int32)
        self.model.engine._check(self.model.engine.lib.pa_ball_locate(self.handle, masks.ctypes.data, n, rects.ctypes.data))
        return rects

    def read_resized(self, frame: Optional[int] = None) -> np.ndarray:
        out = np.empty((self.H, self.W, 3), np.uint8)
        self.model.engine._check(self.model.engine.lib.pa_ball_read_resized(self.handle, -1 if frame is None else int(frame),
                                                                            out.ctypes.data))
        return out

    def close(self):
        if self.handle:
            self.model.engine.lib.pa_ball_destroy(self.handle)
            self.handle = None
```

Baseline: 1114.

## Add 8-row h2v conv tile variant for cin=16 two-product layers

Adds an MF=2 variant of the h2v patch convolution kernel that processes 8x16 output tiles (2 rows per wave) with a smaller LDS patch and launch bounds allowing 3 blocks per CU. It is the default for single-weight (two-product) layers with cin=16, and a tuning knob plus an env var can force 8 or 16 rows. The change trades more halo reloading per output for higher occupancy and more tiles, aimed at small-channel layers where parallelism is limited. It also adds a diagnostic query for which row count ran.

```diff
diff --git a/include/padel_hip.h b/include/padel_hip.h
--- a/include/padel_hip.h
+++ b/include/padel_hip.h
@@ -222,6 +222,7 @@
 int pa_yolo_resample_passes(pa_model* m);
 int pa_model_last_lane(pa_model* m);
 int pa_model_last_stem_path(pa_model* m);
+int pa_model_last_h2v_rows(pa_model* m);
 
 int pa_yolo_netin_shape(pa_model* m, int* h, int* w);
 int pa_yolo_read_netin(pa_model* m, int n, uint8_t* out);
diff --git a/padel_analytics_amd/csrc/conv_patch_h2v.hip b/padel_analytics_amd/csrc/conv_patch_h2v.hip
--- a/padel_analytics_amd/csrc/conv_patch_h2v.hip
+++ b/padel_analytics_amd/csrc/conv_patch_h2v.hip
@@ -8,16 +8,24 @@
 constexpr int kVPlaneB = kVSpans * 1024;
 constexpr int kVTSpans = (kPatchSqPix + 31) / 32;
 constexpr int kVTPlaneB = kVTSpans * 1024;
-
-}
-
-template <int NF, bool CHUNK, bool TAIL, bool WS>
-__global__ void __launch_bounds__(256, 2) conv_h2v_kernel(const ConvArgs a) {
+constexpr int kV8Spans = (kPatchPix + 15) / 16;
+constexpr int kV8PlaneB = kV8Spans * 1024;
+constexpr int kV8TSpans = (kPatchPix + 31) / 32;
+constexpr int kV8TPlaneB = kV8TSpans * 1024;
+
+}
+
+template <int NF, bool CHUNK, bool TAIL, bool WS, int MF = 4>
+__global__ void __launch_bounds__(256, MF == 4 ? 2 : 3) conv_h2v_kernel(const ConvArgs a) {
     static_assert(CHUNK || TAIL, "cin = 32 CHUNK + 16 TAIL");
     static_assert(WS || NF <= 2, "three products: 2 fragments per wave (6 register sets of 4 VGPRs per step)");
-    constexpr int MF = 4;
-    constexpr int PATCH_B = (CHUNK ? 2 * kVPlaneB : 0);
-    constexpr int TPATCH_B = (TAIL ? 2 * kVTPlaneB : 0);
+    static_assert(MF == 4 || (MF == 2 && WS), "rows per wave: 4 (16 x 16 tiles), or 2 (8 x 16 tiles; two-product layers)");
+    constexpr int LH = MF == 4 ? 4 : 3;
+    constexpr int PIX = MF == 4 ? kPatchSqPix : kPatchPix;
+    constexpr int SPANS = MF == 4 ? kVSpans : kV8Spans, PLANE_B = MF == 4 ? kVPlaneB : kV8PlaneB;
+    constexpr int TSPANS = MF == 4 ? kVTSpans : kV8TSpans, TPLANE_B = MF == 4 ? kVTPlaneB : kV8TPlaneB;
+    constexpr int PATCH_B = (CHUNK ? 2 * PLANE_B : 0);
+    constexpr int TPATCH_B = (TAIL ? 2 * TPLANE_B : 0);
     constexpr int NSTEPS = (CHUNK ? 9 : 0) + (TAIL ? 5 : 0);
     constexpr int NPL = WS ? 1 : 2;
     constexpr int NW = NF * NPL;
@@ -33,7 +41,7 @@
     const XcdSlot slot = xcd_slot(nmt, nnt, bid);
     if (xcd_slot_padding(slot)) return;
     const int mt = xcd_slot_mtile(slot), nt = slot.nt;
-    const TileOrigin org = tile_origin<4, 4>(a.Ho, a.Wo, mt);
+    const TileOrigin org = tile_origin<LH, 4>(a.Ho, a.Wo, mt);
     const int n = org.n, y0 = org.y0, x0 = org.x0;
     const int f0 = nt * NF;
 
@@ -46,13 +54,13 @@
         const int p_q = (lane & 3) ^ (((lane >> 4) & 1) << 1);
         const unsigned p_piece = (unsigned)((p_q >> 1) * 64 + (p_q & 1) * 16);
 #define PADEL_HV_PSPAN(S_)                                                                                        \
-        if (((S_) & 3) == wave) {                                                                                 \
+        if constexpr ((S_) < SPANS) if (((S_) & 3) == wave) {                                                     \
             const int pp_ = (S_) * 16 + p_lane;                                                                   \
             const int py_ = pp_ / kPatchW, px_ = pp_ - py_ * kPatchW;                                             \
-            const bool ok_ = pp_ < kPatchSqPix && (unsigned)(y0 - 1 + py_) < (unsigned)a.H && (unsigned)(x0 - 1 + px_) < (unsigned)a.W; \
+            const bool ok_ = pp_ < PIX && (unsigned)(y0 - 1 + py_) < (unsigned)a.H && (unsigned)(x0 - 1 + px_) < (unsigned)a.W; \
             const unsigned vo_ = ok_ ? (unsigned)((py_ * a.W + px_) * a.in_cs * 4) + p_piece : kOOR;              \
             lds_dma<(S_) * 1024>(vo_, rsrcP, 0u, lp0);                                                            \
-            lds_dma<kVPlaneB + (S_) * 1024>(vo_, rsrcP, 32u, lp0);                                                \
+            lds_dma<PLANE_B + (S_) * 1024>(vo_, rsrcP, 32u, lp0);                                                 \
         }
         PADEL_HV_PSPAN(0) PADEL_HV_PSPAN(1) PADEL_HV_PSPAN(2) PADEL_HV_PSPAN(3) PADEL_HV_PSPAN(4) PADEL_HV_PSPAN(5) PADEL_HV_PSPAN(6)
         PADEL_HV_PSPAN(7) PADEL_HV_PSPAN(8) PADEL_HV_PSPAN(9) PADEL_HV_PSPAN(10) PADEL_HV_PSPAN(11) PADEL_HV_PSPAN(12) PADEL_HV_PSPAN(13)
@@ -64,13 +72,13 @@
         const unsigned t_piece = (unsigned)(((lane & 1) ^ ((lane >> 4) & 1)) * 16);
         const unsigned t_so = CHUNK ? 128u : 0u;
 #define PADEL_HV_TSPAN(S_)                                                                                        \
-        if (((S_) & 3) == ((wave + 1) & 3)) {                                                                     \
+        if constexpr ((S_) < TSPANS) if (((S_) & 3) == ((wave + 1) & 3)) {                                        \
             const int pp_ = (S_) * 32 + t_lane;                                                                   \
             const int py_ = pp_ / kPatchW, px_ = pp_ - py_ * kPatchW;                                             \
-            const bool ok_ = pp_ < kPatchSqPix && (unsigned)(y0 - 1 + py_) < (unsigned)a.H && (unsigned)(x0 - 1 + px_) < (unsigned)a.W; \
+            const bool ok_ = pp_ < PIX && (unsigned)(y0 - 1 + py_) < (unsigned)a.H && (unsigned)(x0 - 1 + px_) < (unsigned)a.W; \
             const unsigned vo_ = ok_ ? (unsigned)((py_ * a.W + px_) * a.in_cs * 4) + t_piece : kOOR;              \
             lds_dma<PATCH_B + (S_) * 1024>(vo_, rsrcP, t_so, lp0);                                                \
-            lds_dma<PATCH_B + kVTPlaneB + (S_) * 1024>(vo_, rsrcP, t_so + 32u, lp0);                              \
+            lds_dma<PATCH_B + TPLANE_B + (S_) * 1024>(vo_, rsrcP, t_so + 32u, lp0);                               \
         }
         PADEL_HV_TSPAN(0) PADEL_HV_TSPAN(1) PADEL_HV_TSPAN(2) PADEL_HV_TSPAN(3) PADEL_HV_TSPAN(4) PADEL_HV_TSPAN(5)
         PADEL_HV_TSPAN(6) PADEL_HV_TSPAN(7) PADEL_HV_TSPAN(8) PADEL_HV_TSPAN(9) PADEL_HV_TSPAN(10)
@@ -116,11 +124,11 @@
     if constexpr (CHUNK) {
 #pragma unroll
         for (int r = 0; r < 8; ++r) {
-            const int p0 = 4 * wave * kPatchW + lr;
+            const int p0 = MF * wave * kPatchW + lr;
             rbase[r] = (unsigned)(p0 * 64 + ((lq ^ ((((p0 + r) >> 2) & 1) << 1)) << 4));
         }
     }
-    const int rd_pix = 4 * wave * kPatchW + lr;
+    const int rd_pix = MF * wave * kPatchW + lr;
 
     f32x4 acc[MF][NF], part[MF][NF], cross[MF][NF];
 #pragma unroll
@@ -133,7 +141,7 @@
         constexpr int d_ = (R_) * kPatchW + (KX_);                                                                \
         const char* p_ = ldsb + rbase[d_ & 7];                                                                    \
         ah[(R_) & 3] = *reinterpret_cast<const h16x8*>(p_ + d_ * 64);                                             \
-        am[(R_) & 3] = *reinterpret_cast<const h16x8*>(p_ + d_ * 64 + kVPlaneB);                                  \
+        am[(R_) & 3] = *reinterpret_cast<const h16x8*>(p_ + d_ * 64 + PLANE_B);                                   \
     } while (0)
 #define PADEL_HV_MFMA_ROW(F_, S_, ST_)                                                                            \
     do {                                                                                                          \
@@ -180,6 +188,28 @@
             PADEL_HV_MFMA_ROW(1, 3, T_);                                                                          \
             if constexpr (kx_ < 2) PADEL_HV_READROW(3, kx_ + 1);                                                  \
             __builtin_amdgcn_sched_barrier(0);                                                                    \
+        }                                                                                                         \
+    } while (0)
+#define PADEL_HV_STEP2(T_)                                                                                        \
+    do {                                                                                                          \
+        constexpr int kx_ = h2_tap_kx(T_), ky_ = h2_tap_ky(T_);                                                   \
+        PADEL_HV_TOP(T_);                                                                                         \
+        if constexpr (ky_ == 0) {                                                                                 \
+            PADEL_HV_MFMA_ROW(0, 0, T_);                                                                          \
+            if constexpr (kx_ > 0) PADEL_HV_READROW(2, kx_);        \
+            __builtin_amdgcn_sched_barrier(0);                                                                    \
+            PADEL_HV_MFMA_ROW(1, 1, T_);                                                                          \
+        } else if constexpr (ky_ == 1) {                                                                          \
+            PADEL_HV_MFMA_ROW(0, 1, T_);                                                                          \
+            if constexpr (kx_ > 0) PADEL_HV_READROW(3, kx_);        \
+            if constexpr (kx_ < 2) PADEL_HV_READROW(0, kx_ + 1);        \
+            __builtin_amdgcn_sched_barrier(0);                                                                    \
+            PADEL_HV_MFMA_ROW(1, 2, T_);                                                                          \
+        } else {                                                                                                  \
+            PADEL_HV_MFMA_ROW(0, 2, T_);                                                                          \
+            if constexpr (kx_ < 2) PADEL_HV_READROW(1, kx_ + 1);        \
+            __builtin_amdgcn_sched_barrier(0);                                                                    \
+            PADEL_HV_MFMA_ROW(1, 3, T_);                                                                          \
         }                                                                                                         \
     } while (0)
 #define PADEL_HV_TSTEP(JT_, ST_)                                                                                  \
@@ -191,11 +221,12 @@
             const int pa_ = rp_ + (f + h2_tap_ky(ta_)) * kPatchW + h2_tap_kx(ta_), pb_ = rp_ + (f + h2_tap_ky(tb_)) * kPatchW + h2_tap_kx(tb_); \
             const char* p_ = ldsb + PATCH_B + swz_tail_off((lq >> 1) ? pb_ : pa_, lq & 1);                        \
             ah[f] = *reinterpret_cast<const h16x8*>(p_);                                                          \
-            am[f] = *reinterpret_cast<const h16x8*>(p_ + kVTPlaneB);                                              \
+            am[f] = *reinterpret_cast<const h16x8*>(p_ + TPLANE_B);                                               \
         }                                                                                                         \
         __builtin_amdgcn_sched_barrier(0);                                                                        \
         PADEL_HV_TOP(ST_);                                                                                        \
-        PADEL_HV_MFMA_ROW(0, 0, ST_); PADEL_HV_MFMA_ROW(1, 1, ST_); PADEL_HV_MFMA_ROW(2, 2, ST_); PADEL_HV_MFMA_ROW(3, 3, ST_); \
+        PADEL_HV_MFMA_ROW(0, 0, ST_); PADEL_HV_MFMA_ROW(1, 1, ST_);                                               \
+        if constexpr (MF == 4) { PADEL_HV_MFMA_ROW(2, 2, ST_); PADEL_HV_MFMA_ROW(3, 3, ST_); }                    \
     } while (0)
 #define PADEL_HV_FLUSH()                                                                                          \
     do {                                                                                                          \
@@ -211,8 +242,13 @@
     if constexpr (CHUNK) {
         PADEL_HV_READROW(0, 0); PADEL_HV_READROW(1, 0); PADEL_HV_READROW(2, 0); PADEL_HV_READROW(3, 0);
         __builtin_amdgcn_sched_barrier(0);
-        PADEL_HV_STEP(0); PADEL_HV_STEP(1); PADEL_HV_STEP(2); PADEL_HV_STEP(3); PADEL_HV_STEP(4);
-        PADEL_HV_STEP(5); PADEL_HV_STEP(6); PADEL_HV_STEP(7); PADEL_HV_STEP(8);
+        if constexpr (MF == 4) {
+            PADEL_HV_STEP(0); PADEL_HV_STEP(1); PADEL_HV_STEP(2); PADEL_HV_STEP(3); PADEL_HV_STEP(4);
+            PADEL_HV_STEP(5); PADEL_HV_STEP(6); PADEL_HV_STEP(7); PADEL_HV_STEP(8);
+        } else {
+            PADEL_HV_STEP2(0); PADEL_HV_STEP2(1); PADEL_HV_STEP2(2); PADEL_HV_STEP2(3); PADEL_HV_STEP2(4);
+            PADEL_HV_STEP2(5); PADEL_HV_STEP2(6); PADEL_HV_STEP2(7); PADEL_HV_STEP2(8);
+        }
         PADEL_HV_FLUSH();
     }
     if constexpr (TAIL) {
@@ -222,6 +258,7 @@
     }
 #undef PADEL_HV_FLUSH
 #undef PADEL_HV_TSTEP
+#undef PADEL_HV_STEP2
 #undef PADEL_HV_STEP
 #undef PADEL_HV_TOP
 #undef PADEL_HV_MFMA_ROW
@@ -232,30 +269,37 @@
     int mpix[MF];
 #pragma unroll
     for (int f = 0; f < MF; ++f) {
-        const int oy = y0 + 4 * wave + f, ox = x0 + lr;
+        const int oy = y0 + MF * wave + f, ox = x0 + lr;
         mpix[f] = (oy < a.Ho && ox < a.Wo) ? (n * a.Ho + oy) * a.Wo + ox : -1;
     }
-    const bool fast = y0 + 16 <= a.Ho && x0 + 16 <= a.Wo && (f0 + NF) * 16 <= a.cout && (((a.out_choff | a.out_cs) & 3) == 0) &&
+    const bool fast = y0 + 4 * MF <= a.Ho && x0 + 16 <= a.Wo && (f0 + NF) * 16 <= a.cout && (((a.out_choff | a.out_cs) & 3) == 0) &&
                       (!a.res || (((a.res_choff | a.res_cs) & 3) == 0));
     h2_epilogue<MF, NF>(a, acc, cross, mpix, f0, lq, fast);
 }
 
-template <int NF, bool WS>
+template <int NF, bool WS, int MF = 4>
 static hipError_t launch_hv(const ConvArgs& a_in, hipStream_t s) {
+    constexpr int ROWS = 4 * MF;
     ConvArgs a = a_in;
     const int batch = a.M / (a.Ho * a.Wo);
-    a.n_mtiles = batch * ((a.Ho + 15) / 16) * ((a.Wo + 15) / 16);
+    a.n_mtiles = batch * ((a.Ho + ROWS - 1) / ROWS) * ((a.Wo + 15) / 16);
     a.n_ntiles = (a.n16 + NF - 1) / NF;
     dim3 grid(8u * (unsigned)((a.n_mtiles + 7) / 8) * (unsigned)a.n_ntiles, 1, 1);
-    if (a.cin == 48) hipLaunchKernelGGL((conv_h2v_kernel<NF, true, true, WS>), grid, dim3(256), 0, s, a);
-    else if (a.cin == 32) hipLaunchKernelGGL((conv_h2v_kernel<NF, true, false, WS>), grid, dim3(256), 0, s, a);
-    else hipLaunchKernelGGL((conv_h2v_kernel<NF, false, true, WS>), grid, dim3(256), 0, s, a);
+    if (a.cin == 48) hipLaunchKernelGGL((conv_h2v_kernel<NF, true, true, WS, MF>), grid, dim3(256), 0, s, a);
+    else if (a.cin == 32) hipLaunchKernelGGL((conv_h2v_kernel<NF, true, false, WS, MF>), grid, dim3(256), 0, s, a);
+    else hipLaunchKernelGGL((conv_h2v_kernel<NF, false, true, WS, MF>), grid, dim3(256), 0, s, a);
     return hipGetLastError();
 }
 
 hipError_t launch_conv_h2v(const ConvArgs& a, int tile, hipStream_t s) {
     const int nf = tile - 340;
-    if (a.w_single) {
+    if (a.w_single && conv_h2v_rows(a, tile) == 8) {
+        switch (nf) {
+            case 1: return launch_hv<1, true, 2>(a, s);
+            case 2: return launch_hv<2, true, 2>(a, s);
+            case 3: return launch_hv<3, true, 2>(a, s);
+        }
+    } else if (a.w_single) {
         switch (nf) {
             case 1: return launch_hv<1, true>(a, s);
             case 2: return launch_hv<2, true>(a, s);
diff --git a/padel_analytics_amd/csrc/conv_select.cpp b/padel_analytics_amd/csrc/conv_select.cpp
--- a/padel_analytics_amd/csrc/conv_select.cpp
+++ b/padel_analytics_amd/csrc/conv_select.cpp
@@ -58,6 +58,7 @@
 #endif
 };
 static const float kH2rThreeProducts = 1.22f;
+static const bool kH2vRows8Default[4] = {false, true, false, false};
 
 static const ConvTile kF16Tiles[] = {
     {30, CONV_TAP16, 0, 128, 128, 1.30f, 1.30f},
@@ -239,6 +240,13 @@
         id -= 30;
     }
     return take(P, a, id, CONV_H2T, out);
+}
+
+int conv_h2v_rows(const ConvArgs& a, int tile) {
+    if (tile < 341 || tile > 343 || !conv_h2v_supported(a) || !a.w_single) return 16;
+    if (a.tune & kTuneH2vRows16) return 16;
+    if (a.tune & kTuneH2vRows8) return 8;
+    return kH2vRows8Default[a.cin >> 4] ? 8 : 16;
 }
 
 const char* conv_family_name(ConvFamily f) {
diff --git a/padel_analytics_amd/csrc/engine.cpp b/padel_analytics_amd/csrc/engine.cpp
--- a/padel_analytics_amd/csrc/engine.cpp
+++ b/padel_analytics_amd/csrc/engine.cpp
@@ -15,6 +15,7 @@
 static int knob_flag(int v) { return v ? 1 : 0; }
 static int knob_tap_pd(int v) { return v == 3 ? 3 : 2; }
 static int knob_lanes(int v) { return v >= 2 ? 2 : 1; }
+static int knob_h2v_rows(int v) { return v == 8 || v == 16 ? v : 0; }
 static const struct Knob { const char* key; const char* env; int Tuning::*field; int (*norm)(int); } kKnobs[] = {
     {"variant", "PADEL_CONV_VARIANT", &Tuning::variant, knob_raw},
     {"tune", "PADEL_CONV_TUNE", &Tuning::tune, knob_raw},
@@ -29,6 +30,7 @@
     {"fuse_head", "PADEL_FUSE_HEAD", &Tuning::fuse_head, knob_flag},
     {"fuse_stem_cv1", "PADEL_FUSE_STEM_CV1", &Tuning::fuse_stem_cv1, knob_flag},
     {"w_single", nullptr, &Tuning::w_single, knob_flag},
+    {"h2v_rows", "PADEL_H2V_ROWS", &Tuning::h2v_rows, knob_h2v_rows},
 };
 
 int pa_abi_version(void) { return PA_ABI_VERSION; }
@@ -435,6 +437,7 @@
     if (plan_steps(m, L, n)) return 1;
     const bool cv1_fused = !e->profiling && !e->t.timeline;
     m->last_stem_path = 0;
+    m->last_h2v_rows = 0;
     for (const Step& st : L.steps) {
         if (skip_tail && st.tail) continue;
         if (cv1_fused && st.stem_cv1) continue;
@@ -452,6 +455,7 @@
         }
         const bool timeline = st.kind == PA_OP_CONV && e->t.timeline && !e->timeline_path.empty() && st.ran.tile == st.requested;
         const hipError_t r = timeline ? launch_conv_timeline(m, st, s) : launch_step(st, st.conv, s);
+        m->last_h2v_rows |= st.h2v_rows == 16 ? 1 : st.h2v_rows == 8 ? 2 : 0;
         prof_end(s, pr);
         if (r != hipSuccess && st.n_ops == 2) PA_FAIL(e, "fused stem + layer 1 launch failed: %s", hipGetErrorString(r));
         if (r != hipSuccess) PA_FAIL(e, "op %d (kind %d) launch failed: %s", st.op, st.kind, hipGetErrorString(r));
@@ -526,9 +530,11 @@
         if (ri != hipSuccess) PA_FAIL(e, "hipGraphInstantiate: %s", hipGetErrorString(ri));
         it = L.graphs.emplace(n, ge).first;
         L.graph_stem_path[n] = m->last_stem_path;
+        L.graph_h2v_rows[n] = m->last_h2v_rows;
     }
     PA_HIP(e, hipGraphLaunch(it->second, s));
     m->last_stem_path = L.graph_stem_path[n];
+    m->last_h2v_rows = L.graph_h2v_rows[n];
     return 0;
 }
 
@@ -571,6 +577,8 @@
 int pa_model_last_lane(pa_model* m) { return m ? m->last_lane : 0; }
 
 int pa_model_last_stem_path(pa_model* m) { return m ? m->last_stem_path : 0; }
+
+int pa_model_last_h2v_rows(pa_model* m) { return m ? m->last_h2v_rows : 0; }
 
 int pa_model_profile_text(pa_model* m, char* buf, size_t cap) {
     size_t off = 0;
diff --git a/padel_analytics_amd/csrc/engine_internal.h b/padel_analytics_amd/csrc/engine_internal.h
--- a/padel_analytics_amd/csrc/engine_internal.h
+++ b/padel_analytics_amd/csrc/engine_internal.h
@@ -104,6 +104,7 @@
     std::vector<Step> steps;
     std::map<int, hipGraphExec_t> graphs;
     std::map<int, int> graph_stem_path;
+    std::map<int, int> graph_h2v_rows;
     DevMem<uint8_t> d_rs_tmp;
     LaneState st;
     size_t device_bytes() const {
@@ -156,6 +157,7 @@
     DevMem<int32_t> d_classes;
     int last_n = 0;
     int last_post_path = 0;
+    int last_h2v_rows = 0;
     int last_stem_path = 0;
     bool heads_stale = false;
     std::vector<ProfRec> prof;
diff --git a/padel_analytics_amd/csrc/kernels.h b/padel_analytics_amd/csrc/kernels.h
--- a/padel_analytics_amd/csrc/kernels.h
+++ b/padel_analytics_amd/csrc/kernels.h
@@ -68,6 +68,8 @@
 int choose_conv_h2_variant(const ConvArgs& a);
 int choose_conv_tap16_variant(const ConvArgs& a);
 bool conv_wants_operand_copy(int ksize, int stride, int cin, bool w_single);
+constexpr int kTuneH2vRows8 = 1 << 20, kTuneH2vRows16 = 1 << 21;
+int conv_h2v_rows(const ConvArgs& a, int tile);
 int h2_ksteps(int cin, int ksize);
 size_t conv_h2r_copy_bytes(int n16, int cin, int ksize);
 
diff --git a/padel_analytics_amd/csrc/launch_plan.cpp b/padel_analytics_amd/csrc/launch_plan.cpp
--- a/padel_analytics_amd/csrc/launch_plan.cpp
+++ b/padel_analytics_amd/csrc/launch_plan.cpp
@@ -88,7 +88,7 @@
         a.M = n * Ho * Wo;
         fill_fastdiv((unsigned)(Ho * Wo), &a.howo_magic, &a.howo_shift);
         fill_fastdiv((unsigned)Wo, &a.wo_magic, &a.wo_shift);
-        a.tune = t.tune; a.tap_pd = t.tap_pd;
+        a.tune = t.tune | (t.h2v_rows == 8 ? kTuneH2vRows8 : t.h2v_rows == 16 ? kTuneH2vRows16 : 0); a.tap_pd = t.tap_pd;
         const bool f16 = d.dtype == PA_DTYPE_F16, h2 = d.dtype == PA_DTYPE_H2;
         const bool use_bx3 = !f16 && !h2 && t.impl == 2 && o.reserved > 0;
         a.w3 = use_bx3 ? (const void*)(p.blob + o.reserved) : nullptr;
@@ -109,6 +109,7 @@
         }
         const ConvRequest r = request_conv(st.path, a, t.variant, fold ? &up : nullptr);
         st.requested = r.tile; st.ran = r.ran; st.family = r.family;
+        st.h2v_rows = r.resolved && r.family == CONV_H2V ? conv_h2v_rows(a, r.ran.tile) : 0;
         return r.resolved;
     }
 
@@ -182,7 +183,7 @@
                 } else {
                     st.conv = ConvArgs{};
                 }
-                st.path = st.requested = 0; st.family = CONV_TAP; st.ran = ConvLaunched{-1, ""};
+                st.path = st.requested = 0; st.family = CONV_TAP; st.ran = ConvLaunched{-1, ""}; st.h2v_rows = 0;
             }
         } else if (o.kind == PA_OP_SPPF_POOL) {
             st.sl = SliceArgs{p.bptr[o.in_buf], d.bufs[o.in_buf].channels, o.in_choff, nullptr, 0, 0, o.cin, n, Ho, Wo, 0, 0, (int)d.dtype, t.fuse_sppf,
diff --git a/padel_analytics_amd/csrc/launch_plan.h b/padel_analytics_amd/csrc/launch_plan.h
--- a/padel_analytics_amd/csrc/launch_plan.h
+++ b/padel_analytics_amd/csrc/launch_plan.h
@@ -21,6 +21,7 @@
     int fuse_sppf = 1;
     int fuse_head = 1;
     int lanes = 2;
+    int h2v_rows = 0;
     int fold_up = 1;
 };
 
@@ -69,6 +70,7 @@
     int requested;
     ConvFamily family;
     ConvLaunched ran;
+    int h2v_rows;
     union {
         StemArgs stem;
         Stem7Args stem7;
diff --git a/padel_analytics_amd/engine.py b/padel_analytics_amd/engine.py
--- a/padel_analytics_amd/engine.py
+++ b/padel_analytics_amd/engine.py
@@ -108,7 +108,7 @@
     "pa_jpeg_encode", "pa_jpeg_check", "pa_jpeg_interval_bytes",
     "pa_jpeg_parse", "pa_jpeg_decode", "pa_jpeg_decode_last_path", "pa_jpeg_decode_last_times",
     "pa_yolo_last_post_path", "pa_jpeg_decode_set_split", "pa_jpeg_decode_last_split",
-    "pa_model_lanes_allocated", "pa_model_last_lane", "pa_model_last_stem_path", "pa_yolo_resample_passes", "pa_device_bytes_live",
+    "pa_model_lanes_allocated", "pa_model_last_lane", "pa_model_last_stem_path", "pa_model_last_h2v_rows", "pa_yolo_resample_passes", "pa_device_bytes_live",
     "pa_frame_activity", "pa_frame_activity_check", "pa_frames_median",
     "pa_box_histograms", "pa_box_histograms_check",
 ]
@@ -155,6 +155,7 @@
     lib.pa_model_lanes_allocated.argtypes = [vp]
     lib.pa_model_last_lane.argtypes = [vp]
     lib.pa_model_last_stem_path.argtypes = [vp]
+    lib.pa_model_last_h2v_rows.argtypes = [vp]
     lib.pa_yolo_resample_passes.argtypes = [vp]
     lib.pa_tracknet_infer.argtypes = [vp, vp, i32, i32, i32, i32, vp, i32]
     lib.pa_resnet_infer.argtypes = [vp, vp, i32, i32, i32, i32, vp, vp]
@@ -897,6 +898,9 @@
     def last_stem_path(self) -> int:
         return int(self.engine.lib.pa_model_last_stem_path(self.handle))
 
+    def last_h2v_rows(self) -> int:
+        return int(self.engine.lib.pa_model_last_h2v_rows(self.handle))
+
     def lanes_allocated(self) -> int:
         return int(self.engine.lib.pa_model_lanes_allocated(self.handle))
 
```

After: 1115, median of 2. No clear change (+0.1%).
